# svenstaro/bvh

Measured on AMD Instinct MI355X. Metric: Mrays/s (build+traverse), higher is better.
Workload: dtype f32; 1 GPU; configs[1]: create_n_cubes(10000), 120000 triangles f32/3D, 1000000 create_ray rays per GPU; step = build_par+flatten+traverse; triangles=120000, rays_per_gpu=1000000, rays_total=1000000, scene_dist=single, flat_array=eager, parallelism=rays sharded x1

## Files before the change

### bvh_amd/csrc/build.hip

```cpp
#include "flatten_node.hpp"

namespace bvhgpu {

constexpr int MAXLV = 96;
constexpr int CTR_SMALL = 0;
constexpr int CTR_MID2 = 2;
constexpr int CTR_FLAGS = 4;
constexpr int CTR_TOPMASK = BUILD_CTR_TOPMASK;
constexpr uint32_t BUILD_FLAG_NONFINITE = 1u;
constexpr uint32_t BUILD_FLAG_PERSIST_GAVE_UP = BSTAT_UNFINISHED;
constexpr uint32_t BUILD_FLAG_EMPTY_SPLIT = 2u;
#ifndef BVH_MID_SMALL_MAXN
#define BVH_MID_SMALL_MAXN 768
#endif
#ifndef BVH_MID_SMALL_THREADS
#define BVH_MID_SMALL_THREADS 384
#endif
template <typename T> struct MidSmallScene {
    static constexpr int MAXN = BVH_MID_SMALL_MAXN;
    static constexpr int THREADS = BVH_MID_SMALL_THREADS;
    static constexpr int HANDOFF = SMALL_MAX;
};
#ifndef BVH_MID_LARGE_MAXN
#define BVH_MID_LARGE_MAXN 1536
#endif
#ifndef BVH_MID_LARGE_THREADS
#define BVH_MID_LARGE_THREADS 256
#endif
template <typename T> struct MidLargeScene {
    static constexpr int MAXN = sizeof(T) == 4 ? BVH_MID_LARGE_MAXN : BVH_MID_LARGE_MAXN * 2 / 3;
    static constexpr int THREADS = BVH_MID_LARGE_THREADS;
    static constexpr int HANDOFF = SMALL_MAX;
};
constexpr size_t MID_SCENE_SPLIT = 250000;
#ifndef BVH_STAT_REP
#define BVH_STAT_REP 8
#endif
constexpr int STAT_REP = BVH_STAT_REP;
constexpr int CTR_LEVEL0 = 16;
constexpr int CTR_XDIR = CTR_LEVEL0 + 2 * MAXLV;
static_assert((CTR_XDIR + 8 * 4) * 4 <= 1024, "the directory lives inside the counter page");
constexpr size_t ROOTKEY_OFF = 1024;
constexpr int PREP_MAX_WG = 1024;

__host__ __device__ inline int lvl_slot(int L) { return L < MAXLV - 2 ? L : (MAXLV - 2 + (L & 1)); }

template <typename T> struct ItemStats {
    typename Traits<T>::Key k[NUM_BUCKETS * STAT_KEYS];
    uint32_t cnt[NUM_BUCKETS];
    uint32_t _pad[2];
};

template <typename T> struct LevelArgs {
    Item<T>* item[2];
    uint4* tile_map[3];
    ItemStats<T>* stats[3];
    uint32_t* tile_cnt[3];
    uint8_t* bk[2];
    uint32_t slot_div, n_slots, n_tiles;
};

template <typename T> struct BuildArgs {
    LevelArgs<T> lv;
    uint32_t mid_max;
    const T* aabbs;
    const T* src;
    typename Traits<T>::Node* nodes;
    uint32_t* node_start;
    uint32_t* node_count;
    uint32_t* shape_node;
    uint16_t* node_slot;
    uint32_t* slot_entry;
    uint32_t n_slots;
    uint32_t* wslot_node;
    uint32_t* idx[2];
    uint8_t* bk;
    Item<T>* big[2];
    Item<T>* mid2;
    Item<T>* small;
    ItemStats<T>* stats[2];
    uint32_t* tile_item[2];
    uint32_t* tile_cnt;
    uint32_t* chunk_cnt[2];
    uint32_t n_chunks;
    FlattenArgs<T> fl;
    uint32_t fl_parts;
    uint32_t tile2;
    uint32_t* ctr;
    typename Traits<T>::Key* rootkeys;
    uint32_t prep_wgs;
    uint32_t n;
    unsigned long long* xbar;
};
constexpr int XBAR_WORDS = 8 * 32;

__device__ __forceinline__ bool key_is_min(int j) { return j < 3 || (j >= 6 && j < 9); }

template <typename T>
__device__ void push_item(const BuildArgs<T>& a, int next_level, uint32_t ni, uint32_t parent, uint32_t start,
                          uint32_t count, const T* A, const T* C, uint32_t heap, int lane);
template <typename T> __device__ void init_stats(ItemStats<T>* s, int lane);

template <typename T> __global__ __launch_bounds__(256) void k_prep(BuildArgs<T> a) {
    using Tr = Traits<T>;
    using Key = typename Tr::Key;
    __shared__ Key sk[STAT_KEYS];
    if (threadIdx.x < STAT_KEYS) sk[threadIdx.x] = key_is_min(threadIdx.x) ? Tr::KEY_POS_INF : Tr::KEY_NEG_INF;
    __syncthreads();
    T loc[STAT_KEYS];
#pragma unroll
    for (int j = 0; j < STAT_KEYS; j++) loc[j] = key_is_min(j) ? Tr::inf() : -Tr::inf();
    if (a.lv.tile_map[0]) {
        const uint32_t gt = blockIdx.x * blockDim.x + threadIdx.x, gs = gridDim.x * blockDim.x;
        for (uint32_t i = gt; i < 3u * a.lv.n_tiles; i += gs) a.lv.tile_map[i / a.lv.n_tiles][i % a.lv.n_tiles] = make_uint4(NONE, 0u, 0u, 0u);
        const uint32_t nc = a.lv.n_tiles * (uint32_t)NUM_BUCKETS;
        for (uint32_t i = gt; i < 3u * nc; i += gs) a.lv.tile_cnt[i / nc][i % nc] = 0u;
    }
    if (a.lv.tile_map[0] && blockIdx.x == 0 && threadIdx.x < WAVE)
        for (int r = 0; r < STAT_REP; r++) init_stats<T>(&a.lv.stats[0][r], (int)threadIdx.x);
    if (a.xbar && blockIdx.x == 0)
        for (uint32_t i = threadIdx.x; i < (uint32_t)XBAR_WORDS; i += blockDim.x) a.xbar[i] = 0ull;
    if (a.chunk_cnt[0] && blockIdx.x == 1 % gridDim.x)
        for (uint32_t i = threadIdx.x; i < 2u * a.n_chunks * 2u * (uint32_t)NUM_BUCKETS; i += blockDim.x) a.chunk_cnt[0][i] = 0u;
    if (blockIdx.x == 0) {
        for (uint32_t i = threadIdx.x; i < a.n_slots; i += blockDim.x) a.slot_entry[i] = NONE;
        for (uint32_t i = threadIdx.x; i < WIDE_SLOTS; i += blockDim.x) a.wslot_node[i] = NONE;
    }
    const bool copy = a.src != a.aabbs;
    T* own = const_cast<T*>(a.aabbs);
    bool bad = false;
    for (uint32_t i = blockIdx.x * blockDim.x + threadIdx.x; i < a.n; i += gridDim.x * blockDim.x) {
        a.idx[0][i] = i;
        const T* b = a.src + 6 * (size_t)i;
        T bx[6];
#pragma unroll
        for (int k = 0; k < 6; k++) bx[k] = b[k];
#pragma unroll
        for (int k = 0; k < 6; k++) bad = bad || !(fabs(bx[k]) < Tr::inf());
        if (copy) {
#pragma unroll
            for (int k = 0; k < 6; k++) own[6 * (size_t)i + k] = bx[k];
        }
#pragma unroll
        for (int k = 0; k < 3; k++) {
            const T c = center1(bx[k], bx[3 + k]);
            loc[k] = join_min(loc[k], bx[k]);
            loc[3 + k] = join_max(loc[3 + k], bx[3 + k]);
            loc[6 + k] = join_min(loc[6 + k], c);
            loc[9 + k] = join_max(loc[9 + k], c);
        }
    }
    {
        const int lane = lane_id();
#pragma unroll
        for (int d = 32; d > 0; d >>= 1) {
            T u[STAT_KEYS];
#pragma unroll
            for (int j = 0; j < STAT_KEYS; j++) u[j] = lane_fetch(loc[j], (lane ^ d) << 2);
#pragma unroll
            for (int j = 0; j < STAT_KEYS; j++) loc[j] = key_is_min(j) ? join_min(loc[j], u[j]) : join_max(loc[j], u[j]);
        }
        if (lane == 0) {
#pragma unroll
            for (int j = 0; j < STAT_KEYS; j++) {
                if (key_is_min(j)) atomicMin(&sk[j], Tr::key(loc[j]));
                else atomicMax(&sk[j], Tr::key(loc[j]));
            }
        }
    }
    if (a.n > 1 && __any(bad) && lane_id() == 0) atomicOr(&a.ctr[CTR_FLAGS], BUILD_FLAG_NONFINITE);
    __syncthreads();
    if (threadIdx.x < STAT_KEYS) a.rootkeys[(size_t)blockIdx.x * STAT_KEYS + threadIdx.x] = sk[threadIdx.x];
}

template <typename T> __global__ __launch_bounds__(256) void k_root(BuildArgs<T> a, uint32_t prep_wgs, int fused) {
    using Tr = Traits<T>;
    using Key = typename Tr::Key;
    __shared__ Key sk[STAT_KEYS];
    if (threadIdx.x < STAT_KEYS) sk[threadIdx.x] = key_is_min(threadIdx.x) ? Tr::KEY_POS_INF : Tr::KEY_NEG_INF;
    __syncthreads();
    for (uint32_t e = threadIdx.x; e < prep_wgs * (uint32_t)STAT_KEYS; e += blockDim.x) {
        const Key v = a.rootkeys[e];
        const int j = (int)(e % (uint32_t)STAT_KEYS);
        if (key_is_min(j)) atomicMin(&sk[j], v);
        else atomicMax(&sk[j], v);
    }
    __syncthreads();
    if (threadIdx.x < WAVE) {
        T A[6], C[6];
#pragma unroll
        for (int k = 0; k < 6; k++) { A[k] = Tr::unkey(sk[k]); C[k] = Tr::unkey(sk[6 + k]); }
        uint32_t flags = a.ctr[CTR_FLAGS];
        if (a.n > 1) {
            bool ovf = false;
#pragma unroll
            for (int k = 0; k < 3; k++) ovf = ovf || !(fabs(C[3 + k] - C[k]) < Tr::inf());
            if (ovf) { flags |= BUILD_FLAG_NONFINITE; if (threadIdx.x == 0) atomicOr(&a.ctr[CTR_FLAGS], BUILD_FLAG_NONFINITE); }
        }
        if (flags & BUILD_FLAG_NONFINITE) return;
        if (fused && a.n > a.mid_max) {
            const int lane = (int)threadIdx.x;
            Item<T>* it = &a.lv.item[0][0];
            if (lane == 0) {
                it->ni = 0; it->parent = 0; it->start = 0; it->count = a.n; it->tile_base = 0; it->parity = 0; it->heap = 1u; it->_r1 = 0;
                a.ctr[CTR_LEVEL0] = 1u;
            }
            if (lane < 6) { it->A[lane] = A[lane]; it->C[lane] = C[lane]; }
            const uint32_t ntile = (a.n + TILE - 1) / TILE;
            for (uint32_t j = lane; j < ntile; j += WAVE) a.lv.tile_map[0][j] = make_uint4(0u, 0u, a.n, 0u);
            for (int r = 0; r < STAT_REP; r++) init_stats<T>(&a.lv.stats[0][r], lane);
        } else {
            push_item<T>(a, 0, 0u, 0u, 0u, a.n, A, C, 1u, (int)threadIdx.x);
        }
    }
}

template <typename T> __device__ void init_stats(ItemStats<T>* s, int lane) {
    using Tr = Traits<T>;
    for (int j = lane; j < NUM_BUCKETS * STAT_KEYS; j += WAVE)
        s->k[j] = key_is_min(j % STAT_KEYS) ? Tr::KEY_POS_INF : Tr::KEY_NEG_INF;
    if (lane < NUM_BUCKETS) s->cnt[lane] = 0;
}

template <typename T>
__device__ void push_item(const BuildArgs<T>& a, int next_level, uint32_t ni, uint32_t parent, uint32_t start,
                          uint32_t count, const T* A, const T* C, uint32_t heap, int lane) {
    const int nslot = lvl_slot(next_level);
    const int npar = next_level & 1;
    uint32_t slot = 0, tb = 0;
    const bool is_small = count <= (uint32_t)SMALL_MAX;
    const bool is_mid2 = !is_small && count <= a.mid_max;
    const uint32_t ntile = (count + a.tile2 - 1) / a.tile2;
    if (lane == 0) {
        if (is_small) slot = atomicAdd(&a.ctr[CTR_SMALL], 1u);
        else if (is_mid2) slot = atomicAdd(&a.ctr[CTR_MID2], 1u);
        else {
            slot = atomicAdd(&a.ctr[CTR_LEVEL0 + 2 * nslot], 1u);
            tb = atomicAdd(&a.ctr[CTR_LEVEL0 + 2 * nslot + 1], ntile);
        }
    }
    slot = __shfl(slot, 0);
    tb = __shfl(tb, 0);
    Item<T>* it = is_small ? &a.small[slot] : (is_mid2 ? &a.mid2[slot] : &a.big[npar][slot]);
    if (lane == 0) {
        it->ni = ni; it->parent = parent; it->start = start; it->count = count;
        it->tile_base = tb; it->parity = (uint32_t)npar; it->heap = heap; it->_r1 = 0;
    }
    if (lane < 6) { it->A[lane] = A[lane]; it->C[lane] = C[lane]; }
    if (!is_small && !is_mid2) {
        for (uint32_t j = lane; j < ntile; j += WAVE) a.tile_item[npar][tb + j] = slot;
        for (int r = 0; r < STAT_REP; r++) init_stats<T>(&a.stats[npar][(size_t)slot * STAT_REP + r], lane);
    }
}

template <typename T>
__device__ void push_pair(const BuildArgs<T>& a, int next_level, uint32_t parent, uint32_t li, uint32_t lstart, uint32_t lcount,
                          const T* AL, const T* CL, uint32_t lheap, uint32_t ri, uint32_t rstart, uint32_t rcount,
                          const T* AR, const T* CR, uint32_t rheap, int lane) {
    const int nslot = lvl_slot(next_level);
    const int npar = next_level & 1;
    const uint32_t mycount = lane == 0 ? lcount : rcount;
    const int mykind = mycount <= (uint32_t)SMALL_MAX ? 0 : (mycount <= a.mid_max ? 1 : 3);
    const uint32_t myntile = (mycount + a.tile2 - 1) / a.tile2;
    uint32_t slot = 0, tb = 0;
    if (lane < 2) {
        if (mykind == 0) slot = atomicAdd(&a.ctr[CTR_SMALL], 1u);
        else if (mykind == 1) slot = atomicAdd(&a.ctr[CTR_MID2], 1u);
        else {
            const unsigned long long old = atomicAdd(reinterpret_cast<unsigned long long*>(&a.ctr[CTR_LEVEL0 + 2 * nslot]),
                                                     1ull | ((unsigned long long)myntile << 32));
            slot = (uint32_t)old; tb = (uint32_t)(old >> 32);
        }
    }
#pragma unroll
    for (int side = 0; side < 2; side++) {
        const uint32_t cslot = __shfl(slot, side), ctb = __shfl(tb, side);
        const int kind = __shfl(mykind, side);
        const uint32_t ccount = side ? rcount : lcount, ntile = (ccount + a.tile2 - 1) / a.tile2;
        Item<T>* it = kind == 0 ? &a.small[cslot] : (kind == 1 ? &a.mid2[cslot] : &a.big[npar][cslot]);
        if (lane == 0) {
            it->ni = side ? ri : li; it->parent = parent; it->start = side ? rstart : lstart; it->count = ccount;
            it->tile_base = ctb; it->parity = (uint32_t)npar; it->heap = side ? rheap : lheap; it->_r1 = 0;
        }
        if (lane < 6) { it->A[lane] = side ? AR[lane] : AL[lane]; it->C[lane] = side ? CR[lane] : CL[lane]; }
        if (kind == 3) {
            for (uint32_t j = lane; j < ntile; j += WAVE) a.tile_item[npar][ctb + j] = cslot;
            for (int r = 0; r < STAT_REP; r++) init_stats<T>(&a.stats[npar][(size_t)cslot * STAT_REP + r], lane);
        }
    }
}

template <typename T> __global__ __launch_bounds__(256) void k_init(BuildArgs<T> a) {
    for (int i = threadIdx.x; i < (int)(ROOTKEY_OFF / 4); i += 256) a.ctr[i] = 0;
}

template <typename T> __global__ __launch_bounds__(256) void k_publish_build(BuildArgs<T> a, uint32_t* __restrict__ host_page) {
    for (int i = threadIdx.x; i < (int)(ROOTKEY_OFF / 4); i += 256) { host_page[i] = a.ctr[i]; a.ctr[i] = 0; }
    __threadfence_system();
}

#ifndef BVH_CHUNK_TILES
#define BVH_CHUNK_TILES 256
#endif
constexpr int SCATTER_AHEAD = 4;
constexpr int CHUNK_TILES = BVH_CHUNK_TILES;
constexpr int BIN_REP = 16;
template <typename T> __global__ __launch_bounds__(256) void k_bin(BuildArgs<T> a, int level) {
    using Tr = Traits<T>;
    using Key = typename Tr::Key;
    const int slot = lvl_slot(level), par = level & 1;
    const uint32_t ntiles = a.ctr[CTR_LEVEL0 + 2 * slot + 1];
    __shared__ Key sk[BIN_REP][NUM_BUCKETS * STAT_KEYS];
    __shared__ uint32_t sc[BIN_REP][NUM_BUCKETS];
    const uint32_t* idx = a.idx[par];
    const int rep = threadIdx.x & (BIN_REP - 1);
    for (uint32_t t = blockIdx.x; t < ntiles; t += gridDim.x) {
        const uint32_t item_id = a.tile_item[par][t];
        const Item<T>* it = &a.big[par][item_id];
        const uint32_t start = it->start, count = it->count;
        const uint32_t p0 = start + (t - it->tile_base) * a.tile2;
        const uint32_t pend = min(start + count, p0 + a.tile2);
        T C[6];
#pragma unroll
        for (int k = 0; k < 6; k++) C[k] = it->C[k];
        const int ax = largest_axis(C);
        const T cmin = C[ax];
        const T ext = C[3 + ax] - C[ax];
        const bool degen = ext < Tr::eps();
        const uint32_t half = count / 2;
        for (int j = threadIdx.x; j < BIN_REP * NUM_BUCKETS * STAT_KEYS; j += 256)
            (&sk[0][0])[j] = key_is_min(j % STAT_KEYS) ? Tr::KEY_POS_INF : Tr::KEY_NEG_INF;
        if (threadIdx.x < BIN_REP * NUM_BUCKETS) (&sc[0][0])[threadIdx.x] = 0;
        __syncthreads();
        for (uint32_t p = p0 + threadIdx.x; p < pend; p += 256) {
            const uint32_t s = idx[p];
            const T* b = a.aabbs + 6 * (size_t)s;
            T bx[6];
#pragma unroll
            for (int k = 0; k < 6; k++) bx[k] = b[k];
            T c[3];
#pragma unroll
            for (int k = 0; k < 3; k++) c[k] = center1(bx[k], bx[3 + k]);
            int bkt;
            if (degen) bkt = (p - start) < half ? 0 : 1;
            else bkt = bucket_of(c[ax], cmin, ext);
            a.bk[p] = (uint8_t)bkt;
            Key* kk = &sk[rep][bkt * STAT_KEYS];
#pragma unroll
            for (int k = 0; k < 3; k++) {
                atomicMin(&kk[k], Tr::key(bx[k]));
                atomicMax(&kk[3 + k], Tr::key(bx[3 + k]));
                Key kc = Tr::key(c[k]);
                atomicMin(&kk[6 + k], kc);
                atomicMax(&kk[9 + k], kc);
            }
            atomicAdd(&sc[rep][bkt], 1u);
        }
        __syncthreads();
        ItemStats<T>* gs = &a.stats[par][(size_t)item_id * STAT_REP + ((t - it->tile_base) & (STAT_REP - 1))];
        if (threadIdx.x < NUM_BUCKETS) {
            uint32_t c = 0;
#pragma unroll
            for (int r = 0; r < BIN_REP; r++) c += sc[r][threadIdx.x];
            sc[0][threadIdx.x] = c;
            a.tile_cnt[t * NUM_BUCKETS + threadIdx.x] = c;
            if (c) atomicAdd(&gs->cnt[threadIdx.x], c);
            if (c && count > (uint32_t)CHUNK_TILES * a.tile2) {
                const uint32_t blk = t / (uint32_t)CHUNK_TILES;
                const uint32_t slot = it->tile_base > blk * (uint32_t)CHUNK_TILES ? 1u : 0u;
                atomicAdd(&a.chunk_cnt[par][(size_t)(blk * 2u + slot) * NUM_BUCKETS + threadIdx.x], c);
            }
        }
        __syncthreads();
        if (threadIdx.x < NUM_BUCKETS * STAT_KEYS) {
            const int j = threadIdx.x;
            if (sc[0][j / STAT_KEYS]) {
                Key v = sk[0][j];
                const bool mn = key_is_min(j % STAT_KEYS);
#pragma unroll
                for (int r = 1; r < BIN_REP; r++) { const Key u = sk[r][j]; v = mn ? (u < v ? u : v) : (u > v ? u : v); }
                if (mn) atomicMin(&gs->k[j], v);
                else atomicMax(&gs->k[j], v);
            }
        }
        __syncthreads();
    }
}

template <typename T> __device__ __forceinline__ void box_empty(T* b) {
    b[0] = b[1] = b[2] = Traits<T>::inf();
    b[3] = b[4] = b[5] = -Traits<T>::inf();
}
template <typename T> __device__ __forceinline__ void box_join(T* a, const T* b) {
#pragma unroll
    for (int k = 0; k < 3; k++) {
        a[k] = tmin(a[k], b[k]);
        a[3 + k] = tmax(a[3 + k], b[3 + k]);
    }
}

template <typename T, typename KeyPtr, typename CntPtr>
__device__ __forceinline__ uint32_t sah_select(KeyPtr keys, CntPtr cnts, const T* A, bool degen, uint32_t* cnt, T* AL,
                                               T* CL, T* AR, T* CR, bool& no_winner) {
    using Tr = Traits<T>;
    using Key = typename Tr::Key;
    Key pa[NUM_BUCKETS][6], sa[NUM_BUCKETS][6];
#pragma unroll
    for (int b = 0; b < NUM_BUCKETS; b++) {
        cnt[b] = cnts[b];
#pragma unroll
        for (int k = 0; k < 6; k++) { pa[b][k] = keys[b * STAT_KEYS + k]; sa[b][k] = pa[b][k]; }
    }
#pragma unroll
    for (int b = 1; b < NUM_BUCKETS; b++) {
#pragma unroll
        for (int k = 0; k < 3; k++) {
            pa[b][k] = pa[b][k] < pa[b - 1][k] ? pa[b][k] : pa[b - 1][k];
            pa[b][3 + k] = pa[b][3 + k] > pa[b - 1][3 + k] ? pa[b][3 + k] : pa[b - 1][3 + k];
        }
    }
#pragma unroll
    for (int b = NUM_BUCKETS - 2; b >= 0; b--) {
#pragma unroll
        for (int k = 0; k < 3; k++) {
            sa[b][k] = sa[b][k] < sa[b + 1][k] ? sa[b][k] : sa[b + 1][k];
            sa[b][3 + k] = sa[b][3 + k] > sa[b + 1][3 + k] ? sa[b][3 + k] : sa[b + 1][3 + k];
        }
    }
    T min_cost = Tr::inf();
    int best = -1;
    const T sa_parent = surface_area(A);
    uint32_t ln = 0, total = 0;
#pragma unroll
    for (int b = 0; b < NUM_BUCKETS; b++) total += cnt[b];
#pragma unroll
    for (int s = 0; s < NUM_BUCKETS - 1; s++) {
        ln += cnt[s];
        T la[6], ra[6];
#pragma unroll
        for (int k = 0; k < 6; k++) { la[k] = Tr::unkey(pa[s][k]); ra[k] = Tr::unkey(sa[s + 1][k]); }
        T cl = (T)ln * surface_area(la);
        T cr = (T)(total - ln) * surface_area(ra);
        T num = cl + cr;
        T cost = num / sa_parent;
        bool take = degen ? (s == 0) : (cost < min_cost);
        if (take) { min_cost = cost; best = s; }
    }
    no_winner = best < 0;
    if (best < 0) {
        box_empty(AL); box_empty(CL); box_empty(AR); box_empty(CR);
        return cnt[0];
    }
    Key cl_[6], cr_[6];
#pragma unroll
    for (int k = 0; k < 6; k++) {
        cl_[k] = key_is_min(k) ? Tr::KEY_POS_INF : Tr::KEY_NEG_INF;
        cr_[k] = cl_[k];
    }
    uint32_t nl = 0;
#pragma unroll
    for (int b = 0; b < NUM_BUCKETS; b++) {
        const bool left = b <= best;
        if (left) nl += cnt[b];
#pragma unroll
        for (int k = 0; k < 6; k++) {
            const Key v = keys[b * STAT_KEYS + 6 + k];
            const Key jl = key_is_min(k) ? (v < cl_[k] ? v : cl_[k]) : (v > cl_[k] ? v : cl_[k]);
            const Key jr = key_is_min(k) ? (v < cr_[k] ? v : cr_[k]) : (v > cr_[k] ? v : cr_[k]);
            cl_[k] = left ? jl : cl_[k];
            cr_[k] = left ? cr_[k] : jr;
        }
    }
#pragma unroll
    for (int k = 0; k < 6; k++) {
        Key l = pa[0][k], r = sa[1][k];
#pragma unroll
        for (int s = 1; s < NUM_BUCKETS - 1; s++) { if (best == s) { l = pa[s][k]; r = sa[s + 1][k]; } }
        AL[k] = Tr::unkey(l); AR[k] = Tr::unkey(r);
        CL[k] = Tr::unkey(cl_[k]); CR[k] = Tr::unkey(cr_[k]);
    }
    return nl;
}

template <typename T> __device__ void select_role(const BuildArgs<T>& a, int level, uint32_t block, uint32_t nblocks) {
    using Tr = Traits<T>;
    const int slot = lvl_slot(level), par = level & 1;
    const uint32_t nitems = a.ctr[CTR_LEVEL0 + 2 * slot];
    const int lane = lane_id();
    const uint32_t wave0 = (block * blockDim.x + threadIdx.x) >> 6;
    const uint32_t nwaves = (nblocks * blockDim.x) >> 6;
    for (uint32_t id = wave0; id < nitems; id += nwaves) {
        const Item<T>* it = &a.big[par][id];
        __shared__ ItemStats<T> s_merged[4];
        ItemStats<T>* st = &s_merged[threadIdx.x >> 6];
        {
            using Key = typename Tr::Key;
            const ItemStats<T>* rep = &a.stats[par][(size_t)id * STAT_REP];
            for (int j = lane; j < NUM_BUCKETS * STAT_KEYS; j += WAVE) {
                const bool mn = key_is_min(j % STAT_KEYS);
                Key v = rep[0].k[j];
#pragma unroll
                for (int r = 1; r < STAT_REP; r++) { const Key u = rep[r].k[j]; v = mn ? (u < v ? u : v) : (u > v ? u : v); }
                st->k[j] = v;
            }
            if (lane < NUM_BUCKETS) {
                uint32_t c = 0;
#pragma unroll
                for (int r = 0; r < STAT_REP; r++) c += rep[r].cnt[lane];
                st->cnt[lane] = c;
            }
        }
        const uint32_t ni = it->ni, parent = it->parent, start = it->start, count = it->count;
        T A[6], C[6];
#pragma unroll
        for (int k = 0; k < 6; k++) { A[k] = it->A[k]; C[k] = it->C[k]; }
        const int ax = largest_axis(C);
        const T ext = C[3 + ax] - C[ax];
        const bool degen = ext < Tr::eps();

        uint32_t cnt[NUM_BUCKETS];
        T AL[6], CL[6], AR[6], CR[6];
        bool no_winner;
        const uint32_t nl = sah_select<T>(st->k, st->cnt, A, degen, cnt, AL, CL, AR, CR, no_winner);
        if (no_winner && lane == 0) atomicOr(&a.ctr[CTR_FLAGS], BUILD_FLAG_EMPTY_SPLIT);
        const uint32_t li = ni + 1;
        const uint32_t ri = li + (2 * nl - 1);
        if (lane == 0) {
            typename Tr::Node* nd = &a.nodes[ni];
#pragma unroll
            for (int k = 0; k < 3; k++) {
                nd->l_min[k] = AL[k]; nd->l_max[k] = AL[3 + k];
                nd->r_min[k] = AR[k]; nd->r_max[k] = AR[3 + k];
            }
            nd->parent = parent; nd->l = li; nd->r = ri; nd->shape = NONE;
            a.node_start[ni] = start;
            a.node_count[ni] = count;
            a.node_slot[ni] = (uint16_t)it->heap;
            if (it->heap < 16u) atomicOr(&a.ctr[CTR_TOPMASK], 1u << it->heap);
        }
        push_pair<T>(a, level + 1, ni, li, start, nl, AL, CL, heap_child(it->heap, 0u), ri, start + nl, count - nl, AR, CR,
                     heap_child(it->heap, 1u), lane);

    }
}

template <typename T> __device__ void scatter_role(const BuildArgs<T>& a, int level, uint32_t block, uint32_t nblocks) {
    const int slot = lvl_slot(level), par = level & 1;
    const uint32_t ntiles = a.ctr[CTR_LEVEL0 + 2 * slot + 1];
    __shared__ uint32_t run[NUM_BUCKETS];
    __shared__ uint32_t wcnt[4][NUM_BUCKETS];
    __shared__ __attribute__((aligned(16))) uint32_t wcnt2[2][NUM_BUCKETS][4];
    const int lane = lane_id(), w = threadIdx.x >> 6;
    const unsigned long long lt = lanemask_lt();
    const uint32_t* src = a.idx[par];
    uint32_t* dst = a.idx[par ^ 1];
    for (uint32_t t = block; t < ntiles; t += nblocks) {
        const Item<T>* it = &a.big[par][a.tile_item[par][t]];
        const uint32_t start = it->start, count = it->count;
        const uint32_t p0 = start + (t - it->tile_base) * a.tile2;
        const uint32_t pend = min(start + count, p0 + a.tile2);
        {
            const uint32_t tl = t - it->tile_base, ntl = (count + a.tile2 - 1) / a.tile2;
            uint32_t before[NUM_BUCKETS], all[NUM_BUCKETS];
#pragma unroll
            for (int b = 0; b < NUM_BUCKETS; b++) { before[b] = 0; all[b] = 0; }
            const uint32_t* tc = a.tile_cnt + (size_t)it->tile_base * NUM_BUCKETS;
            if (count > (uint32_t)CHUNK_TILES * a.tile2) {
                const uint32_t T0 = it->tile_base, T1 = T0 + ntl;
                const uint32_t g0 = T0 / (uint32_t)CHUNK_TILES, g1 = (T1 - 1u) / (uint32_t)CHUNK_TILES, gt = t / (uint32_t)CHUNK_TILES;
                const uint32_t* cc = a.chunk_cnt[par];
                for (uint32_t g = g0 + threadIdx.x; g <= g1; g += 256) {
                    const uint32_t sl = T0 > g * (uint32_t)CHUNK_TILES ? 1u : 0u;
#pragma unroll
                    for (int b = 0; b < NUM_BUCKETS; b++) {
                        const uint32_t v = cc[(size_t)(g * 2u + sl) * NUM_BUCKETS + b];
                        all[b] += v;
                        before[b] += g < gt ? v : 0u;
                    }
                }
                const uint32_t j0 = max(gt * (uint32_t)CHUNK_TILES, T0);
                for (uint32_t j = j0 + threadIdx.x; j < t; j += 256) {
#pragma unroll
                    for (int b = 0; b < NUM_BUCKETS; b++) before[b] += a.tile_cnt[(size_t)j * NUM_BUCKETS + b];
                }
            } else {
                for (uint32_t j = threadIdx.x; j < ntl; j += 256) {
#pragma unroll
                    for (int b = 0; b < NUM_BUCKETS; b++) {
                        const uint32_t v = tc[(size_t)j * NUM_BUCKETS + b];
                        all[b] += v;
                        before[b] += j < tl ? v : 0u;
                    }
                }
            }
            uint32_t mine[NUM_BUCKETS];
            uint32_t acc = 0;
#pragma unroll
            for (int b = 0; b < NUM_BUCKETS; b++) { mine[b] = acc + before[b]; acc += all[b]; }
#pragma unroll
// ... 1230 lines not shown
        T salv[NUM_BUCKETS - 1], sarv[NUM_BUCKETS - 1];
        {
            int cum = 0;
#pragma unroll
            for (int s2 = 0; s2 < NUM_BUCKETS - 1; s2++) { cum += cnt[s2]; cumv[s2] = cum; }
        }
#pragma unroll
        for (int s2 = 0; s2 < NUM_BUCKETS - 1; s2++) {
            const int q2 = lo + cumv[s2];
            salv[s2] = lane_fetch(saP, (q2 - 1) << 2);
            sarv[s2] = lane_fetch(saS, q2 << 2);
        }
        int nl = cnt[0];
        bool taken = false;
        T min_cost = Tr::inf();
#pragma unroll
        for (int s2 = 0; s2 < NUM_BUCKETS - 1; s2++) {
            T cl = (T)cumv[s2] * salv[s2];
            T cr = (T)(segn - cumv[s2]) * sarv[s2];
            T num = cl + cr;
            T cost = num / saA;
            bool take = degen ? (s2 == 0) : (cost < min_cost);
            if (take) { min_cost = cost; nl = cumv[s2]; taken = true; }
        }
        const int q = lo + nl;
        const int ql4 = (q - 1) << 2, qr4 = q << 2;
        T AL[6], AR[6], Cn[6];
        const bool left = lane < q;
        {
#pragma unroll
            for (int k = 0; k < 6; k++) AL[k] = lane_fetch(P[k], ql4);
#pragma unroll
            for (int k = 0; k < 6; k++) AR[k] = lane_fetch(S[k], qr4);
            const int nlo = done ? lane : (left ? lo : q), nhi = done ? lane + 1 : (left ? q : hi);
            T Cq[6];
#pragma unroll
            for (int k = 0; k < 3; k++) { Cq[k] = c[k]; Cq[3 + k] = c[k]; }
            seg_prefix_scan<T, 6>(Cq, lane, nlo, span);
            const int last4 = (nhi - 1) << 2;
#pragma unroll
            for (int k = 0; k < 6; k++) Cn[k] = lane_fetch(Cq[k], last4);
        }
        if (!taken) { box_empty(AL); box_empty(AR); box_empty(Cn); }
        if (!done && !taken && lane == lo) atomicOr(&a.ctr[CTR_FLAGS], BUILD_FLAG_EMPTY_SPLIT);
        if constexpr (FLAT_INLINE) {
            wave_empty = wave_empty || __any(!done && !taken);
            const unsigned long long cm = __ballot(!done && lane == lo);
            if (!done && lane == lo) my_inner[ninner + (uint32_t)__popcll(cm & lt)] = ni;
            ninner += (uint32_t)__popcll(cm);
        }
        if (!done) {
            const uint32_t li = ni + 1;
            const uint32_t ri = li + (uint32_t)(2 * nl - 1);
            if (lane == lo) {
                typename Tr::Node* nd = &a.nodes[ni];
#pragma unroll
                for (int k = 0; k < 3; k++) {
                    nd->l_min[k] = AL[k]; nd->l_max[k] = AL[3 + k];
                    nd->r_min[k] = AR[k]; nd->r_max[k] = AR[3 + k];
                }
                nd->parent = parent; nd->l = li; nd->r = ri; nd->shape = NONE;
                a.node_start[ni] = istart + lo;
                a.node_count[ni] = segn;
                a.node_slot[ni] = (uint16_t)heap;
            }
            parent = ni;
            if (left) { hi = q; ni = li; saA = surface_area(AL); heap = heap_child(heap, 0u); }
            else { lo = q; ni = ri; saA = surface_area(AR); heap = heap_child(heap, 1u); }
#pragma unroll
            for (int k = 0; k < 6; k++) Cb[k] = Cn[k];
        }
    }
    if constexpr (FLAT_INLINE && sizeof(T) == 4) if (a.fl_parts != 0u) {
        __builtin_amdgcn_fence(__ATOMIC_SEQ_CST, "workgroup");
        const bool with_flat = (a.fl_parts & (uint32_t)FLATTEN_FLAT) != 0u;
        const bool fast = n >= 2 && !(with_flat && wave_empty);
        if (fast) {
            if (with_flat && lane < n) {
                const uint32_t nav = ni - 1u + (istart + (uint32_t)lane);
                typename Tr::Flat fe = {}, lf = {};
#pragma unroll
                for (int k = 0; k < 3; k++) { fe.min[k] = box[k]; fe.max[k] = box[3 + k]; lf.min[k] = Tr::inf(); lf.max[k] = -Tr::inf(); }
                fe.entry = nav + 1u; fe.exit = nav + 2u; fe.shape = NONE;
                lf.entry = NONE; lf.exit = nav + 2u; lf.shape = shape;
                a.fl.flat[nav] = fe;
                a.fl.flat[nav + 1u] = lf;
            }
        }
        const uint32_t nn_item = 2u * (uint32_t)n - 1u;
        const uint32_t todo = fast ? ninner : nn_item;
#pragma unroll 1
        for (uint32_t j = (uint32_t)lane; j < todo; j += WAVE) {
            const uint32_t i = fast ? my_inner[j] : ni0 + j;
            const typename Tr::Node ndf = a.fl.nodes[i];
            if (with_flat) flatten_node<T, FLATTEN_FLAT | FLATTEN_WIDE>(a.fl, i, ndf);
            else flatten_node<T, FLATTEN_WIDE>(a.fl, i, ndf);
        }
    }
#ifdef BVH_SMALL_PROFILE
    if (sp_on) g_small_prof[20 * wave + 18] = wall_clock64();
#endif
    }
}

template <typename T> struct LevelLayout {
    size_t n_slots, n_tiles, sz_tile_item, sz_tile_cnt, sz_stats, off_tile_item, off_tile_cnt, off_stats, bytes;
    LevelLayout(size_t n, size_t mid_max) {
        n_slots = n / (mid_max + 1) + 2;
        n_tiles = n / TILE + n_slots + 4;
        auto up = [](size_t x) { return (x + 255) & ~(size_t)255; };
        sz_tile_item = up(n_tiles * 16);
        sz_tile_cnt = up(n_tiles * NUM_BUCKETS * 4);
        sz_stats = up(n_slots * STAT_REP * sizeof(ItemStats<T>));
        off_tile_item = 0;
        off_tile_cnt = off_tile_item + 3 * sz_tile_item;
        off_stats = off_tile_cnt + 3 * sz_tile_cnt;
        bytes = off_stats + 3 * sz_stats;
    }
};

template <typename T> static bool level_fused(const bvhgpu_tree* t) {
    const int v = t->ctx->tune[BVHGPU_TUNE_BUILD_LEVEL_LAUNCHES];
    return v == 1 || (v != 2 && t->n <= MID_SCENE_SPLIT);
}
template <typename T> static uint32_t level_tile(const bvhgpu_tree* t) {
    if (level_fused<T>(t)) return (uint32_t)TILE;
    const int v = t->ctx->tune[BVHGPU_TUNE_BUILD_LEVEL_TILE];
    if (v > 0) return (uint32_t)std::min(std::max((v + 255) / 256 * 256, (int)TILE), 16384);
    return t->n >= 6000000 ? 4096u : t->n >= 2000000 ? 2048u : t->n >= 600000 ? 1024u : (uint32_t)TILE;
}

template <typename T> static BuildArgs<T> make_args(bvhgpu_tree* t, const T* src) {
    using Tr = Traits<T>;
    using Key = typename Tr::Key;
    BuildArgs<T> a;
    a.aabbs = t->aabbs.as<T>();
    a.src = src ? src : t->aabbs.as<T>();
    a.nodes = t->nodes.as<typename Tr::Node>();
    a.node_start = t->node_start.as<uint32_t>();
    a.node_count = t->node_count.as<uint32_t>();
    a.shape_node = t->shape_node.as<uint32_t>();
    a.node_slot = t->node_slot.as<uint16_t>();
    a.slot_entry = t->slot_entry.as<uint32_t>();
    a.n_slots = TopCfg<T>::SLOTS;
    a.wslot_node = t->wslot_node.as<uint32_t>();
    a.idx[0] = t->idx[0].as<uint32_t>(); a.idx[1] = t->idx[1].as<uint32_t>();
    a.bk = t->bk.as<uint8_t>();
    a.big[0] = t->big[0].as<Item<T>>(); a.big[1] = t->big[1].as<Item<T>>();
    a.mid2 = t->mid2.as<Item<T>>();
    a.small = t->small.as<Item<T>>();
    a.stats[0] = t->stats[0].as<ItemStats<T>>(); a.stats[1] = t->stats[1].as<ItemStats<T>>();
    a.tile_item[0] = t->tile_item[0].as<uint32_t>(); a.tile_item[1] = t->tile_item[1].as<uint32_t>();
    a.tile_cnt = t->tile_cnt.as<uint32_t>();
    a.tile2 = level_tile<T>(t);
    a.fl = FlattenArgs<T>{}; a.fl_parts = 0;
    a.n_chunks = (uint32_t)(t->chunk_cnt.cap / (2 * 2 * NUM_BUCKETS * 4));
    a.chunk_cnt[0] = t->chunk_cnt.as<uint32_t>();
    a.chunk_cnt[1] = a.chunk_cnt[0] ? a.chunk_cnt[0] + (size_t)a.n_chunks * 2 * NUM_BUCKETS : nullptr;
    a.ctr = t->ctr.as<uint32_t>();
    a.rootkeys = reinterpret_cast<Key*>(reinterpret_cast<char*>(t->ctr.p) + ROOTKEY_OFF);
    a.n = (uint32_t)t->n;
    a.xbar = t->xbar.as<unsigned long long>();
    a.prep_wgs = 0;
    const bool small_scene = t->n <= MID_SCENE_SPLIT;
    a.mid_max = (uint32_t)(small_scene ? MidSmallScene<T>::MAXN : MidLargeScene<T>::MAXN);
    const LevelLayout<T> ly(t->n, a.mid_max);
    a.lv.slot_div = a.mid_max + 1u; a.lv.n_slots = (uint32_t)ly.n_slots; a.lv.n_tiles = (uint32_t)ly.n_tiles;
    char* base = t->lvbuf.cap >= ly.bytes ? reinterpret_cast<char*>(t->lvbuf.p) : nullptr;
    for (int i = 0; i < 3; i++) {
        a.lv.tile_map[i] = base ? reinterpret_cast<uint4*>(base + ly.off_tile_item + i * ly.sz_tile_item) : nullptr;
        a.lv.tile_cnt[i] = base ? reinterpret_cast<uint32_t*>(base + ly.off_tile_cnt + i * ly.sz_tile_cnt) : nullptr;
        a.lv.stats[i] = base ? reinterpret_cast<ItemStats<T>*>(base + ly.off_stats + i * ly.sz_stats) : nullptr;
    }
    a.lv.item[0] = a.big[0]; a.lv.item[1] = a.big[1];
    a.lv.bk[0] = a.bk; a.lv.bk[1] = a.bk ? a.bk + t->n : nullptr;
    return a;
}

template <typename T> struct BuildGrid {
    size_t max_big, max_mid2, max_tiles;
    int tile_grid, sel_grid, mid2_grid, small_grid, level_grid;
    BuildGrid(const bvhgpu_tree* t, size_t mid_max) {
        const size_t n = t->n;
        max_big = n / (mid_max + 1) + 2;
        max_mid2 = n / (SMALL_MAX + 1) + 2;
        max_tiles = n / TILE + max_big + 2;
        tile_grid = (int)std::min<size_t>(n / level_tile<T>(t) + max_big + 2, 2048);
        sel_grid = (int)std::min<size_t>((max_big + 3) / 4, 1024);
        mid2_grid = (int)std::min<size_t>(max_mid2, (size_t)t->ctx->n_cu * 4);
        small_grid = (int)std::min<size_t>((n + 3) / 4, (size_t)t->ctx->n_cu * 8);
        level_grid = (int)std::min<size_t>(LevelLayout<T>(n, mid_max).n_tiles, 2048);
    }
};

template <typename T> static void run_level(bvhgpu_tree* t, const BuildArgs<T>& a, const BuildGrid<T>& g, int L) {
    hipStream_t st = t->ctx->stream;
    if (level_fused<T>(t)) {
        if (L == 0) hipLaunchKernelGGL((k_level<T, true>), dim3(g.level_grid), dim3(LEVEL_THREADS), 0, st, a, 0);
        hipLaunchKernelGGL((k_level<T, false>), dim3(g.level_grid), dim3(LEVEL_THREADS), 0, st, a, L + 1);
        return;
    }
    hipLaunchKernelGGL(k_bin<T>, dim3(g.tile_grid), dim3(256), 0, st, a, L);
    hipLaunchKernelGGL(k_split<T>, dim3(g.sel_grid + g.tile_grid), dim3(256), 0, st, a, L, (uint32_t)g.sel_grid);
}
template <typename T> static void run_lower_tiers(bvhgpu_tree* t, const BuildArgs<T>& a, const BuildGrid<T>& g, uint32_t mid2_done,
                                                  uint32_t small_done) {
    hipStream_t st = t->ctx->stream;
    if (t->n > (size_t)SMALL_MAX) {
        if (t->n <= MID_SCENE_SPLIT) hipLaunchKernelGGL((k_mid<T, MidSmallScene<T>>), dim3(g.mid2_grid), dim3(MidSmallScene<T>::THREADS), 0, st, a, mid2_done);
        else hipLaunchKernelGGL((k_mid<T, MidLargeScene<T>>), dim3(g.mid2_grid), dim3(MidLargeScene<T>::THREADS), 0, st, a, mid2_done);
    }
    if (a.fl_parts != 0u) hipLaunchKernelGGL((k_small<T, true>), dim3(g.small_grid), dim3(256), 0, st, a, small_done);
    else hipLaunchKernelGGL((k_small<T, false>), dim3(g.small_grid), dim3(256), 0, st, a, small_done);
}

template <typename T> void build_enqueue(bvhgpu_tree* t, const T* aabbs_dev, size_t n, bool flatten_after, bool redo) {
    using Tr = Traits<T>;
    using Key = typename Tr::Key;
    bvhgpu_ctx* ctx = t->ctx;
    hipStream_t st = ctx->stream;
    join_flat(t);
    t->built = false; t->flattened = false; t->lazy_flat = false; t->pending_build = false; t->exact_only = false; t->pending_recv = false;
    t->pend_persist = false;
    if (!redo) t->gen++;
    if (n != t->n) { t->has_tris = false; t->has_spheres = false; }
    t->n = n; t->n_nodes = n ? 2 * n - 1 : 0;
    t->n_flat = n >= 2 ? 3 * n - 2 : n;
    t->n_trav = n >= 2 ? 2 * n - 2 : n;
    t->levels = 0;
    if (n == 0) { t->built = true; t->flattened = flatten_after; return; }

    const size_t MID_MAX = n <= MID_SCENE_SPLIT ? (size_t)MidSmallScene<T>::MAXN : (size_t)MidLargeScene<T>::MAXN;
    const BuildGrid<T> g(t, MID_MAX);
    t->aabbs.reserve(n * 6 * sizeof(T));
    if (t->nodes.reserve(t->n_nodes * sizeof(typename Tr::Node))) BVH_HIP(hipMemsetAsync(t->nodes.p, 0, t->nodes.cap, st));
    if (t->node_start.reserve(t->n_nodes * 4)) BVH_HIP(hipMemsetAsync(t->node_start.p, 0, t->node_start.cap, st));
    if (t->node_count.reserve(t->n_nodes * 4)) BVH_HIP(hipMemsetAsync(t->node_count.p, 0, t->node_count.cap, st));
    t->shape_node.reserve(n * 4);
    if (t->node_slot.reserve(t->n_nodes * 2)) BVH_HIP(hipMemsetAsync(t->node_slot.p, 0xFF, t->node_slot.cap, st));
    t->slot_entry.reserve(TopCfg<T>::SLOTS * 4);
    t->wslot_node.reserve(WIDE_SLOTS * 4);
    t->idx[0].reserve(n * 4);
    t->idx[1].reserve(n * 4);
    t->bk.reserve(2 * n);
    if (level_fused<T>(t) && n > (size_t)MID_MAX) t->lvbuf.reserve(LevelLayout<T>(n, MID_MAX).bytes);
    const int persist_knob = ctx->tune[BVHGPU_TUNE_BUILD_LEVEL_PERSIST];
    if (t->persist_broken && persist_knob != 0 && !redo && t->persist_retry_in > 0 && --t->persist_retry_in == 0) t->persist_broken = false;
    const bool persist = persist_knob != 0 && !t->persist_broken && level_fused<T>(t) && n >= 32 * (MID_MAX + 1);
    if (persist) t->xbar.reserve(XBAR_WORDS * sizeof(unsigned long long));
    for (int i = 0; i < 2; i++) {
        t->big[i].reserve(g.max_big * sizeof(Item<T>));
        t->stats[i].reserve(g.max_big * STAT_REP * sizeof(ItemStats<T>));
        t->tile_item[i].reserve(g.max_tiles * 4);
    }
    t->mid2.reserve(g.max_mid2 * sizeof(Item<T>));
    t->small.reserve((n + 1) * sizeof(Item<T>));
    t->tile_cnt.reserve(g.max_tiles * NUM_BUCKETS * 4);
    if (!level_fused<T>(t)) t->chunk_cnt.reserve((g.max_tiles / CHUNK_TILES + 2) * 2 * 2 * NUM_BUCKETS * 4);
    if (t->ctr.reserve(ROOTKEY_OFF + (size_t)PREP_MAX_WG * STAT_KEYS * sizeof(Key))) t->ctr_ready = false;
    if (!t->pin) BVH_HIP(hipHostMalloc(&t->pin, ROOTKEY_OFF, hipHostMallocDefault));

    BuildArgs<T> a = make_args<T>(t, aabbs_dev);
    if (!t->ctr_ready) hipLaunchKernelGGL(k_init<T>, dim3(1), dim3(256), 0, st, a);
    t->ctr_ready = false;
#ifndef BVH_PREP_PER_WG
#define BVH_PREP_PER_WG 1024
#endif
    const int prep_grid = (int)std::min<size_t>((n + BVH_PREP_PER_WG - 1) / BVH_PREP_PER_WG, (size_t)PREP_MAX_WG);
    a.prep_wgs = (uint32_t)prep_grid;
    hipLaunchKernelGGL(k_prep<T>, dim3(prep_grid), dim3(256), 0, st, a);
    if (!(level_fused<T>(t) && n > (size_t)MID_MAX)) hipLaunchKernelGGL(k_root<T>, dim3(1), dim3(256), 0, st, a, (uint32_t)prep_grid, 0);

    int level = 0;
    if (n > (size_t)MID_MAX) {
        int fixed = 1;
        for (size_t m = n; m > (size_t)MID_MAX; m = (m + 1) / 2) fixed++;
        if (t->hint_levels > 0 && t->hint_n == n) fixed = t->hint_levels;
        if (fixed > MAXLV - 4) fixed = MAXLV - 4;
        if (persist) {
            for (; level < 3; level++) run_level<T>(t, a, g, level);
            const int nx = persist_knob >= 8 ? std::min(persist_knob, 64) : 32;
            hipLaunchKernelGGL((k_level<T, false, true>), dim3(8 * nx), dim3(LEVEL_THREADS), 0, st, a, 4);
            t->pend_persist = true;
            fixed = level;
        }
        for (; level < fixed; level++) {
            run_level<T>(t, a, g, level);
            if (level == 3 && ctx->tune[BVHGPU_TUNE_WIDE_EARLY_ITEMS] != 0 && !t->pend_persist) {
                if (!t->ev_top) BVH_HIP(hipEventCreateWithFlags(&t->ev_top, hipEventDisableTiming));
                BVH_HIP(hipEventRecord(t->ev_top, st));
                t->ev_top_gen = t->gen;
            }
        }
    }
    uint32_t inline_parts = 0;
    if (flatten_after && n >= 2 && sizeof(T) == 4 && ctx->tune[BVHGPU_TUNE_FLATTEN_INLINE] != 0) {
        const FlattenPlan p = flatten_plan<T>(t, ctx->tune[BVHGPU_TUNE_FLATTEN_LAZY] != 0);
        if (p.with_wide) {
            inline_parts = (uint32_t)(p.parts & (FLATTEN_FLAT | FLATTEN_WIDE));
            a.fl = flatten_args<T>(t, p.with_wide, p.with_guide); a.fl_parts = inline_parts;
        }
    }
    run_lower_tiers<T>(t, a, g, 0u, 0u);
    t->bstat.reserve(64);
    if (flatten_after && n >= 1)
        flatten_tree<T>(t, a.ctr, reinterpret_cast<uint32_t*>(t->pin), (uint32_t)(ROOTKEY_OFF / 4), t->bstat.as<uint32_t>(), (uint32_t)CTR_FLAGS,
                        (n > (size_t)MID_MAX && !t->pend_persist) ? (uint32_t)(CTR_LEVEL0 + 2 * lvl_slot(level)) : (uint32_t)CTR_FLAGS,
                        ctx->tune[BVHGPU_TUNE_FLATTEN_LAZY] != 0, inline_parts);
    else hipLaunchKernelGGL(k_publish_build<T>, dim3(1), dim3(256), 0, st, a, reinterpret_cast<uint32_t*>(t->pin));
    t->ctr_ready = true;
    t->pending_build = true; t->pend_level = level; t->pend_flatten = flatten_after;
}

template <typename T> void build_finalize(bvhgpu_tree* t) {
    if (!t->pending_build) return;
    t->pending_build = false;
    bvhgpu_ctx* ctx = t->ctx;
    hipStream_t st = ctx->stream;
    join_flat(t);
    BVH_HIP(hipStreamSynchronize(st));
    BVH_HIP(hipGetLastError());
    const size_t n = t->n;
    const size_t MID_MAX = n <= MID_SCENE_SPLIT ? (size_t)MidSmallScene<T>::MAXN : (size_t)MidLargeScene<T>::MAXN;
    uint32_t* pin = reinterpret_cast<uint32_t*>(t->pin);
    if (pin[CTR_FLAGS] & BUILD_FLAG_NONFINITE) {
        t->flattened = false;
        t->failed_gen = t->gen; t->failed_what = Fail::NonFinite;
        throw HipFail{hipErrorInvalidValue, nullptr, __LINE__, Fail::NonFinite};
    }
    if (t->pend_persist && (pin[CTR_FLAGS] & BUILD_FLAG_PERSIST_GAVE_UP)) {
        t->persist_broken = true;
        t->persist_retry_in = 64;
        const bool fl = t->pend_flatten;
        build_enqueue<T>(t, static_cast<const T*>(nullptr), n, fl, true);
        build_finalize<T>(t);
        t->redone_gen = t->gen;
        return;
    }
    int level = t->pend_persist ? MAXLV - 3 : t->pend_level;
    if (n > (size_t)MID_MAX && !t->pend_persist && pin[CTR_LEVEL0 + 2 * lvl_slot(level)] != 0) {
        const BuildGrid<T> g(t, MID_MAX);
        const BuildArgs<T> a = make_args<T>(t, nullptr);
        BVH_HIP(hipMemcpyAsync(a.ctr, t->pin, ROOTKEY_OFF, hipMemcpyHostToDevice, st));
        t->ctr_ready = false;
        uint32_t mid2_done = pin[CTR_MID2], small_done = pin[CTR_SMALL];
        while (true) {
            if (level + 1 >= MAXLV - 2)
                BVH_HIP(hipMemsetAsync(a.ctr + CTR_LEVEL0 + 2 * lvl_slot(level + 1), 0, 8, st));
            run_level<T>(t, a, g, level);
            level++;
            BVH_HIP(hipMemcpyAsync(t->pin, a.ctr, ROOTKEY_OFF, hipMemcpyDeviceToHost, st));
            BVH_HIP(hipStreamSynchronize(st));
            if (pin[CTR_LEVEL0 + 2 * lvl_slot(level)] == 0) break;
        }
        run_lower_tiers<T>(t, a, g, mid2_done, small_done);
        hipLaunchKernelGGL(k_publish_build<T>, dim3(1), dim3(256), 0, st, a, reinterpret_cast<uint32_t*>(t->pin));
        t->ctr_ready = true;
        if (t->pend_flatten) {
            BVH_HIP(hipMemsetAsync(t->wslot_node.p, 0xFF, WIDE_SLOTS * 4, st));
            BVH_HIP(hipMemsetAsync(t->slot_entry.p, 0xFF, TopCfg<T>::SLOTS * 4, st));
            flatten_tree<T>(t);
        }
        BVH_HIP(hipStreamSynchronize(st));
        BVH_HIP(hipGetLastError());
        t->redone_gen = t->gen;
    }
    int used = level;
    while (used > 0 && used - 1 < MAXLV - 2 && pin[CTR_LEVEL0 + 2 * (used - 1)] == 0) used--;
    t->levels = used;
    if (!t->pend_persist) { t->hint_levels = used > 0 ? used : 0; t->hint_n = n; }
    t->exact_only = (pin[CTR_FLAGS] & BUILD_FLAG_EMPTY_SPLIT) != 0;
    t->built = true;
}

template <typename T> void build_tree(bvhgpu_tree* t, const T* aabbs_dev, size_t n, bool flatten_after) {
    build_enqueue<T>(t, aabbs_dev, n, flatten_after, false);
    build_finalize<T>(t);
}

#ifdef BVH_PROFILE_MID
void debug_mid_prof(unsigned long long* out, bool reset) {
    (void)hipDeviceSynchronize();
    (void)hipMemcpyFromSymbol(out, HIP_SYMBOL(g_mid_prof), sizeof(unsigned long long) * 8);
    if (reset) { unsigned long long z[8] = {0}; (void)hipMemcpyToSymbol(HIP_SYMBOL(g_mid_prof), z, sizeof z); }
}
#endif

template void build_tree<float>(bvhgpu_tree*, const float*, size_t, bool);
template void build_tree<double>(bvhgpu_tree*, const double*, size_t, bool);
template void build_enqueue<float>(bvhgpu_tree*, const float*, size_t, bool, bool);
template void build_enqueue<double>(bvhgpu_tree*, const double*, size_t, bool, bool);
template void build_finalize<float>(bvhgpu_tree*);
template void build_finalize<double>(bvhgpu_tree*);

}
```

### bvh_amd/csrc/common.hpp

```cpp
#pragma once

#include <hip/hip_runtime.h>
#include <stdint.h>

#include <cfloat>
#include <cmath>

#include "../../include/bvh_mi355x.h"

namespace bvhgpu {

constexpr uint32_t NONE = BVHGPU_NONE;
constexpr int NUM_BUCKETS = 6;
constexpr int WAVE = 64;
constexpr int SMALL_MAX = 64;
#ifndef BVH_TILE
#define BVH_TILE 512
#endif
constexpr int TILE = BVH_TILE;
constexpr int STAT_KEYS = 12;

template <typename T> struct Traits;

template <> struct Traits<float> {
    using Key = uint32_t;
    using Node = bvhgpu_node_f32;
    using Flat = bvhgpu_flat_f32;
    using Ray = bvhgpu_ray_f32;
    static constexpr int dtype = BVHGPU_F32;
    __host__ __device__ static constexpr float eps() { return FLT_EPSILON; }
    __host__ __device__ static float inf() { return INFINITY; }
    __host__ __device__ static Key key(float f) {
        uint32_t b;
        __builtin_memcpy(&b, &f, 4);
        return (b & 0x80000000u) ? ~b : (b | 0x80000000u);
    }
    __host__ __device__ static float unkey(Key k) {
        uint32_t b = (k & 0x80000000u) ? (k & 0x7FFFFFFFu) : ~k;
        float f;
        __builtin_memcpy(&f, &b, 4);
        return f;
    }
    static constexpr Key KEY_POS_INF = 0xFF800000u;
    static constexpr Key KEY_NEG_INF = 0x007FFFFFu;
};

template <> struct Traits<double> {
    using Key = unsigned long long;
    using Node = bvhgpu_node_f64;
    using Flat = bvhgpu_flat_f64;
    using Ray = bvhgpu_ray_f64;
    static constexpr int dtype = BVHGPU_F64;
    __host__ __device__ static constexpr double eps() { return DBL_EPSILON; }
    __host__ __device__ static double inf() { return INFINITY; }
    __host__ __device__ static Key key(double f) {
        unsigned long long b;
        __builtin_memcpy(&b, &f, 8);
        return (b & 0x8000000000000000ull) ? ~b : (b | 0x8000000000000000ull);
    }
    __host__ __device__ static double unkey(Key k) {
        unsigned long long b = (k & 0x8000000000000000ull) ? (k & 0x7FFFFFFFFFFFFFFFull) : ~k;
        double f;
        __builtin_memcpy(&f, &b, 8);
        return f;
    }
    static constexpr Key KEY_POS_INF = 0xFFF0000000000000ull;
    static constexpr Key KEY_NEG_INF = 0x000FFFFFFFFFFFFFull;
};

template <typename T> struct TravNode;
template <> struct __attribute__((aligned(32))) TravNode<float> {
    float mn[3];
    uint32_t exit;
    float mx[3];
    uint32_t shape;
};
template <> struct __attribute__((aligned(64))) TravNode<double> {
    double mn[3];
    double mx[3];
    uint32_t exit;
    uint32_t shape;
    uint64_t _pad;
};
constexpr uint32_t TRAV_INNER = 0x80000000u;
constexpr uint32_t SLOT_NONE = 0xFFFFu;
__host__ __device__ inline bool trav_is_leaf(uint32_t w) { return (w & TRAV_INNER) == 0u; }
__host__ __device__ inline uint32_t heap_child(uint32_t h, uint32_t side) {
    const uint32_t c = 2u * h + side;
    return (h >= 0x8000u || c > SLOT_NONE) ? SLOT_NONE : c;
}
template <typename T> struct TopCfg;
#ifndef BVH_TOP_SLOTS_F32
#define BVH_TOP_SLOTS_F32 5056
#endif
template <> struct TopCfg<float> { static constexpr uint32_t SLOTS = BVH_TOP_SLOTS_F32; };
template <> struct TopCfg<double> { static constexpr uint32_t SLOTS = 2880; };
static_assert(sizeof(TravNode<float>) == 32, "trav f32");
static_assert(sizeof(TravNode<double>) == 64, "trav f64");

template <typename T> struct WideNode;
template <> struct __attribute__((aligned(128))) WideNode<float> {
    float mn[3][4], mx[3][4];
    uint32_t ref[4];
    uint32_t _pad[4];
};
template <> struct __attribute__((aligned(256))) WideNode<double> {
    double mn[3][4], mx[3][4];
    uint32_t ref[4];
    uint32_t _pad[12];
};
static_assert(sizeof(WideNode<float>) == 128, "wide f32");
static_assert(sizeof(WideNode<double>) == 256, "wide f64");
constexpr double GUIDE_GROW = 1.0 / 262144.0;
constexpr double GUIDE_ORIGIN_MAX = 3.0;
constexpr double GUIDE_SCENE_MIN = 0x1p-125;
constexpr double GUIDE_SCENE_MAX = 0x1p125;
constexpr double GUIDE_F32_MAX = 0x1.fffffep127;
constexpr double GUIDE_F32_MIN_NORMAL = 0x1p-126;
__host__ __device__ inline float f32_below(double x) {
    float f = (float)x;
    if ((double)f > x) {
        uint32_t b; __builtin_memcpy(&b, &f, 4);
        b = f > 0.0f ? b - 1u : (f < 0.0f ? b + 1u : 0x80000001u);
        __builtin_memcpy(&f, &b, 4);
    }
    return f;
}
__host__ __device__ inline float f32_above(double x) { return -f32_below(-x); }
constexpr uint32_t WIDE_INNER = 0x80000000u;
constexpr uint32_t WIDE_RESIDENT = 0x40000000u;
constexpr size_t WIDE_MAX_SHAPES = (size_t)1 << 28;
constexpr uint32_t WIDE_SLOTS = 1365;
__host__ __device__ inline uint32_t wide_level_base(int k) { return ((1u << (2 * k)) - 1u) / 3u; }

template <typename T> struct Item {
    uint32_t ni;
    uint32_t parent;
    uint32_t start;
    uint32_t count;
    uint32_t tile_base;
    uint32_t parity;
    uint32_t heap;
    uint32_t _r1;
    T A[6];
    T C[6];
};

template <typename T> __host__ __device__ inline T tmin(T a, T b) {
    return (a < b || (a == b && signbit(a))) ? a : b;
}
template <typename T> __host__ __device__ inline T tmax(T a, T b) {
    return (a > b || (a == b && !signbit(a))) ? a : b;
}
template <typename T> __host__ __device__ inline T center1(T mn, T mx) {
    T lo = mn * (T)0.5;
    T hi = mx * (T)0.5;
    return lo + hi;
}
template <typename T> __host__ __device__ inline T surface_area(const T* b) {
    T sx = b[3] - b[0], sy = b[4] - b[1], sz = b[5] - b[2];
    T xx = sx * sx, yy = sy * sy, zz = sz * sz;
    T d = xx + yy;
    d = d + zz;
    return (T)2 * d;
}
template <typename T> __host__ __device__ inline int largest_axis(const T* b) {
    T s0 = b[3] - b[0], s1 = b[4] - b[1], s2 = b[5] - b[2];
    int a = 0;
    T m = s0;
    if (s1 > m) { m = s1; a = 1; }
    if (s2 > m) { m = s2; a = 2; }
    return a;
}
template <typename T> __host__ __device__ inline int bucket_of(T c, T cmin, T ext) {
    const T K = (T)NUM_BUCKETS - (T)0.01;
    T rel = (c - cmin) / ext;
    T scaled = rel * K;
    return (int)scaled;
}

__device__ __forceinline__ float join_min(float a, float b) { float r; asm("v_min_f32 %0, %1, %2" : "=v"(r) : "v"(a), "v"(b)); return r; }
__device__ __forceinline__ float join_max(float a, float b) { float r; asm("v_max_f32 %0, %1, %2" : "=v"(r) : "v"(a), "v"(b)); return r; }
__device__ __forceinline__ double join_min(double a, double b) { double r; asm("v_min_f64 %0, %1, %2" : "=v"(r) : "v"(a), "v"(b)); return r; }
__device__ __forceinline__ double join_max(double a, double b) { double r; asm("v_max_f64 %0, %1, %2" : "=v"(r) : "v"(a), "v"(b)); return r; }

template <typename T>
__device__ __forceinline__ bool slab_hit(const T o[3], const T inv[3], const T mn[3], const T mx[3], T& tmin_out,
                                         T& tmax_out) {
    T l0 = (mn[0] - o[0]) * inv[0], h0 = (mx[0] - o[0]) * inv[0];
    T l1 = (mn[1] - o[1]) * inv[1], h1 = (mx[1] - o[1]) * inv[1];
    T l2 = (mn[2] - o[2]) * inv[2], h2 = (mx[2] - o[2]) * inv[2];
    bool nan = (l0 != l0) | (h0 != h0) | (l1 != l1) | (h1 != h1) | (l2 != l2) | (h2 != h2);
    T a0 = join_min(l0, h0), b0 = join_max(l0, h0);
    T a1 = join_min(l1, h1), b1 = join_max(l1, h1);
    T a2 = join_min(l2, h2), b2 = join_max(l2, h2);
    T tmn = join_max(join_max(a0, a1), a2);
    T tmx = join_min(join_min(b0, b1), b2);
    T z = tmn > (T)0 ? tmn : (T)0;
    tmin_out = z;
    tmax_out = tmx;
    return !nan && (tmx >= z);
}

template <typename T>
__device__ __forceinline__ bool slab_hit_finite(const T o[3], const T inv[3], const T mn[3], const T mx[3]) {
    T l0 = (mn[0] - o[0]) * inv[0], h0 = (mx[0] - o[0]) * inv[0];
    T l1 = (mn[1] - o[1]) * inv[1], h1 = (mx[1] - o[1]) * inv[1];
    T l2 = (mn[2] - o[2]) * inv[2], h2 = (mx[2] - o[2]) * inv[2];
    T tmn = fmax(fmax(fmin(l0, h0), fmin(l1, h1)), fmin(l2, h2));
    T tmx = fmin(fmin(fmax(l0, h0), fmax(l1, h1)), fmax(l2, h2));
    return tmx >= fmax(tmn, (T)0);
}
template <>
__device__ __forceinline__ bool slab_hit_finite<float>(const float o[3], const float inv[3], const float mn[3],
                                                       const float mx[3]) {
    float l0 = (mn[0] - o[0]) * inv[0], h0 = (mx[0] - o[0]) * inv[0];
    float l1 = (mn[1] - o[1]) * inv[1], h1 = (mx[1] - o[1]) * inv[1];
    float l2 = (mn[2] - o[2]) * inv[2], h2 = (mx[2] - o[2]) * inv[2];
    float a0, a1, a2, b0, b1, b2, tmn, tmx;
    asm("v_min_f32 %0, %1, %2" : "=v"(a0) : "v"(l0), "v"(h0));
    asm("v_max_f32 %0, %1, %2" : "=v"(b0) : "v"(l0), "v"(h0));
    asm("v_min_f32 %0, %1, %2" : "=v"(a1) : "v"(l1), "v"(h1));
    asm("v_max_f32 %0, %1, %2" : "=v"(b1) : "v"(l1), "v"(h1));
    asm("v_min_f32 %0, %1, %2" : "=v"(a2) : "v"(l2), "v"(h2));
    asm("v_max_f32 %0, %1, %2" : "=v"(b2) : "v"(l2), "v"(h2));
    asm("v_max3_f32 %0, %1, %2, %3" : "=v"(tmn) : "v"(a0), "v"(a1), "v"(a2));
    asm("v_min3_f32 %0, %1, %2, %3" : "=v"(tmx) : "v"(b0), "v"(b1), "v"(b2));
    return (tmx >= tmn) & (tmx >= 0.0f);
}
template <typename T>
__device__ __forceinline__ bool slab_hit_finite_len(const T o[3], const T inv[3], const T mn[3], const T mx[3], T& len) {
    T l0 = (mn[0] - o[0]) * inv[0], h0 = (mx[0] - o[0]) * inv[0];
    T l1 = (mn[1] - o[1]) * inv[1], h1 = (mx[1] - o[1]) * inv[1];
    T l2 = (mn[2] - o[2]) * inv[2], h2 = (mx[2] - o[2]) * inv[2];
    T tmn = fmax(fmax(fmin(l0, h0), fmin(l1, h1)), fmin(l2, h2));
    T tmx = fmin(fmin(fmax(l0, h0), fmax(l1, h1)), fmax(l2, h2));
    const T t0 = fmax(tmn, (T)0);
    len = tmx - t0;
    return tmx >= t0;
}
template <>
__device__ __forceinline__ bool slab_hit_finite_len<float>(const float o[3], const float inv[3], const float mn[3], const float mx[3],
                                                           float& len) {
    float l0 = (mn[0] - o[0]) * inv[0], h0 = (mx[0] - o[0]) * inv[0];
    float l1 = (mn[1] - o[1]) * inv[1], h1 = (mx[1] - o[1]) * inv[1];
    float l2 = (mn[2] - o[2]) * inv[2], h2 = (mx[2] - o[2]) * inv[2];
    float a0, a1, a2, b0, b1, b2, tmn, tmx, t0;
    asm("v_min_f32 %0, %1, %2" : "=v"(a0) : "v"(l0), "v"(h0));
    asm("v_max_f32 %0, %1, %2" : "=v"(b0) : "v"(l0), "v"(h0));
    asm("v_min_f32 %0, %1, %2" : "=v"(a1) : "v"(l1), "v"(h1));
    asm("v_max_f32 %0, %1, %2" : "=v"(b1) : "v"(l1), "v"(h1));
    asm("v_min_f32 %0, %1, %2" : "=v"(a2) : "v"(l2), "v"(h2));
    asm("v_max_f32 %0, %1, %2" : "=v"(b2) : "v"(l2), "v"(h2));
    asm("v_max3_f32 %0, %1, %2, %3" : "=v"(tmn) : "v"(a0), "v"(a1), "v"(a2));
    asm("v_min3_f32 %0, %1, %2, %3" : "=v"(tmx) : "v"(b0), "v"(b1), "v"(b2));
    asm("v_max_f32 %0, 0, %1" : "=v"(t0) : "v"(tmn));
    len = tmx - t0;
    return tmx >= t0;
}
template <typename T> __device__ __forceinline__ bool ray_is_finite(const T o[3], const T inv[3]) {
    bool f = true;
#pragma unroll
    for (int k = 0; k < 3; k++)
        f = f && (fabs(o[k]) < Traits<T>::inf()) && (fabs(inv[k]) < Traits<T>::inf()) && (inv[k] != (T)0);
    return f;
}

__device__ __forceinline__ float lane_fetch(float v, int addr4) {
    return __int_as_float(__builtin_amdgcn_ds_bpermute(addr4, __float_as_int(v)));
}
__device__ __forceinline__ double lane_fetch(double v, int addr4) {
    const long long b = __double_as_longlong(v);
    const int lo = __builtin_amdgcn_ds_bpermute(addr4, (int)(b & 0xFFFFFFFFll));
    const int hi = __builtin_amdgcn_ds_bpermute(addr4, (int)(b >> 32));
    return __longlong_as_double(((long long)hi << 32) | (unsigned int)lo);
}
template <int CTRL, int ROW_MASK = 0xF> __device__ __forceinline__ float dpp_fetch(float v) {
    const int b = __float_as_int(v);
    return __int_as_float(__builtin_amdgcn_update_dpp(b, b, CTRL, ROW_MASK, 0xF, false));
}
template <int CTRL, int ROW_MASK = 0xF> __device__ __forceinline__ double dpp_fetch(double v) {
    const long long b = __double_as_longlong(v);
    const int lo = (int)(b & 0xFFFFFFFFll), hi = (int)(b >> 32);
    const int l2 = __builtin_amdgcn_update_dpp(lo, lo, CTRL, ROW_MASK, 0xF, false);
    const int h2 = __builtin_amdgcn_update_dpp(hi, hi, CTRL, ROW_MASK, 0xF, false);
    return __longlong_as_double(((long long)h2 << 32) | (unsigned int)l2);
}
template <int CTRL, int ROW_MASK = 0xF> __device__ __forceinline__ float dpp_fetch_raw(float v) {
    return __int_as_float(__builtin_amdgcn_mov_dpp(__float_as_int(v), CTRL, ROW_MASK, 0xF, false));
}
template <int CTRL, int ROW_MASK = 0xF> __device__ __forceinline__ double dpp_fetch_raw(double v) {
    const long long b = __double_as_longlong(v);
    const int l2 = __builtin_amdgcn_mov_dpp((int)(b & 0xFFFFFFFFll), CTRL, ROW_MASK, 0xF, false);
    const int h2 = __builtin_amdgcn_mov_dpp((int)(b >> 32), CTRL, ROW_MASK, 0xF, false);
    return __longlong_as_double(((long long)h2 << 32) | (unsigned int)l2);
}
template <int LANE> __device__ __forceinline__ float lane_bcast(float v) { return __int_as_float(__builtin_amdgcn_readlane(__float_as_int(v), LANE)); }
template <int LANE> __device__ __forceinline__ double lane_bcast(double v) {
    const long long b = __double_as_longlong(v);
    const int lo = __builtin_amdgcn_readlane((int)(b & 0xFFFFFFFFll), LANE), hi = __builtin_amdgcn_readlane((int)(b >> 32), LANE);
    return __longlong_as_double(((long long)hi << 32) | (unsigned int)lo);
}
__device__ __forceinline__ int lane_id() { return (int)(threadIdx.x & 63); }
#ifndef BVH_LDS_BARRIER
#define BVH_LDS_BARRIER 1
#endif
__device__ __forceinline__ void lds_barrier() {
#if BVH_LDS_BARRIER
    asm volatile("s_waitcnt lgkmcnt(0)\n\ts_barrier" ::: "memory");
#else
    __syncthreads();
#endif
}
__device__ __forceinline__ unsigned long long lanemask_lt() {
    int l = lane_id();
    return l == 0 ? 0ull : (~0ull >> (64 - l));
}
__device__ __forceinline__ unsigned long long mask_range(int lo, int hi) {
    unsigned long long h = hi >= 64 ? ~0ull : ((1ull << hi) - 1ull);
    unsigned long long l = lo >= 64 ? ~0ull : ((1ull << lo) - 1ull);
    return h & ~l;
}

enum class Fail { None, NonFinite, Overflow, Rebroadcast, RecvRebroadcast, RecvInvalid, RecvGarbled, StaleTree, OrderedDepth };
struct HipFail { hipError_t err; const char* what; int line; Fail kind = Fail::None; };
#define BVH_HIP(x)                                                     \
    do {                                                               \
        hipError_t _e = (x);                                           \
        if (_e != hipSuccess) throw ::bvhgpu::HipFail{_e, #x, __LINE__}; \
    } while (0)

}
```

### bvh_amd/csrc/engine.hpp

```cpp
#pragma once

#include <string>
#include <vector>

#include "common.hpp"

namespace bvhgpu {

struct DevBuf {
    void* p = nullptr;
    size_t cap = 0;
    DevBuf() = default;
    DevBuf(const DevBuf&) = delete;
    DevBuf& operator=(const DevBuf&) = delete;
    ~DevBuf() { release(); }
    bool reserve(size_t bytes) {
        if (bytes <= cap) return false;
        if (p) (void)hipFree(p);
        p = nullptr;
        cap = 0;
        size_t want = bytes + bytes / 8 + 256;
        hipError_t e = hipMalloc(&p, want);
        if (e != hipSuccess) {
            p = nullptr;
            throw HipFail{e, "hipMalloc", __LINE__};
        }
        cap = want;
        return true;
    }
    void release() {
        if (p) (void)hipFree(p);
        p = nullptr;
        cap = 0;
    }
    template <typename U> U* as() const { return reinterpret_cast<U*>(p); }
};

constexpr unsigned TRAVERSE_ANY_HIT = 1u << 31;
constexpr unsigned TRAVERSE_BOX_HIT = 1u << 30;
constexpr unsigned TRAVERSE_SPHERE_HIT = 1u << 29;
constexpr unsigned TRAVERSE_ALLHITS = 1u << 28;

}

struct bvhgpu_comm;
struct bvhgpu_hits;
namespace bvhgpu {
struct HostBatch {
    static constexpr int MAX_CHUNKS = 16;
    bvhgpu_hits* hits[MAX_CHUNKS] = {};
    hipEvent_t ev_up[MAX_CHUNKS] = {}, ev_done[MAX_CHUNKS] = {};
    hipStream_t up = nullptr, up2 = nullptr, down = nullptr;
    hipEvent_t ev_main = nullptr, ev_aabbs = nullptr, ev_up2[MAX_CHUNKS] = {};
    DevBuf indices;
    static constexpr size_t IDX_STAGE_MAX = (size_t)1 << 26;
    size_t idx_stage = 0;
    uint64_t guess = 0;
    DevBuf od;
    DevBuf rays;
    DevBuf offsets;
    size_t n_rays = 0, r0[MAX_CHUNKS + 1] = {};
    int chunks = 0;
    uint64_t total = 0;
    bool fetched = false;
    bool zero_copy_in = false;
    uint32_t* offsets_host = nullptr;
    uint32_t* indices_host = nullptr;
    bool od6 = false;
    bool with_od = false;
    ~HostBatch() {
        for (auto& h : hits) if (h) { bvhgpu_hits_destroy(h); h = nullptr; }
        for (auto& e : ev_up) if (e) (void)hipEventDestroy(e);
        for (auto& e : ev_done) if (e) (void)hipEventDestroy(e);
        if (up) { (void)hipStreamSynchronize(up); (void)hipStreamDestroy(up); }
        if (up2) { (void)hipStreamSynchronize(up2); (void)hipStreamDestroy(up2); }
        for (auto& e : ev_up2) if (e) (void)hipEventDestroy(e);
        if (ev_main) (void)hipEventDestroy(ev_main);
        if (ev_aabbs) (void)hipEventDestroy(ev_aabbs);
        if (down) { (void)hipStreamSynchronize(down); (void)hipStreamDestroy(down); }
    }
};
}

#ifndef BVH_FLATTEN_INLINE_DEFAULT
#define BVH_FLATTEN_INLINE_DEFAULT 1
#endif
struct bvhgpu_ctx {
    int device = 0;
    hipStream_t stream = nullptr;
    bool own_stream = false;
    std::string err;
    int n_cu = 256;
    int tune[BVHGPU_TUNE_COUNT] = {3, -1, -1, 16384, 0, 0, 1, 0, 0, 0, 0, 0, -1, 1, 1, 1, 0, 0, 256, 2, 0, BVH_FLATTEN_INLINE_DEFAULT, -1};
    bool timing = false;
    hipEvent_t ev[8] = {};
    unsigned ev_set = 0;
    bvhgpu_timings last = {0, 0, 0, 0};
    bvhgpu::DevBuf upload;
    bvhgpu::DevBuf counters;
    void* pinned = nullptr;
    bvhgpu::HostBatch* host = nullptr;
    hipStream_t side = nullptr;
    ~bvhgpu_ctx() {
        delete host;
        for (auto& e : ev) if (e) (void)hipEventDestroy(e);
        if (pinned) (void)hipHostFree(pinned);
        if (side) { (void)hipStreamSynchronize(side); (void)hipStreamDestroy(side); }
        if (own_stream && stream) (void)hipStreamDestroy(stream);
    }
};

struct bvhgpu_tree {
    bvhgpu_ctx* ctx = nullptr;
    int dtype = BVHGPU_F32;
    size_t n = 0;
    size_t n_nodes = 0;
    size_t n_flat = 0;
    size_t n_trav = 0;
    bool built = false;
    bool flattened = false;
    bool lazy_flat = false;
    int lazy_parts = 0;
    bool flat_beside = false;
    hipEvent_t ev_flat0 = nullptr, ev_flat = nullptr;
    bool unfolded = false;
    bool ctr_ready = false;
    bool pending_build = false;
    bool pend_flatten = false;
    uint64_t gen = 0;
    uint64_t redone_gen = 0;
    uint64_t bcast_gen = 0;
    uint64_t failed_gen = 0;
    bvhgpu::Fail failed_what = bvhgpu::Fail::None;
    bool pending_recv = false;
    void* pin_recv = nullptr;
    bvhgpu_comm* recv_comm = nullptr;
    bvhgpu::DevBuf bstat;
    std::vector<bvhgpu_hits*> waiters;
    hipEvent_t ev_top = nullptr;
    uint64_t ev_top_gen = 0;
    bool exact_only = false;
    int pend_level = 0;
    bool pend_persist = false;
    bool persist_broken = false;
    int persist_retry_in = 0;
    int levels = 0;
    int hint_levels = 0;
    size_t hint_n = 0;
    void* pin = nullptr;
    bvhgpu::DevBuf aabbs;
    bvhgpu::DevBuf nodes;
    bvhgpu::DevBuf node_start;
    bvhgpu::DevBuf node_count;
    bvhgpu::DevBuf shape_node;
    bvhgpu::DevBuf flat;
    bvhgpu::DevBuf trav;
    bvhgpu::DevBuf wide;
    bvhgpu::DevBuf wslot_node;
    bool has_wide = false;
    bvhgpu::DevBuf wide_guide;
    bvhgpu::DevBuf guide_info;
    bool has_guide = false;
    bvhgpu::DevBuf tris;
    bool has_tris = false;
    bvhgpu::DevBuf spheres;
    bool has_spheres = false;
    bvhgpu::DevBuf slot_entry;
    bvhgpu::DevBuf node_slot;
    bvhgpu::DevBuf idx[2];
    bvhgpu::DevBuf bk;
    bvhgpu::DevBuf lvbuf;
    bvhgpu::DevBuf xbar;
    bvhgpu::DevBuf big[2];
    bvhgpu::DevBuf mid2;
    bvhgpu::DevBuf small;
    bvhgpu::DevBuf stats[2];
    bvhgpu::DevBuf tile_item[2];
    bvhgpu::DevBuf tile_cnt;
    bvhgpu::DevBuf chunk_cnt;
    bvhgpu::DevBuf ctr;
    bvhgpu::DevBuf refit_seg;
    ~bvhgpu_tree() {
        if (flat_beside && ctx && ctx->side) { (void)hipStreamSynchronize(ctx->side); flat_beside = false; }
        if (ev_flat0) (void)hipEventDestroy(ev_flat0);
        if (ev_flat) (void)hipEventDestroy(ev_flat);
        if (ev_top) (void)hipEventDestroy(ev_top);
        if (pin) (void)hipHostFree(pin);
        if (pin_recv) (void)hipHostFree(pin_recv);
    }
};

struct bvhgpu_hits {
    bvhgpu_ctx* ctx = nullptr;
    int dtype = BVHGPU_F32;
    size_t n_rays = 0;
    uint64_t total = 0;
    unsigned flags = 0;
    bvhgpu_traverse_stats stats = {0, 0, 0, 0, 0};
    bvhgpu::DevBuf counts;
    bvhgpu::DevBuf offsets;
    bvhgpu::DevBuf pool;
    bvhgpu::DevBuf pool_t;
    bvhgpu::DevBuf indices;
    bvhgpu::DevBuf tslice;
    bvhgpu::DevBuf isect;
    bvhgpu::DevBuf closest;
    bvhgpu::DevBuf closest_prim;
    bvhgpu::DevBuf closest_key;
    bool ckey_clean = false;
    bvhgpu::DevBuf blocksums;
    bvhgpu::DevBuf scan_sums;
    bvhgpu::DevBuf ctr;
    bvhgpu::DevBuf heap_dist, heap_node;
    uint32_t heap_cap = 48;
    size_t pool_cap = 0;
    size_t idx_cap = 0;
    bvhgpu::DevBuf raybuf;
    bool pend_staged = false;
    std::string walk_kernel;
    bool pend_rec8 = false;
    bool pend_guide = false, no_guide = false;
    uint32_t guide_backoff = 0, guide_skip = 0;
    bool ctr_clean = false;
    int ctr_set = 0;
    int bsum_set = 0;
    bvhgpu::DevBuf wcounts;
    bvhgpu::DevBuf ray_mask;
    bvhgpu::DevBuf ray_items;
    bvhgpu::DevBuf witems;
    bvhgpu::DevBuf item_cnt;
    bvhgpu::DevBuf wstack;
    bool wcounts_clean = false;
    bool bs_clean = false;
    bool force_binary = false;
    void* pin = nullptr;
    bvhgpu_tree* pend_tree = nullptr;
    const void* pend_rays = nullptr;
    bool pend_wide = false, pend_unfolded = false, pend_async = false;
    int pend_attempts = 0;
    bvhgpu_tree* wait_tree = nullptr;
    uint64_t pend_gen = 0;
    bool pend_on_pending = false;
    hipEvent_t ev_items = nullptr;
    bvhgpu::DevBuf wg_items;
    int pend_kind = 0;
    const void* pend_queries = nullptr;
    bool pend_qwide = false;
    bvhgpu::DevBuf qbuf;
    const void* pend_tmax = nullptr;
    bvhgpu::DevBuf tmaxbuf;
    bvhgpu::DevBuf any_key;
    bool akey_clean = false;
    bvhgpu::DevBuf any_part;
    int ah_leaf = 0;
    bvhgpu::DevBuf ah_vals;
    bvhgpu::DevBuf ah_counts, ah_sums;
    bvhgpu::DevBuf ah_work, ah_pos;
    uint32_t replays = 0;
    int deferred_rc = 0;
    std::string deferred_err;
    ~bvhgpu_hits() {
        if (ev_items) (void)hipEventDestroy(ev_items);
        if (pin) (void)hipHostFree(pin);
    }
};

namespace bvhgpu {

template <typename T> void build_tree(bvhgpu_tree* t, const T* aabbs_dev, size_t n, bool flatten_after);
template <typename T> void build_enqueue(bvhgpu_tree* t, const T* aabbs_dev, size_t n, bool flatten_after, bool redo = false);
template <typename T> void build_finalize(bvhgpu_tree* t);
template <typename T> void flatten_tree(bvhgpu_tree* t, uint32_t* pub_ctr = nullptr, uint32_t* pub_host = nullptr, uint32_t pub_words = 0,
                                        uint32_t* bstat = nullptr, uint32_t flags_idx = 0, uint32_t level_idx = 0, bool wide_only = false,
                                        uint32_t inline_parts = 0);
struct FlattenPlan { int parts = 0; bool with_wide = false, with_guide = false; };
template <typename T> FlattenPlan flatten_plan(bvhgpu_tree* t, bool wide_only);
void ensure_flat_arrays(bvhgpu_tree* t);
void join_flat(bvhgpu_tree* t);
constexpr uint32_t BSTAT_NONFINITE = 1u, BSTAT_EMPTY_SPLIT = 2u;
constexpr uint32_t BSTAT_UNFINISHED = 0x100u;
constexpr int BUILD_CTR_TOPMASK = 5;
template <typename T> void wide_from_trav(bvhgpu_tree* t);
void recv_finalize(bvhgpu_tree* t);
void settle_waiters(bvhgpu_tree* t);
template <typename T> void query_batch(bvhgpu_tree* t, int kind, const T* queries_dev, size_t n, bvhgpu_hits* h);
template <typename T> struct WalkOut;
template <typename T> void launch_query(bvhgpu_tree* t, size_t n, const WalkOut<T>& w, bvhgpu_hits* h, uint32_t* ovf_flag);
template <typename T> void refit_tree(bvhgpu_tree* t, const T* aabbs_dev);
template <typename T> bool refit_input_ok(bvhgpu_tree* t, const T* aabbs_dev);
template <typename T>
void traverse_batch(bvhgpu_tree* t, const typename Traits<T>::Ray* rays_dev, size_t n_rays, unsigned flags,
                    bvhgpu_hits* h);
template <typename T>
void traverse_enqueue(bvhgpu_tree* t, const typename Traits<T>::Ray* rays_dev, size_t n_rays, unsigned flags,
                      bvhgpu_hits* h);
bool traverse_check(bvhgpu_hits* h);
template <typename T>
void nearest_batch(bvhgpu_tree* t, const T* points_dev, size_t n, int kind, uint32_t* out_shape_dev, T* out_dist_dev);
template <typename T>
void knearest_batch(bvhgpu_tree* t, const T* points_dev, size_t n, int kind, uint32_t k, uint32_t* out_shape_dev, T* out_dist_dev);
template <typename T>
void knearest_tree_batch(bvhgpu_tree* t, const T* points_dev, size_t n, int kind, uint32_t k, const T* max_dist_dev, uint32_t* out_shape_dev,
                         T* out_dist_dev);
template <typename T>
void khits_batch(bvhgpu_tree* t, const typename Traits<T>::Ray* rays_dev, const T* tmax_dev, size_t n, int leaf, uint32_t k,
                 uint32_t* out_shape_dev, T* out_vals_dev);
template <typename T>
void allhits_batch(bvhgpu_tree* t, const typename Traits<T>::Ray* rays_dev, const T* tmax_dev, size_t n, int leaf, unsigned flags, bvhgpu_hits* h);
template <typename T>
void ray_triangle_pairs(bvhgpu_ctx* ctx, const typename Traits<T>::Ray* rays_dev, const T* tris_dev, size_t n, T* out_dev);
template <typename T>
void rays_new(bvhgpu_ctx* ctx, const T* origins_dev, const T* dirs_dev, size_t n, typename Traits<T>::Ray* out_dev, hipStream_t st = nullptr,
              unsigned max_blocks = 0, unsigned stride = 3);
void offsets_rebase(hipStream_t st, const uint32_t* offs_dev, size_t n_rays, uint32_t* out_dev, uint32_t* out_host = nullptr,
                    const uint32_t* idx_dev = nullptr, uint32_t* idx_all = nullptr, size_t idx_cap = 0, bool first = false);
void copy16(hipStream_t st, const void* src, void* dst, size_t bytes);
template <typename T>
void gen_primary(bvhgpu_ctx* ctx, const float cam[14], uint32_t width, uint32_t height, uint64_t first, size_t n,
                 typename Traits<T>::Ray* out_dev);
void gen_rays_f32(bvhgpu_ctx* ctx, uint64_t first, size_t n, const float bounds[6], bvhgpu_ray_f32* out_dev);
void gen_rays_f64(bvhgpu_ctx* ctx, uint64_t first, size_t n, const float bounds[6], bvhgpu_ray_f64* out_dev);

}
```

### bvh_amd/csrc/flatten.hip

```cpp
#include <algorithm>

#include "flatten_node.hpp"

namespace bvhgpu {

template <typename T, int PARTS>
__global__ __launch_bounds__(256) void k_flatten(const typename Traits<T>::Node* __restrict__ nodes,
                                                 const uint32_t* __restrict__ node_start,
                                                 const uint32_t* __restrict__ node_count, const T* __restrict__ aabbs,
                                                 const uint16_t* __restrict__ node_slot, uint32_t* __restrict__ slot_entry,
                                                 typename Traits<T>::Flat* __restrict__ flat, TravNode<T>* __restrict__ trav,
                                                 WideNode<T>* __restrict__ wide, uint32_t* __restrict__ wslot_node,
                                                 uint32_t n_nodes, uint32_t n_shapes, uint32_t* __restrict__ pub_ctr,
                                                 uint32_t* __restrict__ pub_host, uint32_t pub_words, uint32_t* __restrict__ bstat,
                                                 uint32_t flags_idx, uint32_t level_idx, WideNode<float>* __restrict__ guide,
                                                 float* __restrict__ guide_info, uint32_t inline_parts) {
    if (pub_ctr && blockIdx.x == 0) {
        if (bstat) {
            if (threadIdx.x == 0) bstat[0] = pub_ctr[flags_idx] | ((level_idx != flags_idx && pub_ctr[level_idx] != 0u) ? BSTAT_UNFINISHED : 0u);
            __syncthreads();
        }
        for (uint32_t k = threadIdx.x; k < pub_words; k += blockDim.x) { pub_host[k] = pub_ctr[k]; pub_ctr[k] = 0; }
        __threadfence_system();
    }
    const uint32_t i = blockIdx.x * blockDim.x + threadIdx.x;
    if (i >= n_nodes) return;
    if (inline_parts != 0u && node_count[i] <= (uint32_t)SMALL_MAX) {
        if ((PARTS & FLATTEN_WIDE) && wide) {
            const uint32_t h = node_slot[i];
            if (h >= 1u && h < 2048u && ((31 - __clz((int)h)) & 1) == 0) {
                const typename Traits<T>::Node nd = nodes[i];
                if (nd.shape == NONE && nd.l < n_nodes && nd.r < n_nodes) {
                    const int level = 31 - __clz((int)h);
                    wslot_node[wide_level_base(level >> 1) + (h - (1u << level))] = i;
                }
            }
        }
        constexpr int REST = PARTS & FLATTEN_TRAV;
        if (REST != 0 && (PARTS & ~(int)inline_parts) == REST) {
            flatten_node_impl<T, REST>(nodes, node_start, node_count, aabbs, node_slot, slot_entry, flat, trav, wide, wslot_node, guide, guide_info, n_nodes,
                                       n_shapes, i, nodes[i]);
            return;
        }
        if ((PARTS & ~(int)inline_parts) == 0) return;
    }
    flatten_node_impl<T, PARTS>(nodes, node_start, node_count, aabbs, node_slot, slot_entry, flat, trav, wide, wslot_node, guide, guide_info, n_nodes, n_shapes,
                                i, nodes[i]);
}

template <typename T> struct WideSlot { T mn[3], mx[3]; uint32_t ref; };

template <typename T> __device__ __forceinline__ void wide_slot_from_entry(const TravNode<T>* __restrict__ trav, uint32_t e,
                                                                           WideSlot<T>& s) {
    const TravNode<T> g = trav[e];
#pragma unroll
    for (int k = 0; k < 3; k++) { s.mn[k] = g.mn[k]; s.mx[k] = g.mx[k]; }
    s.ref = trav_is_leaf(g.shape) ? g.shape : (WIDE_INNER | (e + 1u));
}
template <typename T> __device__ __forceinline__ void wide_slot_absent(WideSlot<T>& s) {
    const T nan = __builtin_nan("");
#pragma unroll
    for (int k = 0; k < 3; k++) { s.mn[k] = nan; s.mx[k] = nan; }
    s.ref = NONE;
}

template <typename T>
__global__ __launch_bounds__(256) void k_wide(const TravNode<T>* __restrict__ trav, uint32_t n_nodes, uint32_t n_trav,
                                              const uint32_t* __restrict__ slot_entry, uint32_t n_bin_slots,
                                              WideNode<T>* __restrict__ wide, uint32_t* __restrict__ wslot_node,
                                              WideNode<float>* __restrict__ guide, float* __restrict__ guide_info) {
    const uint32_t b = blockIdx.x * blockDim.x + threadIdx.x;
    if (b < WIDE_SLOTS) {
        int k = 0;
        while (k < 5 && wide_level_base(k + 1) <= b) k++;
        const uint32_t h = (1u << (2 * k)) + (b - wide_level_base(k));
        uint32_t node = NONE;
        if (h == 1u) node = 0u;
        else if (h < n_bin_slots) {
            const uint32_t e = slot_entry[h];
            if (e != NONE && e < n_trav && !trav_is_leaf(trav[e].shape)) node = e + 1u;
        }
        wslot_node[b] = node;
    }
    if (b >= n_nodes) return;
    if (b > 0 && trav_is_leaf(trav[b - 1].shape)) return;
    WideSlot<T> s[4];
    uint32_t child = b < n_trav ? b : n_trav - 1u;
#pragma unroll
    for (int side = 0; side < 2; side++) {
        const TravNode<T> c = trav[child];
        if (trav_is_leaf(c.shape) || child + 1u >= n_trav) {
#pragma unroll
            for (int k = 0; k < 3; k++) { s[2 * side].mn[k] = c.mn[k]; s[2 * side].mx[k] = c.mx[k]; }
            s[2 * side].ref = trav_is_leaf(c.shape) ? c.shape : NONE;
            wide_slot_absent<T>(s[2 * side + 1]);
        } else {
            wide_slot_from_entry<T>(trav, child + 1u, s[2 * side]);
            const uint32_t g1 = trav[child + 1u].exit;
            if (g1 < n_trav) wide_slot_from_entry<T>(trav, g1, s[2 * side + 1]); else wide_slot_absent<T>(s[2 * side + 1]);
        }
        child = c.exit < n_trav ? c.exit : n_trav - 1u;
    }
    WideNode<T> w;
#pragma unroll
    for (int c = 0; c < 4; c++) {
#pragma unroll
        for (int k = 0; k < 3; k++) { w.mn[k][c] = s[c].mn[k]; w.mx[k][c] = s[c].mx[k]; }
        w.ref[c] = s[c].ref;
    }
    for (int k = 0; k < (int)(sizeof(w._pad) / 4); k++) w._pad[k] = 0;
    wide[b] = w;
    if (sizeof(T) == 8 && guide && n_trav >= 2u) {
        const TravNode<T> c0 = trav[0];
        const TravNode<T> c1 = trav[c0.exit < n_trav ? c0.exit : n_trav - 1u];
        const double S = guide_scene_extent<T>(c0.mn, c0.mx, c1.mn, c1.mx);
        guide[b] = guide_node(w, GUIDE_GROW * S);
        if (b == 0 && guide_info) guide_info[0] = (float)S;
    }
}

template <typename T> void wide_from_trav(bvhgpu_tree* t) {
    t->has_wide = false; t->has_guide = false;
    if (t->n < 2 || t->n >= WIDE_MAX_SHAPES || t->unfolded || !t->slot_entry.p) return;
    const uint32_t nn = (uint32_t)(t->n_trav + 1);
    t->wide.reserve((size_t)nn * sizeof(WideNode<T>));
    t->wslot_node.reserve(WIDE_SLOTS * 4);
    const bool with_guide = sizeof(T) == 8;
    if (with_guide) { t->wide_guide.reserve((size_t)nn * sizeof(WideNode<float>)); t->guide_info.reserve(16); }
    hipLaunchKernelGGL(k_wide<T>, dim3((std::max(nn, WIDE_SLOTS) + 255) / 256), dim3(256), 0, t->ctx->stream, t->trav.as<TravNode<T>>(),
                       nn, (uint32_t)t->n_trav, t->slot_entry.as<uint32_t>(), (uint32_t)TopCfg<T>::SLOTS, t->wide.as<WideNode<T>>(),
                       t->wslot_node.as<uint32_t>(), with_guide ? t->wide_guide.as<WideNode<float>>() : nullptr,
                       with_guide ? t->guide_info.as<float>() : nullptr);
    BVH_HIP(hipGetLastError());
    t->has_wide = true;
    t->has_guide = with_guide;
}
template void wide_from_trav<float>(bvhgpu_tree*);
template void wide_from_trav<double>(bvhgpu_tree*);

template <typename T> FlattenArgs<T> flatten_args(bvhgpu_tree* t, bool with_wide, bool with_guide) {
    using Tr = Traits<T>;
    FlattenArgs<T> f;
    f.nodes = t->nodes.as<typename Tr::Node>(); f.node_start = t->node_start.as<uint32_t>(); f.node_count = t->node_count.as<uint32_t>();
    f.aabbs = t->aabbs.as<T>(); f.node_slot = t->node_slot.as<uint16_t>(); f.slot_entry = t->slot_entry.as<uint32_t>();
    f.flat = t->flat.as<typename Tr::Flat>(); f.trav = t->trav.as<TravNode<T>>();
    f.wide = with_wide ? t->wide.as<WideNode<T>>() : nullptr; f.wslot_node = t->wslot_node.as<uint32_t>();
    f.guide = with_guide ? t->wide_guide.as<WideNode<float>>() : nullptr; f.guide_info = with_guide ? t->guide_info.as<float>() : nullptr;
    f.n_nodes = (uint32_t)t->n_nodes; f.n_shapes = (uint32_t)t->n;
    return f;
}
template FlattenArgs<float> flatten_args<float>(bvhgpu_tree*, bool, bool);
template FlattenArgs<double> flatten_args<double>(bvhgpu_tree*, bool, bool);

template <typename T> FlattenPlan flatten_plan(bvhgpu_tree* t, bool wide_only) {
    using Tr = Traits<T>;
    FlattenPlan p;
    p.with_wide = t->n >= 2 && t->n < WIDE_MAX_SHAPES && t->wslot_node.p != nullptr;
    p.with_guide = p.with_wide && sizeof(T) == 8;
    const uint32_t nn = (uint32_t)t->n_nodes;
    if (p.with_wide && t->wide.reserve((size_t)nn * sizeof(WideNode<T>))) BVH_HIP(hipMemsetAsync(t->wide.p, 0xFF, t->wide.cap, t->ctx->stream));
    if (p.with_guide) { t->wide_guide.reserve((size_t)nn * sizeof(WideNode<float>)); t->guide_info.reserve(16); }
    if (wide_only && p.with_wide && t->ctx->tune[BVHGPU_TUNE_FLATTEN_LAZY] == 3) p.parts = FLATTEN_FLAT | FLATTEN_WIDE;
    else if (wide_only && p.with_wide) p.parts = FLATTEN_WIDE;
    else p.parts = FLATTEN_FLAT | FLATTEN_TRAV | FLATTEN_WIDE;
    if (p.parts & FLATTEN_FLAT) t->flat.reserve(t->n_flat * sizeof(typename Tr::Flat));
    if (p.parts & FLATTEN_TRAV) t->trav.reserve(t->n_trav * sizeof(TravNode<T>));
    return p;
}
template FlattenPlan flatten_plan<float>(bvhgpu_tree*, bool);
template FlattenPlan flatten_plan<double>(bvhgpu_tree*, bool);

template <typename T, int PARTS> static void launch_flatten(bvhgpu_tree* t, bool with_wide, bool with_guide, uint32_t* pub_ctr, uint32_t* pub_host,
                                                             uint32_t pub_words, uint32_t* bstat, uint32_t flags_idx, uint32_t level_idx,
                                                             hipStream_t st = nullptr, uint32_t inline_parts = 0) {
    const uint32_t nn = (uint32_t)t->n_nodes;
    const FlattenArgs<T> f = flatten_args<T>(t, with_wide, with_guide);
    hipLaunchKernelGGL((k_flatten<T, PARTS>), dim3((nn + 255) / 256), dim3(256), 0, st ? st : t->ctx->stream, f.nodes, f.node_start, f.node_count, f.aabbs,
                       f.node_slot, f.slot_entry, f.flat, f.trav, f.wide, f.wslot_node, nn, (uint32_t)t->n, pub_ctr, pub_host, pub_words, bstat, flags_idx,
                       level_idx, f.guide, f.guide_info, inline_parts);
    BVH_HIP(hipGetLastError());
}

void join_flat(bvhgpu_tree* t) {
    if (!t->flat_beside) return;
    t->flat_beside = false;
    BVH_HIP(hipStreamWaitEvent(t->ctx->stream, t->ev_flat, 0));
}

template <typename T> static void flat_beside(bvhgpu_tree* t) {
    bvhgpu_ctx* ctx = t->ctx;
    if (!ctx->side) BVH_HIP(hipStreamCreateWithFlags(&ctx->side, hipStreamNonBlocking));
    if (!t->ev_flat0) BVH_HIP(hipEventCreateWithFlags(&t->ev_flat0, hipEventDisableTiming));
    if (!t->ev_flat) BVH_HIP(hipEventCreateWithFlags(&t->ev_flat, hipEventDisableTiming));
    t->flat.reserve(t->n_flat * sizeof(typename Traits<T>::Flat));
    t->trav.reserve(t->n_trav * sizeof(TravNode<T>));
    BVH_HIP(hipEventRecord(t->ev_flat0, ctx->stream));
    BVH_HIP(hipStreamWaitEvent(ctx->side, t->ev_flat0, 0));
    launch_flatten<T, FLATTEN_FLAT | FLATTEN_TRAV>(t, false, false, nullptr, nullptr, 0, nullptr, 0, 0, ctx->side);
    BVH_HIP(hipEventRecord(t->ev_flat, ctx->side));
    t->lazy_flat = false;
    t->flat_beside = true;
}

template <typename T> void flatten_tree(bvhgpu_tree* t, uint32_t* pub_ctr, uint32_t* pub_host, uint32_t pub_words, uint32_t* bstat,
                                        uint32_t flags_idx, uint32_t level_idx, bool wide_only, uint32_t inline_parts) {
    join_flat(t);
    t->lazy_flat = false;
    if (t->n == 0) { t->flattened = true; return; }
    const FlattenPlan p = flatten_plan<T>(t, wide_only);
    const bool with_wide = p.with_wide, with_guide = p.with_guide;
    if (p.parts == (FLATTEN_FLAT | FLATTEN_WIDE)) {
        launch_flatten<T, FLATTEN_FLAT | FLATTEN_WIDE>(t, true, with_guide, pub_ctr, pub_host, pub_words, bstat, flags_idx, level_idx, nullptr, inline_parts);
        t->lazy_flat = true; t->lazy_parts = FLATTEN_TRAV;
    } else if (p.parts == FLATTEN_WIDE) {
        launch_flatten<T, FLATTEN_WIDE>(t, true, with_guide, pub_ctr, pub_host, pub_words, bstat, flags_idx, level_idx, nullptr, inline_parts);
        t->lazy_flat = true; t->lazy_parts = FLATTEN_FLAT | FLATTEN_TRAV;
        if (t->ctx->tune[BVHGPU_TUNE_FLATTEN_LAZY] == 2) flat_beside<T>(t);
    } else {
        launch_flatten<T, FLATTEN_FLAT | FLATTEN_TRAV | FLATTEN_WIDE>(t, with_wide, with_guide, pub_ctr, pub_host, pub_words, bstat, flags_idx, level_idx, nullptr, inline_parts);
    }
    t->has_wide = with_wide;
    t->has_guide = with_guide;
    t->flattened = true;
}

void ensure_flat_arrays(bvhgpu_tree* t) {
    join_flat(t);
    if (!t->lazy_flat) return;
    t->lazy_flat = false;
    const bool trav_only = t->lazy_parts == FLATTEN_TRAV;
    if (t->dtype == BVHGPU_F32) {
        t->flat.reserve(t->n_flat * sizeof(Traits<float>::Flat));
        t->trav.reserve(t->n_trav * sizeof(TravNode<float>));
        if (trav_only) launch_flatten<float, FLATTEN_TRAV>(t, false, false, nullptr, nullptr, 0, nullptr, 0, 0);
        else launch_flatten<float, FLATTEN_FLAT | FLATTEN_TRAV>(t, false, false, nullptr, nullptr, 0, nullptr, 0, 0);
    } else {
        t->flat.reserve(t->n_flat * sizeof(Traits<double>::Flat));
        t->trav.reserve(t->n_trav * sizeof(TravNode<double>));
        if (trav_only) launch_flatten<double, FLATTEN_TRAV>(t, false, false, nullptr, nullptr, 0, nullptr, 0, 0);
        else launch_flatten<double, FLATTEN_FLAT | FLATTEN_TRAV>(t, false, false, nullptr, nullptr, 0, nullptr, 0, 0);
    }
}

template void flatten_tree<float>(bvhgpu_tree*, uint32_t*, uint32_t*, uint32_t, uint32_t*, uint32_t, uint32_t, bool, uint32_t);
template void flatten_tree<double>(bvhgpu_tree*, uint32_t*, uint32_t*, uint32_t, uint32_t*, uint32_t, uint32_t, bool, uint32_t);

}
```

### bvh_amd/csrc/refit.hip

```cpp
#include "engine.hpp"

namespace bvhgpu {

constexpr uint32_t SEG_GROUP = 1024;

template <typename T>
__global__ __launch_bounds__(256) void k_refit_leaves(const T* __restrict__ new_aabbs, const uint32_t* __restrict__ shape_node,
                                                      const uint32_t* __restrict__ node_start, T* __restrict__ tree_aabbs,
                                                      T* __restrict__ seg, uint32_t n, uint32_t n_pad) {
    const uint32_t s = blockIdx.x * blockDim.x + threadIdx.x;
    if (s >= n_pad) return;
    if (s < n) {
        const uint32_t pos = node_start[shape_node[s]];
        T b[6];
#pragma unroll
        for (int k = 0; k < 6; k++) b[k] = new_aabbs[6 * (size_t)s + k];
#pragma unroll
        for (int k = 0; k < 6; k++) seg[6 * ((size_t)n_pad + pos) + k] = b[k];
        if (tree_aabbs) {
#pragma unroll
            for (int k = 0; k < 6; k++) tree_aabbs[6 * (size_t)s + k] = b[k];
        }
    } else {
#pragma unroll
        for (int k = 0; k < 6; k++) seg[6 * ((size_t)n_pad + s) + k] = k < 3 ? Traits<T>::inf() : -Traits<T>::inf();
    }
}

template <typename T>
__global__ __launch_bounds__(256) void k_refit_segs(T* __restrict__ seg, uint32_t lv, uint32_t group, int levels) {
    __shared__ T s_box[SEG_GROUP * 6];
    const uint32_t b = blockIdx.x, tid = threadIdx.x;
    const T* src = seg + 6 * ((size_t)lv + (size_t)b * group);
    for (uint32_t e = tid; e < group * 6; e += 256) s_box[e] = src[e];
    __syncthreads();
    for (int d = 1; d <= levels; d++) {
        const uint32_t cnt = group >> d;
        T out[(SEG_GROUP / 2 / 256) > 0 ? (SEG_GROUP / 2 / 256) : 1][6];
        int m = 0;
        for (uint32_t j = tid; j < cnt; j += 256, m++) {
#pragma unroll
            for (int k = 0; k < 3; k++) {
                out[m][k] = join_min(s_box[6 * (2 * j) + k], s_box[6 * (2 * j + 1) + k]);
                out[m][3 + k] = join_max(s_box[6 * (2 * j) + 3 + k], s_box[6 * (2 * j + 1) + 3 + k]);
            }
        }
        __syncthreads();
        T* dst = seg + 6 * ((size_t)(lv >> d) + (size_t)b * cnt);
        m = 0;
        for (uint32_t j = tid; j < cnt; j += 256, m++) {
#pragma unroll
            for (int k = 0; k < 6; k++) { s_box[6 * j + k] = out[m][k]; dst[6 * (size_t)j + k] = out[m][k]; }
        }
        __syncthreads();
    }
}

template <typename T>
__device__ __forceinline__ void seg_query(const T* __restrict__ seg, uint32_t n_pad, uint32_t l, uint32_t r, T out[6]) {
#pragma unroll
    for (int k = 0; k < 6; k++) out[k] = k < 3 ? Traits<T>::inf() : -Traits<T>::inf();
    l += n_pad; r += n_pad;
    while (l < r) {
        if (l & 1u) {
            const T* p = seg + 6 * (size_t)l;
#pragma unroll
            for (int k = 0; k < 3; k++) { out[k] = join_min(out[k], p[k]); out[3 + k] = join_max(out[3 + k], p[3 + k]); }
            l++;
        }
        if (r & 1u) {
            r--;
            const T* p = seg + 6 * (size_t)r;
#pragma unroll
            for (int k = 0; k < 3; k++) { out[k] = join_min(out[k], p[k]); out[3 + k] = join_max(out[3 + k], p[3 + k]); }
        }
        l >>= 1; r >>= 1;
    }
}

template <typename T>
__global__ __launch_bounds__(256) void k_refit_nodes(typename Traits<T>::Node* __restrict__ nodes,
                                                     const uint32_t* __restrict__ node_start,
                                                     const uint32_t* __restrict__ node_count, const T* __restrict__ seg,
                                                     uint32_t n_pad, uint32_t n_nodes) {
    const uint32_t i = blockIdx.x * blockDim.x + threadIdx.x;
    if (i >= n_nodes) return;
    typename Traits<T>::Node* nd = nodes + i;
    if (nd->shape != NONE) return;
    const uint32_t s = node_start[i], c = node_count[i];
    const uint32_t nl = node_count[nd->l];
    T lb[6], rb[6];
    seg_query<T>(seg, n_pad, s, s + nl, lb);
    seg_query<T>(seg, n_pad, s + nl, s + c, rb);
#pragma unroll
    for (int k = 0; k < 3; k++) {
        nd->l_min[k] = lb[k]; nd->l_max[k] = lb[3 + k];
        nd->r_min[k] = rb[k]; nd->r_max[k] = rb[3 + k];
    }
}

template <typename T>
__global__ __launch_bounds__(256) void k_refit_check(const T* __restrict__ aabbs, size_t count, uint32_t* __restrict__ flag) {
    bool bad = false;
    for (size_t i = (size_t)blockIdx.x * blockDim.x + threadIdx.x; i < count; i += (size_t)gridDim.x * blockDim.x)
        bad = bad || !(fabs(aabbs[i]) < Traits<T>::inf());
    if (__any(bad) && lane_id() == 0) atomicOr(flag, 1u);
}

template <typename T> bool refit_input_ok(bvhgpu_tree* t, const T* aabbs_dev) {
    if (t->n < 2) return true;
    bvhgpu_ctx* ctx = t->ctx;
    hipStream_t st = ctx->stream;
    ctx->counters.reserve(64);
    uint32_t* flag = ctx->counters.as<uint32_t>();
    BVH_HIP(hipMemsetAsync(flag, 0, sizeof(uint32_t), st));
    const size_t count = 6 * t->n;
    const uint32_t grid = (uint32_t)std::min<size_t>((count + 255) / 256, 2048);
    hipLaunchKernelGGL(k_refit_check<T>, dim3(grid), dim3(256), 0, st, aabbs_dev, count, flag);
    BVH_HIP(hipGetLastError());
    uint32_t* host = static_cast<uint32_t*>(ctx->pinned);
    BVH_HIP(hipMemcpyAsync(host, flag, sizeof(uint32_t), hipMemcpyDeviceToHost, st));
    BVH_HIP(hipStreamSynchronize(st));
    return *host == 0u;
}

template bool refit_input_ok<float>(bvhgpu_tree*, const float*);
template bool refit_input_ok<double>(bvhgpu_tree*, const double*);

template <typename T> void refit_tree(bvhgpu_tree* t, const T* aabbs_dev) {
    using Tr = Traits<T>;
    const size_t n = t->n;
    if (n == 0) return;
    hipStream_t st = t->ctx->stream;
    if (t->ctx->timing) { BVH_HIP(hipEventRecord(t->ctx->ev[0], st)); }
    if (n == 1) {
        if (aabbs_dev != t->aabbs.as<T>()) BVH_HIP(hipMemcpyAsync(t->aabbs.p, aabbs_dev, 6 * sizeof(T), hipMemcpyDeviceToDevice, st));
        if (t->ctx->timing) { BVH_HIP(hipEventRecord(t->ctx->ev[1], st)); t->ctx->ev_set |= 1u; }
        if (t->flattened) flatten_tree<T>(t, nullptr, nullptr, 0, nullptr, 0, 0, t->ctx->tune[BVHGPU_TUNE_FLATTEN_LAZY] != 0);
        return;
    }
    uint32_t n_pad = 1;
    while (n_pad < n) n_pad <<= 1;
    t->refit_seg.reserve((size_t)2 * n_pad * 6 * sizeof(T));
    T* seg = t->refit_seg.as<T>();
    hipLaunchKernelGGL(k_refit_leaves<T>, dim3((n_pad + 255) / 256), dim3(256), 0, st, aabbs_dev, t->shape_node.as<uint32_t>(),
                       t->node_start.as<uint32_t>(), aabbs_dev == t->aabbs.as<T>() ? nullptr : t->aabbs.as<T>(), seg, (uint32_t)n, n_pad);
    for (uint32_t lv = n_pad; lv > 1;) {
        const uint32_t group = std::min<uint32_t>(SEG_GROUP, lv);
        int levels = 0;
        while ((1u << levels) < group) levels++;
        hipLaunchKernelGGL(k_refit_segs<T>, dim3(lv / group), dim3(256), 0, st, seg, lv, group, levels);
        lv /= group;
    }
    const uint32_t nn = (uint32_t)t->n_nodes;
    hipLaunchKernelGGL(k_refit_nodes<T>, dim3((nn + 255) / 256), dim3(256), 0, st, t->nodes.as<typename Tr::Node>(),
                       t->node_start.as<uint32_t>(), t->node_count.as<uint32_t>(), seg, n_pad, nn);
    BVH_HIP(hipGetLastError());
    if (t->ctx->timing) { BVH_HIP(hipEventRecord(t->ctx->ev[1], st)); t->ctx->ev_set |= 1u; }
    t->exact_only = false;
    if (t->flattened) flatten_tree<T>(t, nullptr, nullptr, 0, nullptr, 0, 0, t->ctx->tune[BVHGPU_TUNE_FLATTEN_LAZY] != 0);
}

template void refit_tree<float>(bvhgpu_tree*, const float*);
template void refit_tree<double>(bvhgpu_tree*, const double*);

}
```

### bvh_amd/csrc/walk.hpp

```cpp
#pragma once

#include "engine.hpp"

namespace bvhgpu {

constexpr int SCAN_ITEMS = 4;
constexpr int SCAN_BLOCK = 256 * SCAN_ITEMS;
constexpr uint32_t SCAN_FUSED_MAX_BLOCKS = 2048;
constexpr int COUNT_PLAIN = 0, COUNT_PAIR = 1, COUNT_MASKED = 2;
constexpr uint32_t WIDE_ITEM_BITS = 5;
constexpr uint32_t WIDE_BSUM_MAX = 128;
constexpr size_t WIDE_ITEM_MAX_RAYS = (size_t)1 << 27;
constexpr unsigned long long WALK_FLAG_GUIDE_RANGE = 16ull;
constexpr uint32_t HEAP_OVERFLOW_BIT = 2u;

enum : int {
    MODE_INDICES = 0,
    MODE_T_SLICE = 1,
    MODE_TRIANGLES = 2,
    MODE_CLOSEST = 3,
    MODE_ANY = 4,
    MODE_BOX_CLOSEST = 5,
    MODE_BOX_FIRST = 6,
    MODE_SPHERE_CLOSEST = 7,
    MODE_SPHERE_FIRST = 8
};
constexpr bool mode_tris(int m) { return m >= MODE_TRIANGLES && m <= MODE_ANY; }
constexpr bool mode_box(int m) { return m == MODE_BOX_CLOSEST || m == MODE_BOX_FIRST; }
constexpr bool mode_sphere(int m) { return m == MODE_SPHERE_CLOSEST || m == MODE_SPHERE_FIRST; }
constexpr bool mode_first(int m) { return m == MODE_ANY || m == MODE_BOX_FIRST || m == MODE_SPHERE_FIRST; }
constexpr bool mode_tmax(int m) { return m == MODE_ANY || mode_box(m) || mode_sphere(m); }
constexpr bool mode_pair(int m) { return mode_box(m) || mode_sphere(m); }
template <int MODE> struct ModeVals { static constexpr int N = MODE == MODE_T_SLICE ? 2 : (MODE == MODE_TRIANGLES ? 3 : 0); };

template <typename T> struct NodeRegs { T mn[3], mx[3]; uint32_t exit, shape; };

__device__ __forceinline__ NodeRegs<float> load_node(const TravNode<float>* p) {
    const float4* q = reinterpret_cast<const float4*>(p);
    float4 a = q[0], b = q[1];
    NodeRegs<float> r;
    r.mn[0] = a.x; r.mn[1] = a.y; r.mn[2] = a.z; r.exit = __float_as_uint(a.w);
    r.mx[0] = b.x; r.mx[1] = b.y; r.mx[2] = b.z; r.shape = __float_as_uint(b.w);
    return r;
}
__device__ __forceinline__ NodeRegs<double> load_node(const TravNode<double>* p) {
    const double2* q = reinterpret_cast<const double2*>(p);
    double2 a = q[0], b = q[1], c = q[2], d = q[3];
    NodeRegs<double> r;
    r.mn[0] = a.x; r.mn[1] = a.y; r.mn[2] = b.x;
    r.mx[0] = b.y; r.mx[1] = c.x; r.mx[2] = c.y;
    unsigned long long es = (unsigned long long)__double_as_longlong(d.x);
    r.exit = (uint32_t)(es & 0xFFFFFFFFull);
    r.shape = (uint32_t)(es >> 32);
    return r;
}

struct HitRec { uint32_t ray, k, shape; };

template <typename T> struct WalkOut {
    uint32_t* counts;
    HitRec* pool;
    T* pool_v;
    unsigned long long pool_cap;
    unsigned long long* ctr;
    const T* tris;
    T* closest;
    uint32_t* closest_prim;
    unsigned long long* closest_key;
    uint32_t* item_cnt;
    uint32_t* ray_items;
    uint32_t* scan_sums;
    uint4* pool_pair;
    uint32_t* raybuf;
    uint32_t stage_shift;
    const T* tmax;
    uint32_t* any_key;
    __host__ __device__ __forceinline__ const T* box(uint32_t s) const { return tris + 6 * (size_t)s; }
    __host__ __device__ __forceinline__ void set_boxes(const T* aabbs) { tris = aabbs; }
    __host__ __device__ __forceinline__ const T* sphere(uint32_t s) const { return tris + 4 * (size_t)s; }
    __host__ __device__ __forceinline__ void set_spheres(const T* spheres) { tris = spheres; }
};

template <typename T> __device__ __forceinline__ void cross3(const T a[3], const T b[3], T out[3]) {
    T p0 = a[1] * b[2], q0 = a[2] * b[1];
    T p1 = a[2] * b[0], q1 = a[0] * b[2];
    T p2 = a[0] * b[1], q2 = a[1] * b[0];
    out[0] = p0 - q0; out[1] = p1 - q1; out[2] = p2 - q2;
}
template <typename T> __device__ __forceinline__ T dot3(const T a[3], const T b[3]) {
    T x = a[0] * b[0], y = a[1] * b[1], z = a[2] * b[2];
    T s = x + y;
    return s + z;
}
template <typename T>
__device__ __forceinline__ void ray_triangle(const T o[3], const T d[3], const T* __restrict__ tri, T out[3]) {
    const T a[3] = {tri[0], tri[1], tri[2]};
    T ab[3], ac[3], uvec[3], ao[3], vvec[3];
#pragma unroll
    for (int k = 0; k < 3; k++) { ab[k] = tri[3 + k] - a[k]; ac[k] = tri[6 + k] - a[k]; }
    cross3<T>(d, ac, uvec);
    const T det = dot3<T>(ab, uvec);
    out[0] = Traits<T>::inf(); out[1] = 0; out[2] = 0;
    if (det < Traits<T>::eps()) return;
    const T inv_det = (T)1 / det;
#pragma unroll
    for (int k = 0; k < 3; k++) ao[k] = o[k] - a[k];
    const T u = dot3<T>(ao, uvec) * inv_det;
    out[1] = u;
    if (!(u >= (T)0 && u <= (T)1)) return;
    cross3<T>(ao, ab, vvec);
    const T v = dot3<T>(d, vvec) * inv_det;
    out[2] = v;
    if (v < (T)0 || u + v > (T)1) return;
    const T dist = dot3<T>(ac, vvec) * inv_det;
    if (dist > Traits<T>::eps()) out[0] = dist;
}

__device__ __forceinline__ void load_sphere(const float* __restrict__ p, float s[4]) {
    const float4 v = *reinterpret_cast<const float4*>(p);
    s[0] = v.x; s[1] = v.y; s[2] = v.z; s[3] = v.w;
}
__device__ __forceinline__ void load_sphere(const double* __restrict__ p, double s[4]) {
    const double2 a = reinterpret_cast<const double2*>(p)[0], b = reinterpret_cast<const double2*>(p)[1];
    s[0] = a.x; s[1] = a.y; s[2] = b.x; s[3] = b.y;
}
template <typename T>
__device__ __forceinline__ void ray_sphere(const T o[3], const T d[3], const T* __restrict__ sphere, T out[2]) {
    T s[4], f[3], l[3];
    load_sphere(sphere, s);
#pragma unroll
    for (int k = 0; k < 3; k++) f[k] = o[k] - s[k];
    const T a = dot3<T>(d, d);
    const T tc = (-dot3<T>(f, d)) / a;
#pragma unroll
    for (int k = 0; k < 3; k++) { const T td = tc * d[k]; l[k] = f[k] + td; }
    const T rr = s[3] * s[3];
    const T disc = rr - dot3<T>(l, l);
    out[0] = Traits<T>::inf(); out[1] = 0;
    if (!(disc >= (T)0)) return;
    const T h = sqrt(disc / a);
    const T t0 = tc - h, t1 = tc + h;
    const T t = t0 > Traits<T>::eps() ? t0 : t1;
    if (t > Traits<T>::eps()) { out[0] = t; out[1] = t1; }
}

template <typename T, int MODE> struct LaneRay {
    T o[3], inv[3];
    T d[mode_tris(MODE) || mode_sphere(MODE) ? 3 : 1];
    T best[MODE >= MODE_CLOSEST ? 3 : 1];
    T tmax;
    uint32_t best_prim;
    uint32_t r, cnt;
    bool fin;
    __device__ __forceinline__ void clear() {
#pragma unroll
        for (int k = 0; k < 3; k++) { o[k] = 0; inv[k] = 0; }
        d[0] = 0; best[0] = 0; tmax = 0; best_prim = NONE; r = NONE; cnt = 0; fin = true;
    }
    __device__ __forceinline__ void load(const typename Traits<T>::Ray* __restrict__ rays, uint32_t ray, const T* __restrict__ tmaxs = nullptr) {
        const typename Traits<T>::Ray* rp = rays + ray;
#pragma unroll
        for (int k = 0; k < 3; k++) { o[k] = rp->o[k]; inv[k] = rp->inv[k]; }
        if (mode_tris(MODE) || mode_sphere(MODE)) {
#pragma unroll
            for (int k = 0; k < 3; k++) d[k] = rp->d[k];
        }
        if (MODE >= MODE_CLOSEST) { best[0] = Traits<T>::inf(); best[1] = 0; best[2] = 0; }
        if (mode_tmax(MODE)) tmax = tmaxs ? tmaxs[ray] : Traits<T>::inf();
        best_prim = NONE; r = ray; cnt = 0;
        fin = ray_is_finite<T>(o, inv);
    }
    __device__ __forceinline__ void loaded(uint32_t ray) {
        best_prim = NONE; r = ray; cnt = 0;
        fin = ray_is_finite<T>(o, inv);
    }
    __device__ __forceinline__ void retire(const WalkOut<T>& w) {
        if (mode_pair(MODE)) {
            w.closest[2 * (size_t)r] = best[0]; w.closest[2 * (size_t)r + 1] = best[1];
            w.closest_prim[r] = best_prim;
        } else if (MODE >= MODE_CLOSEST) {
            w.closest[3 * (size_t)r] = best[0]; w.closest[3 * (size_t)r + 1] = best[1]; w.closest[3 * (size_t)r + 2] = best[2];
            w.closest_prim[r] = best_prim;
        } else {
            w.counts[r] = cnt;
        }
        r = NONE;
    }
};

constexpr uint32_t POOL_CHUNK_MIN = 64;
constexpr uint32_t POOL_CHUNK_MAX = 8192;
struct PoolCursor { unsigned long long pos = 0; uint32_t left = 0; uint32_t next = POOL_CHUNK_MIN; };

__device__ __forceinline__ void pool_invalidate_tail(HitRec* pool, unsigned long long pool_cap, const PoolCursor& pc, int lane) {
    for (uint32_t j = (uint32_t)lane; j < pc.left; j += WAVE)
        if (pc.pos + j < pool_cap) pool[pc.pos + j].ray = NONE;
}

template <typename T, int MODE>
__device__ __forceinline__ void report(bool rec, uint32_t shape, T t0, T t1, LaneRay<T, MODE>& ray, const WalkOut<T>& w,
                                       PoolCursor& pc, int lane, unsigned long long lt) {
    const unsigned long long m = __ballot(rec);
    if (!m) return;
    T vals[3] = {t0, t1, 0};
    if (mode_tris(MODE) && rec) ray_triangle<T>(ray.o, ray.d, w.tris + 9 * (size_t)shape, vals);
    if (MODE == MODE_CLOSEST) {
        if (rec) {
            if (vals[0] < ray.best[0]) { ray.best[0] = vals[0]; ray.best[1] = vals[1]; ray.best[2] = vals[2]; ray.best_prim = shape; }
            ray.cnt++;
        }
        return;
    }
    if (MODE == MODE_ANY) {
        if (rec && vals[0] < ray.tmax) { ray.best[0] = vals[0]; ray.best[1] = vals[1]; ray.best[2] = vals[2]; ray.best_prim = shape; }
        return;
    }
    if (mode_box(MODE)) {
        if (rec && t0 < ray.tmax && (MODE == MODE_BOX_FIRST || t0 < ray.best[0])) { ray.best[0] = t0; ray.best[1] = t1; ray.best_prim = shape; }
        return;
    }
    if (mode_sphere(MODE)) {
        if (rec) {
            T hit[2];
            ray_sphere<T>(ray.o, ray.d, w.sphere(shape), hit);
            if (hit[0] < ray.tmax && (MODE == MODE_SPHERE_FIRST || hit[0] < ray.best[0])) { ray.best[0] = hit[0]; ray.best[1] = hit[1]; ray.best_prim = shape; }
        }
        return;
    }
    constexpr int NV = ModeVals<MODE>::N;
    const uint32_t h = (uint32_t)__popcll(m);
    if (h > pc.left) {
        pool_invalidate_tail(w.pool, w.pool_cap, pc, lane);
        unsigned int blo = 0, bhi = 0;
        if (lane == 0) {
            unsigned long long b = atomicAdd(&w.ctr[0], (unsigned long long)pc.next);
            blo = (unsigned int)b; bhi = (unsigned int)(b >> 32);
        }
        blo = __builtin_amdgcn_readfirstlane(blo); bhi = __builtin_amdgcn_readfirstlane(bhi);
        pc.pos = ((unsigned long long)bhi << 32) | blo;
        pc.left = pc.next;
        pc.next = pc.next < POOL_CHUNK_MAX ? pc.next * 2 : POOL_CHUNK_MAX;
    }
    if (rec) {
        const unsigned long long slot = pc.pos + __popcll(m & lt);
        if (slot < w.pool_cap) {
            HitRec hr; hr.ray = ray.r; hr.k = ray.cnt; hr.shape = shape;
            w.pool[slot] = hr;
#pragma unroll
            for (int k = 0; k < NV; k++) w.pool_v[NV * slot + k] = vals[k];
        }
        ray.cnt++;
    }
    pc.pos += h; pc.left -= h;
}

struct __attribute__((packed, aligned(4))) DwordPair { uint32_t a, b; };
#ifndef SCATTER8_UNROLL
#define SCATTER8_UNROLL 16
#endif
__device__ __forceinline__ void pool_invalidate_tail16(uint4* pool, unsigned long long pool_cap, const PoolCursor& pc, int lane) {
    for (uint32_t j = (uint32_t)lane; j < pc.left; j += WAVE)
        if (pc.pos + j < pool_cap) pool[pc.pos + j].x = NONE;
}
template <typename RAY>
__device__ __forceinline__ void report_pair(bool rec, bool flush, uint32_t shape, RAY& ray, uint32_t& pend, uint4* pool, unsigned long long pool_cap,
                                            unsigned long long* ctr, PoolCursor& pc, int lane, unsigned long long lt) {
    const bool emit = (rec || flush) && pend != NONE;
    const unsigned long long m = __ballot(emit);
    if (m) {
        const uint32_t h = (uint32_t)__popcll(m);
        if (h > pc.left) {
            pool_invalidate_tail16(pool, pool_cap, pc, lane);
            unsigned int blo = 0, bhi = 0;
            if (lane == 0) {
                unsigned long long b = atomicAdd(&ctr[0], (unsigned long long)pc.next);
                blo = (unsigned int)b; bhi = (unsigned int)(b >> 32);
            }
            blo = __builtin_amdgcn_readfirstlane(blo); bhi = __builtin_amdgcn_readfirstlane(bhi);
            pc.pos = ((unsigned long long)bhi << 32) | blo;
            pc.left = pc.next;
            pc.next = pc.next < POOL_CHUNK_MAX ? pc.next * 2 : POOL_CHUNK_MAX;
        }
        if (emit) {
            const unsigned long long slot = pc.pos + __popcll(m & lt);
            if (slot < pool_cap) pool[slot] = make_uint4(ray.r, ray.cnt - 1u, pend, rec ? shape : NONE);
        }
        pc.pos += h; pc.left -= h;
    }
    if (rec) { pend = emit ? NONE : shape; ray.cnt++; }
    else if (emit) pend = NONE;
}

template <typename T, int MODE>
__device__ __forceinline__ void walk_epilogue(const WalkOut<T>& w, PoolCursor& pc, int lane, bool stats,
                                              unsigned long long steps, unsigned long long leaf_steps,
                                              unsigned long long wsteps, unsigned long long cands) {
    if (MODE < MODE_CLOSEST) pool_invalidate_tail(w.pool, w.pool_cap, pc, lane);
    if (stats) {
#pragma unroll
        for (int d = 32; d > 0; d >>= 1) {
            steps += __shfl_down(steps, d);
            leaf_steps += __shfl_down(leaf_steps, d);
            cands += __shfl_down(cands, d);
        }
        if (lane == 0) {
            atomicAdd(&w.ctr[1], steps); atomicAdd(&w.ctr[2], leaf_steps); atomicAdd(&w.ctr[4], wsteps);
            if (MODE == MODE_CLOSEST) atomicAdd(&w.ctr[5], cands);
        }
    }
}

template <typename T> struct WideRegs { T mn[3][4], mx[3][4]; uint32_t ref[4]; };
template <typename T> struct WideIo {
    static constexpr int CHUNKS = (int)(sizeof(WideRegs<T>) / 16);
    static_assert(sizeof(WideRegs<T>) % 16 == 0, "wide regs");
    static __device__ __forceinline__ WideRegs<T> from_global(const WideNode<T>* __restrict__ p) {
        const uint4* q = reinterpret_cast<const uint4*>(p);
        uint4 c[CHUNKS];
#pragma unroll
        for (int j = 0; j < CHUNKS; j++) c[j] = q[j];
        WideRegs<T> r;
        __builtin_memcpy(&r, c, sizeof r);
        return r;
    }
    static __device__ __forceinline__ WideRegs<T> from_lds(const uint4* nodes, uint32_t slot) {
        const uint4* q = nodes + __umul24(slot, (uint32_t)CHUNKS);
        uint4 c[CHUNKS];
#pragma unroll
        for (int j = 0; j < CHUNKS; j++) c[j] = q[j];
        WideRegs<T> r;
        __builtin_memcpy(&r, c, sizeof r);
        return r;
    }
};

template <typename T> inline const char* walk_type_name() { return sizeof(T) == 4 ? "float" : "double"; }
template <typename T>
void launch_binary(bvhgpu_tree* t, const typename Traits<T>::Ray* rays_dev, size_t n_rays, const WalkOut<T>& w, bvhgpu_hits* h, int mode, bool stats,
                   bool use_lds, uint32_t split_at);
template <typename T>
void launch_ordered(bvhgpu_tree* t, const typename Traits<T>::Ray* rays_dev, size_t n_rays, const WalkOut<T>& w, bvhgpu_hits* h, int mode, bool ascending,
                    bool best_first, uint32_t* ovf_flag);
template <typename T>
void launch_wide_walk(bvhgpu_tree* t, const typename Traits<T>::Ray* rays_dev, size_t n_rays, const WalkOut<T>& w, bvhgpu_hits* h, int mode, int items_log4,
                      bool use_guide, bool early_items, uint32_t* ovf_flag);
template <typename T> size_t wide_walk_grid(const bvhgpu_ctx* ctx, size_t n_rays, int items_log4, bool coherent, bool use_guide);
struct CsrArgs {
    int count_kind;
    int nv;
    int items_log4;
    int stage_shift;
    bool rec8;
    uint32_t nb;
    unsigned long long cap;
    unsigned long long *ctr_other, *pin;
    uint32_t* bsum_other;
};
template <typename T> void csr_enqueue(bvhgpu_hits* h, size_t n_rays, const WalkOut<T>& w, const CsrArgs& a);
void publish_counters(hipStream_t st, unsigned long long* ctr, unsigned long long* host_page);

}
```

### bvh_amd/csrc/walk_wide.hip

```cpp
#include <cstdio>

#include "walk.hpp"

namespace bvhgpu {

constexpr uint32_t CUR_NONE = 0x7FFFFFFFu;
#ifndef BVH_WIDE_INNER_STEPS
#define BVH_WIDE_INNER_STEPS 4
#endif
#ifndef BVH_WIDE_INNER_STEPS_WHOLE
#define BVH_WIDE_INNER_STEPS_WHOLE 8
#endif
#ifndef BVH_WIDE_INNER_STEPS_COHERENT
#define BVH_WIDE_INNER_STEPS_COHERENT 12
#endif
#ifndef BVH_WIDE_MIN_WAVES_F32
#define BVH_WIDE_MIN_WAVES_F32 8
#endif
#ifndef BVH_WIDE_MIN_WAVES_F64
#define BVH_WIDE_MIN_WAVES_F64 4
#endif
constexpr uint32_t WIDE_ITEM_WHOLE = 16;


__device__ __forceinline__ uint32_t wide_resident_ref(uint32_t ref, uint32_t q, uint32_t c, uint32_t K) {
    const uint32_t cs = 4u * q + 1u + c;
    return (ref != NONE && (ref & WIDE_INNER) && cs < K) ? (WIDE_INNER | WIDE_RESIDENT | cs) : ref;
}

template <typename T, bool EXACT>
__device__ __forceinline__ uint32_t wide_hits(const T o[3], const T inv[3], const WideRegs<T>& nd) {
    uint32_t m = 0;
    if (!EXACT) {
#pragma unroll
        for (int c = 0; c < 4; c++) {
            const T mn[3] = {nd.mn[0][c], nd.mn[1][c], nd.mn[2][c]}, mx[3] = {nd.mx[0][c], nd.mx[1][c], nd.mx[2][c]};
            m |= slab_hit_finite<T>(o, inv, mn, mx) ? (1u << c) : 0u;
        }
        return m;
    }
#pragma unroll
    for (int p = 0; p < 2; p++) {
        const int c0 = 2 * p, c1 = 2 * p + 1;
        const T mn0[3] = {nd.mn[0][c0], nd.mn[1][c0], nd.mn[2][c0]}, mx0[3] = {nd.mx[0][c0], nd.mx[1][c0], nd.mx[2][c0]};
        T t0, t1;
        if (nd.ref[c1] == NONE) {
            if (nd.ref[c0] != NONE && slab_hit<T>(o, inv, mn0, mx0, t0, t1)) m |= 1u << c0;
        } else {
            const T mn1[3] = {nd.mn[0][c1], nd.mn[1][c1], nd.mn[2][c1]}, mx1[3] = {nd.mx[0][c1], nd.mx[1][c1], nd.mx[2][c1]};
            T jmn[3], jmx[3];
#pragma unroll
            for (int k = 0; k < 3; k++) { jmn[k] = tmin(mn0[k], mn1[k]); jmx[k] = tmax(mx0[k], mx1[k]); }
            if (slab_hit<T>(o, inv, jmn, jmx, t0, t1)) {
                if (slab_hit<T>(o, inv, mn0, mx0, t0, t1)) m |= 1u << c0;
                if (slab_hit<T>(o, inv, mn1, mx1, t0, t1)) m |= 1u << c1;
            }
        }
    }
    return m;
}

#ifndef BVH_WIDE_LONG_FRAC
#define BVH_WIDE_LONG_FRAC 0.2
#endif
template <typename T> struct ItemTable {
    T box[16][6];
    uint32_t ref[16];
    T half_diag[16];
};
template <typename T, int ITEMS_LOG4>
__device__ __forceinline__ void item_table_build(const WideNode<T>* __restrict__ wide, ItemTable<T>* tb, uint32_t tid) {
    constexpr uint32_t ITEMS = 1u << (2 * ITEMS_LOG4);
    if (tid < ITEMS) {
        const uint32_t c = ITEMS_LOG4 == 2 ? tid >> 2 : tid, k = tid & 3u;
        const WideNode<T>* root = wide;
        uint32_t ref = root->ref[c];
        T b[6];
#pragma unroll
        for (int a = 0; a < 3; a++) { b[a] = root->mn[a][c]; b[3 + a] = root->mx[a][c]; }
        if (ITEMS_LOG4 == 2) {
            if (ref != NONE && (ref & WIDE_INNER)) {
                const WideNode<T>* g = wide + (ref & (WIDE_RESIDENT - 1u));
                ref = g->ref[k];
#pragma unroll
                for (int a = 0; a < 3; a++) { b[a] = g->mn[a][k]; b[3 + a] = g->mx[a][k]; }
            } else if (k != 0) {
                ref = NONE;
            }
        }
        if (ref == NONE) {
            const T nan = __builtin_nan("");
#pragma unroll
            for (int a = 0; a < 6; a++) b[a] = nan;
        }
#pragma unroll
        for (int a = 0; a < 6; a++) tb->box[tid][a] = b[a];
        tb->ref[tid] = ref;
        const T dx = b[3] - b[0], dy = b[4] - b[1], dz = b[5] - b[2];
        tb->half_diag[tid] = (T)BVH_WIDE_LONG_FRAC * sqrt(dx * dx + dy * dy + dz * dz);
    }
}
template <int ITEMS_LOG4> __device__ __forceinline__ uint32_t item_slot(uint32_t j) {
    return ITEMS_LOG4 == 2 ? 5u + j : 1u + j;
}

struct GuideArgs;
__device__ __forceinline__ void guide_ray_load(const bvhgpu_ray_f64* __restrict__ rays64, uint32_t r, double S, float o[3], float inv[3], bool& bad);
template <typename T, int L4, bool GUIDE = false>
__device__ __forceinline__ void filter_rays_into_list(const ItemTable<T>* tb, const typename Traits<T>::Ray* __restrict__ rays, uint32_t n_rays,
                                                      uint32_t* __restrict__ list, uint32_t per_wg, uint32_t my_rays, uint32_t G, uint32_t b,
                                                      uint32_t tid, uint32_t bd, int lane, uint32_t* s_nlist, uint32_t* s_nback,
                                                      const bvhgpu_ray_f64* __restrict__ rays64 = nullptr, double guide_S = 0.0, bool* any_bad = nullptr) {
    constexpr uint32_t ITEMS = 1u << (2 * L4);
    for (uint32_t l0 = 0; l0 < my_rays; l0 += bd) {
        const uint32_t local = l0 + tid;
        const uint32_t r = local < my_rays ? ((((local >> 6) * G + b) << 6) | (local & 63u)) : n_rays;
        uint32_t mask = 0, longm = 0;
        if (r < n_rays) {
            T o[3], inv[3];
            if constexpr (GUIDE) {
                bool bad;
                guide_ray_load(rays64, r, guide_S, o, inv, bad);
                *any_bad = *any_bad || bad;
            } else {
                const typename Traits<T>::Ray* rp = rays + r;
#pragma unroll
                for (int k = 0; k < 3; k++) { o[k] = rp->o[k]; inv[k] = rp->inv[k]; }
            }
            if (!ray_is_finite<T>(o, inv)) {
                mask = 1u << WIDE_ITEM_WHOLE; longm = mask;
            } else {
#pragma unroll 4
                for (uint32_t j = 0; j < ITEMS; j++) {
                    const T mn[3] = {tb->box[j][0], tb->box[j][1], tb->box[j][2]}, mx[3] = {tb->box[j][3], tb->box[j][4], tb->box[j][5]};
                    T len;
                    const bool hit = slab_hit_finite_len<T>(o, inv, mn, mx, len);
                    mask |= hit ? (1u << j) : 0u;
                    longm |= (hit && len > tb->half_diag[j]) ? (1u << j) : 0u;
                }
            }
        }
        const uint32_t cap = per_wg * ITEMS;
#pragma unroll
        for (int side = 0; side < 2; side++) {
            const uint32_t mm0 = side ? (mask & ~longm) : (mask & longm);
            const uint32_t mine = (uint32_t)__popc(mm0);
            uint32_t incl = mine;
#pragma unroll
            for (int d = 1; d < WAVE; d <<= 1) {
                const uint32_t u = __shfl_up(incl, d);
                if (lane >= d) incl += u;
            }
            const uint32_t total = __shfl(incl, WAVE - 1);
            uint32_t base = 0;
            if (lane == 0 && total) base = atomicAdd(side ? s_nback : s_nlist, total);
            base = __shfl(base, 0) + incl - mine;
            uint32_t mm = mm0;
            while (mm) {
                const uint32_t bit = (uint32_t)__ffs(mm) - 1u;
                mm &= mm - 1u;
                list[side ? cap - 1u - base : base] = (r << WIDE_ITEM_BITS) | bit;
                base++;
            }
        }
    }
}

template <typename T>
__global__ __launch_bounds__(256) void k_wide_items(const typename Traits<T>::Node* __restrict__ nodes, uint32_t n_nodes,
                                                    const uint32_t* __restrict__ node_count, const uint32_t* __restrict__ build_ctr,
                                                    const typename Traits<T>::Ray* __restrict__ rays, uint32_t n_rays,
                                                    uint32_t* __restrict__ list_all, uint32_t* __restrict__ wg_items) {
    constexpr int L4 = 2;
    constexpr uint32_t ITEMS = 16;
    __shared__ ItemTable<T> tb;
    __shared__ uint32_t s_nlist, s_nback, s_bad;
    const uint32_t tid = threadIdx.x, bd = blockDim.x;
    const int lane = lane_id();
    if (tid == 0) { s_nlist = 0u; s_nback = 0u; s_bad = (build_ctr[BUILD_CTR_TOPMASK] & 0xFFFEu) == 0xFFFEu ? 0u : 1u; }
    __syncthreads();
    if (s_bad) { if (tid == 0) wg_items[2u * blockIdx.x] = NONE; return; }
    if (tid < ITEMS) {
        uint32_t node = 0;
        T bx[6];
        bool ok = n_nodes > 1u;
        uint32_t cnt = ok ? node_count[0] : 0u;
#pragma unroll
        for (int lv = 3; lv >= 0 && ok; lv--) {
            const typename Traits<T>::Node nd = nodes[node];
            const uint32_t right = ((16u + tid) >> lv) & 1u;
            ok = nd.shape == NONE && nd.l < n_nodes && nd.r < n_nodes && nd.r > nd.l;
            if (!ok) break;
            const uint32_t nl = (nd.r - nd.l + 1u) >> 1;
            cnt = right ? cnt - nl : nl;
            node = right ? nd.r : nd.l;
#pragma unroll
            for (int k = 0; k < 3; k++) { bx[k] = right ? nd.r_min[k] : nd.l_min[k]; bx[3 + k] = right ? nd.r_max[k] : nd.l_max[k]; }
        }
        ok = ok && cnt > 1u;
        if (!ok) atomicOr(&s_bad, 1u);
#pragma unroll
        for (int k = 0; k < 6; k++) tb.box[tid][k] = bx[k];
        const T dx = bx[3] - bx[0], dy = bx[4] - bx[1], dz = bx[5] - bx[2];
        tb.half_diag[tid] = (T)BVH_WIDE_LONG_FRAC * sqrt(dx * dx + dy * dy + dz * dz);
    }
    __syncthreads();
    if (s_bad) { if (tid == 0) wg_items[2u * blockIdx.x] = NONE; return; }
    const uint32_t n_blocks = (n_rays + 63u) >> 6;
    const uint32_t my_blocks = n_blocks > blockIdx.x ? (n_blocks - blockIdx.x + gridDim.x - 1u) / gridDim.x : 0u;
    const uint32_t per_wg = ((n_blocks + gridDim.x - 1u) / gridDim.x) << 6;
    uint32_t* list = list_all + (size_t)blockIdx.x * per_wg * ITEMS;
    filter_rays_into_list<T, L4>(&tb, rays, n_rays, list, per_wg, my_blocks << 6, gridDim.x, blockIdx.x, tid, bd, lane, &s_nlist, &s_nback);
    __syncthreads();
    if (tid == 0) { wg_items[2u * blockIdx.x] = s_nlist; wg_items[2u * blockIdx.x + 1u] = s_nback; }
}

struct GuideArgs { const bvhgpu_ray_f64* rays64; const double* aabbs64; const float* info; const double* tris64; };
__device__ __forceinline__ void guide_ray_load(const bvhgpu_ray_f64* __restrict__ rays64, uint32_t r, double S, float o[3], float inv[3], bool& bad) {
    const bvhgpu_ray_f64* q = rays64 + r;
    bad = !(S >= GUIDE_SCENE_MIN) || !(S <= GUIDE_SCENE_MAX);
#pragma unroll
    for (int k = 0; k < 3; k++) {
        const double ok = q->o[k], ik = q->inv[k];
        const double ao = fabs(ok), ainv = fabs(ik), ai = ainv * (4.0 * S);
        bad = bad || !(ao <= GUIDE_ORIGIN_MAX * S) || !(ao <= GUIDE_F32_MAX) || !(ai <= 0x1p100) || !(ai >= 0x1p-100) ||
              !(ainv <= GUIDE_F32_MAX) || !(ainv >= GUIDE_F32_MIN_NORMAL);
        o[k] = (float)ok; inv[k] = (float)ik;
    }
}
__device__ __forceinline__ bool guide_leaf_hit(const GuideArgs& ga, uint32_t ray, uint32_t shape) {
    const bvhgpu_ray_f64* rp = ga.rays64 + ray;
    const double* b = ga.aabbs64 + 6 * (size_t)shape;
    const double o[3] = {rp->o[0], rp->o[1], rp->o[2]}, inv[3] = {rp->inv[0], rp->inv[1], rp->inv[2]};
    const double mn[3] = {b[0], b[1], b[2]}, mx[3] = {b[3], b[4], b[5]};
    return slab_hit_finite<double>(o, inv, mn, mx);
}

#ifndef BVH_GUIDE_CANDIDATE_ATTR
#define BVH_GUIDE_CANDIDATE_ATTR __forceinline__
#endif
__device__ BVH_GUIDE_CANDIDATE_ATTR double guide_candidate_distance(const bvhgpu_ray_f64* __restrict__ rays64, const double* __restrict__ tris64, uint32_t ray, uint32_t shape) {
    const bvhgpu_ray_f64* rp = rays64 + ray;
    const double o[3] = {rp->o[0], rp->o[1], rp->o[2]}, d[3] = {rp->d[0], rp->d[1], rp->d[2]};
    double out[3];
    ray_triangle<double>(o, d, tris64 + 9 * (size_t)shape, out);
    return out[0];
}

#ifdef BVH_WIDE_PROFILE
__device__ unsigned long long g_wide_prof[4 * 16384];
__device__ unsigned long long g_wide_util[16 * 16384];
#endif
template <typename T, int MODE, int ITEMS_LOG4, int MAX_THREADS, int MIN_WAVES, int GUIDE = 0>
__global__ __launch_bounds__(MAX_THREADS, MIN_WAVES) void k_traverse_wide(
    const WideNode<T>* __restrict__ wide, const uint32_t* __restrict__ wslot_node, uint32_t K, uint32_t stack_lds,
    const typename Traits<T>::Ray* __restrict__ rays, uint32_t n_rays, uint32_t* __restrict__ list_all, const uint32_t* __restrict__ wg_items,
    WalkOut<T> w, uint32_t* __restrict__ gstack, uint32_t gstack_cap, uint32_t* __restrict__ overflow, GuideArgs ga, uint32_t whole_steps) {
    static_assert(GUIDE == 0 || ((MODE == MODE_INDICES || MODE == MODE_CLOSEST) && sizeof(T) == 4), "the guide walk is the f32 walk of an f64 index / closest-hit batch");
    constexpr bool GUIDE_CLOSEST = GUIDE != 0 && MODE == MODE_CLOSEST;
    double gbest = 0.0;
    static_assert(ITEMS_LOG4 >= 0 && ITEMS_LOG4 <= 2, "1, 4 or 16 items per ray");
    static_assert(MODE != MODE_T_SLICE, "the t-slice output walks the binary array");
    constexpr int CH = WideIo<T>::CHUNKS;
    constexpr int L4 = ITEMS_LOG4 > 0 ? ITEMS_LOG4 : 1;
    constexpr uint32_t ITEMS = 1u << (2 * L4);
    extern __shared__ __attribute__((aligned(16))) uint4 wsmem[];
    uint32_t& s_next = *reinterpret_cast<uint32_t*>(wsmem);
    uint32_t& s_nlist = *(reinterpret_cast<uint32_t*>(wsmem) + 1);
    uint32_t& s_nback = *(reinterpret_cast<uint32_t*>(wsmem) + 2);
    uint32_t* s_item_ref = reinterpret_cast<uint32_t*>(wsmem + 1);
    uint4* nodes = wsmem + 5;
    uint32_t* s_stack = reinterpret_cast<uint32_t*>(nodes + (size_t)CH * K);
    const uint32_t bd = blockDim.x, tid = threadIdx.x;
    const int WIDE_INNER_STEPS = ITEMS_LOG4 == 0 ? (int)whole_steps : BVH_WIDE_INNER_STEPS;
    constexpr uint32_t SB = MAX_THREADS;
    const size_t G = (size_t)gridDim.x * bd, gid = (size_t)blockIdx.x * bd + tid;
    const int lane = lane_id();
    const unsigned long long lt = lanemask_lt();
    double guide_S = 0.0;
    bool guide_bad = false;
    if constexpr (GUIDE != 0) guide_S = (double)ga.info[0];
#ifdef BVH_WIDE_PROFILE
    const unsigned long long prof_t0 = wall_clock64();
    unsigned long long prof_steps = 0;
    unsigned long long pu[16];
    for (int i = 0; i < 16; i++) pu[i] = 0;
    uint32_t pl_boxes = 0, pl_nohit = 0;
#endif
    const uint32_t n_blocks = (n_rays + 63u) >> 6;
    const uint32_t my_blocks = n_blocks > blockIdx.x ? (n_blocks - blockIdx.x + gridDim.x - 1u) / gridDim.x : 0u;
    const uint32_t per_wg = ((n_blocks + gridDim.x - 1u) / gridDim.x) << 6;
    const uint32_t my_rays = my_blocks << 6;
    auto ray_of = [&](uint32_t local) -> uint32_t { return (((local >> 6) * gridDim.x + blockIdx.x) << 6) | (local & 63u); };
    __shared__ uint32_t s_bsum[WIDE_BSUM_MAX];
    if (w.scan_sums) for (uint32_t b = tid; b < WIDE_BSUM_MAX; b += bd) s_bsum[b] = 0u;
    if (tid == 0) { s_next = 0u; s_nlist = 0u; s_nback = 0u; }
    for (uint32_t q = tid; q < K; q += bd) {
        const uint32_t node = wslot_node[q];
        if (node != NONE) {
            const uint4* src = reinterpret_cast<const uint4*>(wide + node);
            uint4* dst = nodes + (size_t)q * CH;
#pragma unroll
            for (int c = 0; c < CH - 1; c++) dst[c] = src[c];
            uint4 rf = src[CH - 1];
            rf.x = wide_resident_ref(rf.x, q, 0u, K); rf.y = wide_resident_ref(rf.y, q, 1u, K);
            rf.z = wide_resident_ref(rf.z, q, 2u, K); rf.w = wide_resident_ref(rf.w, q, 3u, K);
            dst[CH - 1] = rf;
        }
    }
    uint32_t* list = nullptr;
    if (ITEMS_LOG4 > 0) {
        __shared__ ItemTable<T> tb;
        item_table_build<T, L4>(wide, &tb, tid);
        __syncthreads();
        if (tid < ITEMS) {
            const uint32_t ref = tb.ref[tid], slot = item_slot<L4>(tid);
            s_item_ref[tid] = (ref != NONE && (ref & WIDE_INNER) && slot < K) ? (WIDE_INNER | WIDE_RESIDENT | slot) : ref;
        }
        list = list_all + (size_t)blockIdx.x * per_wg * ITEMS;
        const uint32_t pre_front = wg_items ? wg_items[2u * blockIdx.x] : NONE;
        if (pre_front != NONE) {
            if (tid == 0) { s_nlist = pre_front; s_nback = wg_items[2u * blockIdx.x + 1u]; }
        } else {
            if constexpr (GUIDE != 0) filter_rays_into_list<T, L4, true>(&tb, rays, n_rays, list, per_wg, my_rays, gridDim.x, blockIdx.x, tid, bd, lane, &s_nlist, &s_nback,
                                                                            ga.rays64, guide_S, &guide_bad);
            else filter_rays_into_list<T, L4>(&tb, rays, n_rays, list, per_wg, my_rays, gridDim.x, blockIdx.x, tid, bd, lane, &s_nlist, &s_nback);
        }
        __threadfence_block();
    }
    __syncthreads();
    const uint32_t wg_begin = 0u;
    const uint32_t n_front = s_nlist;
    const uint32_t wg_end = ITEMS_LOG4 == 0 ? my_rays : n_front + s_nback;
#ifdef BVH_WIDE_PROFILE
    const unsigned long long prof_t1 = wall_clock64();
#endif

    LaneRay<T, MODE> ray;
    ray.clear();
    uint32_t cur = CUR_NONE, sp = 0, item = NONE;
    bool exhausted = wg_begin >= wg_end;
    bool ovf = false;
    uint32_t pair_pend = NONE;
    PoolCursor pc;
    auto push_slow = [&](uint32_t v) {
        if (sp < stack_lds) s_stack[sp * SB + tid] = v;
        else if (sp - stack_lds < gstack_cap) gstack[(size_t)(sp - stack_lds) * G + gid] = v;
        else ovf = true;
        sp++;
    };
    auto pop_or_none = [&]() -> uint32_t {
        if (sp == 0) return CUR_NONE;
        sp--;
        if (sp < stack_lds) return s_stack[sp * SB + tid];
        return sp - stack_lds < gstack_cap ? gstack[(size_t)(sp - stack_lds) * G + gid] : CUR_NONE;
    };
    while (true) {
        bool run = cur != CUR_NONE;
        const unsigned long long idle = __ballot(!run);
        if (idle) {
            if (MODE == MODE_INDICES && ITEMS_LOG4 == 0 && w.pool_pair)
                report_pair(false, !run && item != NONE, 0u, ray, pair_pend, w.pool_pair, w.pool_cap, w.ctr, pc, lane, lt);
            if (!run && item != NONE) {
                if (mode_first(MODE)) {
                    if constexpr (ITEMS_LOG4 == 0) {
                        const size_t r = item;
                        if constexpr (mode_pair(MODE)) { w.closest[2 * r] = ray.best[0]; w.closest[2 * r + 1] = ray.best[1]; }
                        else { w.closest[3 * r] = ray.best[0]; w.closest[3 * r + 1] = ray.best[1]; w.closest[3 * r + 2] = ray.best[2]; }
                        w.closest_prim[r] = ray.best_prim;
                    } else if (ray.best_prim != NONE) {
                        const uint32_t j = item & ((1u << WIDE_ITEM_BITS) - 1u);
                        const uint32_t jj = j == WIDE_ITEM_WHOLE ? 0u : j;
                        atomicMin(&w.any_key[item >> WIDE_ITEM_BITS], (jj << 28) | ray.best_prim);
                    }
                } else if (MODE == MODE_CLOSEST || MODE == MODE_BOX_CLOSEST || MODE == MODE_SPHERE_CLOSEST) {
                    if constexpr (ITEMS_LOG4 == 0) {
                        const size_t r = item;
                        if constexpr (mode_pair(MODE)) { w.closest[2 * r] = ray.best[0]; w.closest[2 * r + 1] = ray.best[1]; }
                        else if constexpr (!GUIDE_CLOSEST) { w.closest[3 * r] = ray.best[0]; w.closest[3 * r + 1] = ray.best[1]; w.closest[3 * r + 2] = ray.best[2]; }
                        w.closest_prim[r] = ray.best_prim;
                    } else if (ray.best_prim != NONE) {
                        const uint32_t j = item & ((1u << WIDE_ITEM_BITS) - 1u);
                        const uint32_t jj = j == WIDE_ITEM_WHOLE ? 0u : j;
                        if constexpr (sizeof(T) == 4 && !GUIDE_CLOSEST) {
                            const unsigned long long key = ((unsigned long long)Traits<T>::key(ray.best[0]) << 32) | ((unsigned long long)jj << 28) | (unsigned long long)ray.best_prim;
                            atomicMin(&w.closest_key[item >> WIDE_ITEM_BITS], key);
                        } else {
                            const size_t r = item >> WIDE_ITEM_BITS;
                            w.item_cnt[(r << (2 * ITEMS_LOG4)) + jj] = ray.best_prim;
                            atomicOr(&w.ray_items[r], 1u << jj);
                        }
                    }
                } else if (ray.cnt) {
                    uint32_t r = item;
                    if (ITEMS_LOG4 == 0) {
                        w.counts[item] = ray.cnt;
                    } else {
                        const uint32_t j = item & ((1u << WIDE_ITEM_BITS) - 1u);
                        const uint32_t jj = j == WIDE_ITEM_WHOLE ? 0u : j;
                        r = item >> WIDE_ITEM_BITS;
                        atomicAdd(&w.counts[r], ray.cnt);
                        atomicOr(&w.ray_items[r], 1u << jj);
                        w.item_cnt[((size_t)r << (2 * ITEMS_LOG4)) + jj] = ray.cnt;
                    }
                    if (w.scan_sums) atomicAdd(&s_bsum[((r >> 6) - blockIdx.x) / gridDim.x], ray.cnt);
                }
                item = NONE;
            }
            if (!exhausted) {
                const uint32_t nidle = (uint32_t)__popcll(idle);
                uint32_t base = 0;
                if (lane == 0) base = atomicAdd(&s_next, nidle);
                base = __builtin_amdgcn_readfirstlane(base);
                const uint32_t mine = base + (uint32_t)__popcll(idle & lt);
                if (!run && base < wg_end && mine < wg_end) {
                    if (ITEMS_LOG4 == 0) {
                        item = ray_of(mine);
                        if (item < n_rays) {
                            if constexpr (GUIDE != 0) { bool bad; guide_ray_load(ga.rays64, item, guide_S, ray.o, ray.inv, bad); guide_bad = guide_bad || bad; ray.loaded(item); gbest = __builtin_inf(); }
                            else ray.load(rays, item, w.tmax);
                            cur = WIDE_INNER | WIDE_RESIDENT | 0u;
                        } else {
                            item = NONE;
                        }
                    } else {
                        item = list[mine < n_front ? mine : per_wg * ITEMS - 1u - (mine - n_front)];
                        const uint32_t j = item & ((1u << WIDE_ITEM_BITS) - 1u);
                        if constexpr (GUIDE != 0) { bool bad; guide_ray_load(ga.rays64, item >> WIDE_ITEM_BITS, guide_S, ray.o, ray.inv, bad); ray.loaded(item >> WIDE_ITEM_BITS); gbest = __builtin_inf(); }
                        else ray.load(rays, item >> WIDE_ITEM_BITS, w.tmax);
                        cur = j == WIDE_ITEM_WHOLE ? (WIDE_INNER | WIDE_RESIDENT | 0u) : s_item_ref[j];
                        if (j == WIDE_ITEM_WHOLE) item = item & ~((1u << WIDE_ITEM_BITS) - 1u);
                    }
                    ray.r = item;
                    sp = 0;
                    run = cur != CUR_NONE;
                }
                exhausted = base >= wg_end || (wg_end - base) <= nidle;
            }
            if (!__any(run)) break;
        }
        const bool fast = !__any(run && !ray.fin);
#ifdef BVH_WIDE_PROFILE
        prof_steps += WIDE_INNER_STEPS;
        pu[9]++; pu[10] += fast ? 0 : 1;
        pu[8] += WIDE_INNER_STEPS * (unsigned long long)__popcll(__ballot(run));
#endif
        for (int s = 0; s < WIDE_INNER_STEPS; s++) {
#ifdef BVH_WIDE_PROFILE
            {
                const bool in = (cur & WIDE_INNER) != 0u;
                pu[0]++; pu[1] += __popcll(__ballot(in));
                pu[2] += __any(in && (cur & WIDE_RESIDENT)) ? 1 : 0;
                pu[3] += __any(in && !(cur & WIDE_RESIDENT)) ? 1 : 0;
                const bool slow = in && sp + 3u > stack_lds;
                pu[4] += __any(slow) ? 1 : 0; pu[5] += __popcll(__ballot(slow));
                const bool lf = !in && cur < CUR_NONE;
                pu[6] += __popcll(__ballot(lf)); pu[7] += __any(lf) ? 1 : 0;
                pu[11] += __any((in || lf) && sp > stack_lds) ? 1 : 0;
            }
#endif
            if (cur & WIDE_INNER) {
                const uint32_t id = cur & (WIDE_RESIDENT - 1u);
                WideRegs<T> nd;
                if (cur & WIDE_RESIDENT) nd = WideIo<T>::from_lds(nodes, id);
                else nd = WideIo<T>::from_global(wide + id);
                const uint32_t m = fast ? wide_hits<T, false>(ray.o, ray.inv, nd) : wide_hits<T, true>(ray.o, ray.inv, nd);
                const uint32_t first = m & (0u - m);
                const uint32_t rest = m ^ first;
#ifdef BVH_WIDE_PROFILE
                pl_boxes += (uint32_t)__popc(m); pl_nohit += m == 0u ? 1u : 0u;
#endif
                const uint32_t s0 = (rest & 8u) ? nd.ref[3] : ((rest & 4u) ? nd.ref[2] : nd.ref[1]);
                const uint32_t s1 = ((rest & 12u) == 12u) ? nd.ref[2] : nd.ref[1];
                if (sp + 3u <= stack_lds) {
                    uint32_t* at = s_stack + sp * SB + tid;
                    at[0] = s0; at[SB] = s1; at[2 * SB] = nd.ref[1];
                    sp += (uint32_t)__popc(rest);
                } else {
                    if (rest & 8u) push_slow(nd.ref[3]);
                    if (rest & 4u) push_slow(nd.ref[2]);
                    if (rest & 2u) push_slow(nd.ref[1]);
                }
                cur = first == 0u ? pop_or_none() : (first == 1u ? nd.ref[0] : (first == 2u ? nd.ref[1] : (first == 4u ? nd.ref[2] : nd.ref[3])));
            }
            bool rec = cur < CUR_NONE;
            const uint32_t shape = cur;
            if (rec) cur = pop_or_none();
            if (GUIDE) {
                if (__any(rec)) {
                    if (rec) rec = guide_leaf_hit(ga, ITEMS_LOG4 == 0 ? ray.r : (ray.r >> WIDE_ITEM_BITS), shape);
                }
            }
            if (MODE == MODE_INDICES && ITEMS_LOG4 == 0 && w.raybuf) {
                if (rec && (ray.cnt >> w.stage_shift) == 0u) {
                    w.raybuf[((size_t)ray.r << w.stage_shift) | ray.cnt] = shape;
                    ray.cnt++;
                    rec = false;
                }
            }
            T t0 = 0, t1 = 0;
            if constexpr (mode_box(MODE)) {
                if (rec) {
                    const T* b = w.box(shape);
                    const T mn[3] = {b[0], b[1], b[2]}, mx[3] = {b[3], b[4], b[5]};
                    slab_hit<T>(ray.o, ray.inv, mn, mx, t0, t1);
                }
            }
            if constexpr (GUIDE_CLOSEST) {
                if (__any(rec)) {
                    if (rec) {
                        const double dist = guide_candidate_distance(ga.rays64, ga.tris64, ITEMS_LOG4 == 0 ? ray.r : (ray.r >> WIDE_ITEM_BITS), shape);
                        if (dist < gbest) { gbest = dist; ray.best_prim = shape; }
                        ray.cnt++;
                    }
                }
            } else if (MODE == MODE_INDICES && ITEMS_LOG4 == 0 && w.pool_pair) report_pair(rec, false, shape, ray, pair_pend, w.pool_pair, w.pool_cap, w.ctr, pc, lane, lt);
            else report<T, MODE>(rec, shape, t0, t1, ray, w, pc, lane, lt);
            if (mode_first(MODE) && ray.best_prim != NONE) { cur = CUR_NONE; sp = 0; }
        }
        if (ovf) { cur = CUR_NONE; sp = 0; }
    }
    if (__any(ovf) && lane == 0) atomicOr(overflow, 4u);
    if constexpr (GUIDE != 0) { if (__any(guide_bad) && lane == 0) atomicOr(overflow, (uint32_t)WALK_FLAG_GUIDE_RANGE); }
    if (MODE == MODE_INDICES && ITEMS_LOG4 == 0 && w.pool_pair) {
        pool_invalidate_tail16(w.pool_pair, w.pool_cap, pc, lane);
        pc.left = 0;
    }
    walk_epilogue<T, MODE>(w, pc, lane, false, 0, 0, 0, 0);
    if (MODE < MODE_CLOSEST && w.scan_sums) {
        __syncthreads();
        for (uint32_t b = tid; b < my_blocks; b += bd)
            if (s_bsum[b]) atomicAdd(&w.scan_sums[(b * gridDim.x + blockIdx.x) / (uint32_t)(SCAN_BLOCK / 64)], s_bsum[b]);
    }
#ifdef BVH_WIDE_PROFILE
    if (lane == 0) {
        const size_t wv = gid >> 6;
        if (wv < 16384) {
            g_wide_prof[4 * wv] = prof_t0; g_wide_prof[4 * wv + 1] = prof_t1; g_wide_prof[4 * wv + 2] = wall_clock64(); g_wide_prof[4 * wv + 3] = prof_steps;
            for (int i = 0; i < 12; i++) g_wide_util[16 * wv + i] = pu[i];
            g_wide_util[16 * wv + 12] = 0; g_wide_util[16 * wv + 13] = 0;
        }
    }
    __syncthreads();
    if ((gid >> 6) < 16384) { atomicAdd(&g_wide_util[16 * (gid >> 6) + 12], (unsigned long long)pl_boxes); atomicAdd(&g_wide_util[16 * (gid >> 6) + 13], (unsigned long long)pl_nohit); }
#endif
}

template <typename T> struct WideGeom {
    uint32_t threads, wg_per_cu, stack_lds, K;
    size_t lds_bytes;
    WideGeom(const bvhgpu_ctx* ctx, bool whole_rays, bool coherent = false) {
        const bool f64 = sizeof(T) == 8;
        const int want_threads = ctx->tune[BVHGPU_TUNE_WIDE_THREADS] > 0 ? ctx->tune[BVHGPU_TUNE_WIDE_THREADS] : (f64 ? 512 : 1024);
        threads = (uint32_t)std::min(f64 ? 512 : 1024, std::max(64, want_threads & ~63));
        wg_per_cu = (uint32_t)std::max(1, std::min(ctx->tune[BVHGPU_TUNE_WIDE_WG_PER_CU] > 0 ? ctx->tune[BVHGPU_TUNE_WIDE_WG_PER_CU] : 2,
                                                   (int)(2048 / threads)));
        stack_lds = (uint32_t)std::max(0, std::min(ctx->tune[BVHGPU_TUNE_WIDE_STACK_LDS] >= 0 ? ctx->tune[BVHGPU_TUNE_WIDE_STACK_LDS] : (whole_rays ? (coherent ? 10 : 8) : 6), 32));
        const size_t budget = (size_t)(160 * 1024) / wg_per_cu - (f64 ? 1536 : 1024);
        const size_t stack_stride = f64 ? 512 : 1024;
        const size_t fixed = 80 + (size_t)stack_lds * stack_stride * 4;
        const size_t per_slot = (size_t)WideIo<T>::CHUNKS * 16;
        size_t k = budget > fixed + per_slot ? (budget - fixed) / per_slot : 1;
        if (ctx->tune[BVHGPU_TUNE_WIDE_SLOTS] > 0) k = std::min<size_t>(k, (size_t)ctx->tune[BVHGPU_TUNE_WIDE_SLOTS]);
        K = (uint32_t)std::max<size_t>(1, std::min<size_t>(k, WIDE_SLOTS));
        lds_bytes = 80 + (size_t)K * per_slot + (size_t)stack_lds * stack_stride * 4;
    }
};
inline size_t wide_grid(const bvhgpu_ctx* ctx, uint32_t threads, uint32_t wg_per_cu, size_t n_rays, int items_log4) {
    const size_t slots = (size_t)ctx->n_cu * wg_per_cu;
    size_t per_wg = threads;
    const int min_rays = ctx->tune[BVHGPU_TUNE_WIDE_MIN_RAYS_PER_WG];
    if (items_log4 == 2 && min_rays > 0 && n_rays * 4 <= slots * threads) {
        const size_t spread = ((n_rays + slots - 1) / slots + 63) & ~(size_t)63;
        per_wg = std::min<size_t>(threads, std::max<size_t>(spread, (size_t)std::max(64, min_rays & ~63)));
    }
    const size_t full = (n_rays + per_wg - 1) / per_wg;
    return std::min<size_t>(std::max<size_t>(full, 1), slots);
}
constexpr uint32_t WIDE_GSTACK = 24;

template <typename T, int MODE, int ITEMS_LOG4, int GUIDE = 0>
static void launch_wide(bvhgpu_tree* t, const typename Traits<T>::Ray* rays_dev, size_t n_rays, const WalkOut<T>& w, bvhgpu_hits* h,
                        uint32_t* ovf_flag, bool early_items, GuideArgs ga = GuideArgs{nullptr, nullptr, nullptr, nullptr}) {
    bvhgpu_ctx* ctx = t->ctx;
    hipStream_t st = ctx->stream;
    const WideGeom<T> g(ctx, ITEMS_LOG4 == 0, (h->flags & BVHGPU_TRAVERSE_COHERENT) != 0);
    const dim3 grid((unsigned)wide_grid(ctx, g.threads, g.wg_per_cu, n_rays, ITEMS_LOG4));
    uint32_t* list = nullptr;
    if (ITEMS_LOG4 > 0) {
        const size_t n_blocks = (n_rays + 63) / 64;
        const size_t per_wg = ((n_blocks + grid.x - 1) / grid.x) * 64;
        h->witems.reserve(((size_t)grid.x * per_wg << (2 * ITEMS_LOG4)) * 4 + 16);
        list = h->witems.as<uint32_t>();
    }
    const uint32_t* wg_items = nullptr;
    if (ITEMS_LOG4 == 2 && early_items) {
        if (!ctx->side) BVH_HIP(hipStreamCreateWithFlags(&ctx->side, hipStreamNonBlocking));
        if (!h->ev_items) BVH_HIP(hipEventCreateWithFlags(&h->ev_items, hipEventDisableTiming));
        h->wg_items.reserve((size_t)grid.x * 2 * 4 + 16);
        BVH_HIP(hipStreamWaitEvent(ctx->side, t->ev_top, 0));
        hipLaunchKernelGGL(k_wide_items<T>, grid, dim3(256), 0, ctx->side, t->nodes.as<typename Traits<T>::Node>(), (uint32_t)t->n_nodes,
                           t->node_count.as<uint32_t>(), t->ctr.as<uint32_t>(), rays_dev, (uint32_t)n_rays, list, h->wg_items.as<uint32_t>());
        BVH_HIP(hipEventRecord(h->ev_items, ctx->side));
        BVH_HIP(hipStreamWaitEvent(st, h->ev_items, 0));
        wg_items = h->wg_items.as<uint32_t>();
    }
    const size_t lanes = (size_t)grid.x * g.threads;
    h->wstack.reserve(lanes * WIDE_GSTACK * 4);
    constexpr int MAXT = sizeof(T) == 8 ? 512 : 1024;
    constexpr int MINW = sizeof(T) == 8 ? BVH_WIDE_MIN_WAVES_F64 : BVH_WIDE_MIN_WAVES_F32;
    auto kern = &k_traverse_wide<T, MODE, ITEMS_LOG4, MAXT, MINW, GUIDE>;
    char name[128];
    std::snprintf(name, sizeof name, "bvhgpu::k_traverse_wide<%s, %d, %d, %d, %d, %d>", walk_type_name<T>(), MODE, ITEMS_LOG4, MAXT, MINW, GUIDE);
    static thread_local size_t lds_attr[16] = {};
    size_t& have = lds_attr[ctx->device & 15];
    if (have < g.lds_bytes) {
        BVH_HIP(hipFuncSetAttribute(reinterpret_cast<const void*>(kern), hipFuncAttributeMaxDynamicSharedMemorySize, (int)g.lds_bytes));
        have = g.lds_bytes;
    }
    hipLaunchKernelGGL(kern, grid, dim3(g.threads), g.lds_bytes, st, GUIDE ? t->wide_guide.as<WideNode<T>>() : t->wide.as<WideNode<T>>(),
                       t->wslot_node.as<uint32_t>(), g.K, g.stack_lds, rays_dev, (uint32_t)n_rays, list, wg_items, w, h->wstack.as<uint32_t>(),
                       WIDE_GSTACK, ovf_flag, ga,
                       (uint32_t)((h->flags & BVHGPU_TRAVERSE_COHERENT) ? BVH_WIDE_INNER_STEPS_COHERENT : BVH_WIDE_INNER_STEPS_WHOLE));
    h->walk_kernel = name;
}

template <typename T, int MODE, int GUIDE = 0>
static void launch_wide_items(bvhgpu_tree* t, const typename Traits<T>::Ray* rays_dev, size_t n_rays, const WalkOut<T>& w, bvhgpu_hits* h, int items_log4,
                              uint32_t* ovf_flag, bool early_items, GuideArgs ga = GuideArgs{nullptr, nullptr, nullptr, nullptr}) {
    if (items_log4 == 2) { launch_wide<T, MODE, 2, GUIDE>(t, rays_dev, n_rays, w, h, ovf_flag, early_items, ga); return; }
    if constexpr (MODE < MODE_CLOSEST) {
        if (items_log4 == 1) { launch_wide<T, MODE, 1, GUIDE>(t, rays_dev, n_rays, w, h, ovf_flag, false, ga); return; }
    }
    launch_wide<T, MODE, 0, GUIDE>(t, rays_dev, n_rays, w, h, ovf_flag, false, ga);
}

template <typename T>
void launch_wide_walk(bvhgpu_tree* t, const typename Traits<T>::Ray* rays_dev, size_t n_rays, const WalkOut<T>& w, bvhgpu_hits* h, int mode, int items_log4,
                      bool use_guide, bool early_items, uint32_t* ovf_flag) {
    if constexpr (sizeof(T) == 8) {
        if (use_guide) {
            WalkOut<float> wg{};
            wg.counts = w.counts; wg.pool = w.pool; wg.pool_cap = w.pool_cap; wg.ctr = w.ctr; wg.closest_prim = w.closest_prim;
            wg.item_cnt = w.item_cnt; wg.ray_items = w.ray_items; wg.scan_sums = w.scan_sums;
            wg.pool_pair = w.pool_pair; wg.raybuf = w.raybuf; wg.stage_shift = w.stage_shift;
            const GuideArgs ga{reinterpret_cast<const bvhgpu_ray_f64*>(rays_dev), t->aabbs.as<double>(), t->guide_info.as<float>(),
                               mode == MODE_CLOSEST ? t->tris.as<double>() : nullptr};
            if (mode == MODE_CLOSEST) launch_wide_items<float, MODE_CLOSEST, 1>(t, nullptr, n_rays, wg, h, items_log4, ovf_flag, false, ga);
            else launch_wide_items<float, MODE_INDICES, 1>(t, nullptr, n_rays, wg, h, items_log4, ovf_flag, false, ga);
            return;
        }
    }
    switch (mode) {
        case MODE_INDICES: launch_wide_items<T, MODE_INDICES>(t, rays_dev, n_rays, w, h, items_log4, ovf_flag, early_items); break;
        case MODE_TRIANGLES: launch_wide_items<T, MODE_TRIANGLES>(t, rays_dev, n_rays, w, h, items_log4, ovf_flag, early_items); break;
        case MODE_ANY: launch_wide_items<T, MODE_ANY>(t, rays_dev, n_rays, w, h, items_log4, ovf_flag, false); break;
        case MODE_BOX_CLOSEST: launch_wide_items<T, MODE_BOX_CLOSEST>(t, rays_dev, n_rays, w, h, items_log4, ovf_flag, false); break;
        case MODE_BOX_FIRST: launch_wide_items<T, MODE_BOX_FIRST>(t, rays_dev, n_rays, w, h, items_log4, ovf_flag, false); break;
        case MODE_SPHERE_CLOSEST: launch_wide_items<T, MODE_SPHERE_CLOSEST>(t, rays_dev, n_rays, w, h, items_log4, ovf_flag, false); break;
        case MODE_SPHERE_FIRST: launch_wide_items<T, MODE_SPHERE_FIRST>(t, rays_dev, n_rays, w, h, items_log4, ovf_flag, false); break;
        default: launch_wide_items<T, MODE_CLOSEST>(t, rays_dev, n_rays, w, h, items_log4, ovf_flag, false); break;
    }
}
template void launch_wide_walk<float>(bvhgpu_tree*, const bvhgpu_ray_f32*, size_t, const WalkOut<float>&, bvhgpu_hits*, int, int, bool, bool, uint32_t*);
template void launch_wide_walk<double>(bvhgpu_tree*, const bvhgpu_ray_f64*, size_t, const WalkOut<double>&, bvhgpu_hits*, int, int, bool, bool, uint32_t*);

template <typename T>
size_t wide_walk_grid(const bvhgpu_ctx* ctx, size_t n_rays, int items_log4, bool coherent, bool use_guide) {
    if (sizeof(T) == 8 && use_guide) return wide_walk_grid<float>(ctx, n_rays, items_log4, coherent, false);
    const WideGeom<T> g(ctx, items_log4 == 0, coherent);
    return wide_grid(ctx, g.threads, g.wg_per_cu, n_rays, items_log4);
}
template size_t wide_walk_grid<float>(const bvhgpu_ctx*, size_t, int, bool, bool);
template size_t wide_walk_grid<double>(const bvhgpu_ctx*, size_t, int, bool, bool);

#ifdef BVH_WIDE_PROFILE
void debug_wide_prof(unsigned long long* out, size_t n) {
    (void)hipDeviceSynchronize();
    (void)hipMemcpyFromSymbol(out, HIP_SYMBOL(g_wide_prof), sizeof(unsigned long long) * n);
}
void debug_wide_util(unsigned long long* out, size_t n) {
    (void)hipDeviceSynchronize();
    (void)hipMemcpyFromSymbol(out, HIP_SYMBOL(g_wide_util), sizeof(unsigned long long) * n);
}
#endif

}
```

Measured before the change: 2980 Mrays/s.

## Fetch wide-node planes in ray-sign order to drop per-axis min/max in slab test

Precomputes, per ray, a byte offset per axis from the sign of its inverse direction. Wide-node child boxes are then loaded from LDS or global memory with near and far planes already swapped, so the slab test needs no per-axis min/max, only max3/min3. The reordering is only valid when every box has min <= max, so build, flatten and refit now detect inverted boxes and record a per-tree flag that the traversal kernel reads to pick between the ordered path and the old one. The change also narrows the global-stack indexing to 32-bit and adds extra atomics and memsets around build and flatten.

```diff
diff --git a/bvh_amd/csrc/build.hip b/bvh_amd/csrc/build.hip
--- a/bvh_amd/csrc/build.hip
+++ b/bvh_amd/csrc/build.hip
@@ -9,6 +9,7 @@
 constexpr int CTR_TOPMASK = BUILD_CTR_TOPMASK;
 constexpr uint32_t BUILD_FLAG_NONFINITE = 1u;
 constexpr uint32_t BUILD_FLAG_PERSIST_GAVE_UP = BSTAT_UNFINISHED;
+constexpr uint32_t BUILD_FLAG_INVERTED = BSTAT_INVERTED;
 constexpr uint32_t BUILD_FLAG_EMPTY_SPLIT = 2u;
 #ifndef BVH_MID_SMALL_MAXN
 #define BVH_MID_SMALL_MAXN 768
@@ -129,6 +130,7 @@
     const bool copy = a.src != a.aabbs;
     T* own = const_cast<T*>(a.aabbs);
     bool bad = false;
+    bool inverted = false;
     for (uint32_t i = blockIdx.x * blockDim.x + threadIdx.x; i < a.n; i += gridDim.x * blockDim.x) {
         a.idx[0][i] = i;
         const T* b = a.src + 6 * (size_t)i;
@@ -137,6 +139,8 @@
         for (int k = 0; k < 6; k++) bx[k] = b[k];
 #pragma unroll
         for (int k = 0; k < 6; k++) bad = bad || !(fabs(bx[k]) < Tr::inf());
+#pragma unroll
+        for (int k = 0; k < 3; k++) inverted = inverted || bx[k] > bx[3 + k];
         if (copy) {
 #pragma unroll
             for (int k = 0; k < 6; k++) own[6 * (size_t)i + k] = bx[k];
@@ -169,6 +173,7 @@
         }
     }
     if (a.n > 1 && __any(bad) && lane_id() == 0) atomicOr(&a.ctr[CTR_FLAGS], BUILD_FLAG_NONFINITE);
+    if (__any(inverted) && lane_id() == 0) atomicOr(&a.ctr[CTR_FLAGS], BUILD_FLAG_INVERTED);
     __syncthreads();
     if (threadIdx.x < STAT_KEYS) a.rootkeys[(size_t)blockIdx.x * STAT_KEYS + threadIdx.x] = sk[threadIdx.x];
 }
@@ -294,7 +299,9 @@
     for (int i = threadIdx.x; i < (int)(ROOTKEY_OFF / 4); i += 256) a.ctr[i] = 0;
 }
 
-template <typename T> __global__ __launch_bounds__(256) void k_publish_build(BuildArgs<T> a, uint32_t* __restrict__ host_page) {
+template <typename T> __global__ __launch_bounds__(256) void k_publish_build(BuildArgs<T> a, uint32_t* __restrict__ host_page, uint32_t* __restrict__ fact) {
+    if (threadIdx.x == 0) fact[0] = a.ctr[CTR_FLAGS];
+    __syncthreads();
     for (int i = threadIdx.x; i < (int)(ROOTKEY_OFF / 4); i += 256) { host_page[i] = a.ctr[i]; a.ctr[i] = 0; }
     __threadfence_system();
 }
@@ -2131,12 +2138,12 @@
         }
     }
     run_lower_tiers<T>(t, a, g, 0u, 0u);
-    t->bstat.reserve(64);
+    uint32_t* const fact = tree_fact(t);
     if (flatten_after && n >= 1)
         flatten_tree<T>(t, a.ctr, reinterpret_cast<uint32_t*>(t->pin), (uint32_t)(ROOTKEY_OFF / 4), t->bstat.as<uint32_t>(), (uint32_t)CTR_FLAGS,
                         (n > (size_t)MID_MAX && !t->pend_persist) ? (uint32_t)(CTR_LEVEL0 + 2 * lvl_slot(level)) : (uint32_t)CTR_FLAGS,
                         ctx->tune[BVHGPU_TUNE_FLATTEN_LAZY] != 0, inline_parts);
-    else hipLaunchKernelGGL(k_publish_build<T>, dim3(1), dim3(256), 0, st, a, reinterpret_cast<uint32_t*>(t->pin));
+    else hipLaunchKernelGGL(k_publish_build<T>, dim3(1), dim3(256), 0, st, a, reinterpret_cast<uint32_t*>(t->pin), fact);
     t->ctr_ready = true;
     t->pending_build = true; t->pend_level = level; t->pend_flatten = flatten_after;
 }
@@ -2183,7 +2190,7 @@
             if (pin[CTR_LEVEL0 + 2 * lvl_slot(level)] == 0) break;
         }
         run_lower_tiers<T>(t, a, g, mid2_done, small_done);
-        hipLaunchKernelGGL(k_publish_build<T>, dim3(1), dim3(256), 0, st, a, reinterpret_cast<uint32_t*>(t->pin));
+        hipLaunchKernelGGL(k_publish_build<T>, dim3(1), dim3(256), 0, st, a, reinterpret_cast<uint32_t*>(t->pin), tree_fact(t));
         t->ctr_ready = true;
         if (t->pend_flatten) {
             BVH_HIP(hipMemsetAsync(t->wslot_node.p, 0xFF, WIDE_SLOTS * 4, st));
diff --git a/bvh_amd/csrc/common.hpp b/bvh_amd/csrc/common.hpp
--- a/bvh_amd/csrc/common.hpp
+++ b/bvh_amd/csrc/common.hpp
@@ -227,6 +227,48 @@
     asm("v_max3_f32 %0, %1, %2, %3" : "=v"(tmn) : "v"(a0), "v"(a1), "v"(a2));
     asm("v_min3_f32 %0, %1, %2, %3" : "=v"(tmx) : "v"(b0), "v"(b1), "v"(b2));
     return (tmx >= tmn) & (tmx >= 0.0f);
+}
+template <typename T>
+__device__ __forceinline__ bool slab_hit_ordered(const T o[3], const T inv[3], const T nr[3], const T fr[3]) {
+    T l0 = (nr[0] - o[0]) * inv[0], h0 = (fr[0] - o[0]) * inv[0];
+    T l1 = (nr[1] - o[1]) * inv[1], h1 = (fr[1] - o[1]) * inv[1];
+    T l2 = (nr[2] - o[2]) * inv[2], h2 = (fr[2] - o[2]) * inv[2];
+    T tmn = fmax(fmax(l0, l1), l2);
+    T tmx = fmin(fmin(h0, h1), h2);
+    return (tmx >= tmn) & (tmx >= (T)0);
+}
+template <>
+__device__ __forceinline__ bool slab_hit_ordered<float>(const float o[3], const float inv[3], const float nr[3], const float fr[3]) {
+    float l0 = (nr[0] - o[0]) * inv[0], h0 = (fr[0] - o[0]) * inv[0];
+    float l1 = (nr[1] - o[1]) * inv[1], h1 = (fr[1] - o[1]) * inv[1];
+    float l2 = (nr[2] - o[2]) * inv[2], h2 = (fr[2] - o[2]) * inv[2];
+    float tmn, tmx;
+    asm("v_max3_f32 %0, %1, %2, %3" : "=v"(tmn) : "v"(l0), "v"(l1), "v"(l2));
+    asm("v_min3_f32 %0, %1, %2, %3" : "=v"(tmx) : "v"(h0), "v"(h1), "v"(h2));
+    return (tmx >= tmn) & (tmx >= 0.0f);
+}
+template <typename T>
+__device__ __forceinline__ bool slab_hit_ordered_len(const T o[3], const T inv[3], const T nr[3], const T fr[3], T& len) {
+    T l0 = (nr[0] - o[0]) * inv[0], h0 = (fr[0] - o[0]) * inv[0];
+    T l1 = (nr[1] - o[1]) * inv[1], h1 = (fr[1] - o[1]) * inv[1];
+    T l2 = (nr[2] - o[2]) * inv[2], h2 = (fr[2] - o[2]) * inv[2];
+    T tmn = fmax(fmax(l0, l1), l2);
+    T tmx = fmin(fmin(h0, h1), h2);
+    const T t0 = fmax(tmn, (T)0);
+    len = tmx - t0;
+    return tmx >= t0;
+}
+template <>
+__device__ __forceinline__ bool slab_hit_ordered_len<float>(const float o[3], const float inv[3], const float nr[3], const float fr[3], float& len) {
+    float l0 = (nr[0] - o[0]) * inv[0], h0 = (fr[0] - o[0]) * inv[0];
+    float l1 = (nr[1] - o[1]) * inv[1], h1 = (fr[1] - o[1]) * inv[1];
+    float l2 = (nr[2] - o[2]) * inv[2], h2 = (fr[2] - o[2]) * inv[2];
+    float tmn, tmx, t0;
+    asm("v_max3_f32 %0, %1, %2, %3" : "=v"(tmn) : "v"(l0), "v"(l1), "v"(l2));
+    asm("v_min3_f32 %0, %1, %2, %3" : "=v"(tmx) : "v"(h0), "v"(h1), "v"(h2));
+    asm("v_max_f32 %0, 0, %1" : "=v"(t0) : "v"(tmn));
+    len = tmx - t0;
+    return tmx >= t0;
 }
 template <typename T>
 __device__ __forceinline__ bool slab_hit_finite_len(const T o[3], const T inv[3], const T mn[3], const T mx[3], T& len) {
diff --git a/bvh_amd/csrc/engine.hpp b/bvh_amd/csrc/engine.hpp
--- a/bvh_amd/csrc/engine.hpp
+++ b/bvh_amd/csrc/engine.hpp
@@ -139,6 +139,7 @@
     std::vector<bvhgpu_hits*> waiters;
     hipEvent_t ev_top = nullptr;
     uint64_t ev_top_gen = 0;
+    bool refit_inverted = false;
     bool exact_only = false;
     int pend_level = 0;
     bool pend_persist = false;
@@ -279,6 +280,12 @@
 void join_flat(bvhgpu_tree* t);
 constexpr uint32_t BSTAT_NONFINITE = 1u, BSTAT_EMPTY_SPLIT = 2u;
 constexpr uint32_t BSTAT_UNFINISHED = 0x100u;
+constexpr uint32_t BSTAT_INVERTED = 4u;
+inline uint32_t* tree_fact(bvhgpu_tree* t) {
+    if (t->bstat.reserve(64)) BVH_HIP(hipMemsetAsync(t->bstat.p, 0xFF, 64, t->ctx->stream));
+    return t->bstat.as<uint32_t>() + 1;
+}
+inline void tree_fact_set(bvhgpu_tree* t, bool regular) { BVH_HIP(hipMemsetAsync(tree_fact(t), regular ? 0 : 0xFF, sizeof(uint32_t), t->ctx->stream)); }
 constexpr int BUILD_CTR_TOPMASK = 5;
 template <typename T> void wide_from_trav(bvhgpu_tree* t);
 void recv_finalize(bvhgpu_tree* t);
diff --git a/bvh_amd/csrc/flatten.hip b/bvh_amd/csrc/flatten.hip
--- a/bvh_amd/csrc/flatten.hip
+++ b/bvh_amd/csrc/flatten.hip
@@ -17,7 +17,11 @@
                                                  float* __restrict__ guide_info, uint32_t inline_parts) {
     if (pub_ctr && blockIdx.x == 0) {
         if (bstat) {
-            if (threadIdx.x == 0) bstat[0] = pub_ctr[flags_idx] | ((level_idx != flags_idx && pub_ctr[level_idx] != 0u) ? BSTAT_UNFINISHED : 0u);
+            if (threadIdx.x == 0) {
+                const uint32_t s = pub_ctr[flags_idx] | ((level_idx != flags_idx && pub_ctr[level_idx] != 0u) ? BSTAT_UNFINISHED : 0u);
+                bstat[0] = s;
+                bstat[1] = s;
+            }
             __syncthreads();
         }
         for (uint32_t k = threadIdx.x; k < pub_words; k += blockDim.x) { pub_host[k] = pub_ctr[k]; pub_ctr[k] = 0; }
@@ -68,7 +72,7 @@
 __global__ __launch_bounds__(256) void k_wide(const TravNode<T>* __restrict__ trav, uint32_t n_nodes, uint32_t n_trav,
                                               const uint32_t* __restrict__ slot_entry, uint32_t n_bin_slots,
                                               WideNode<T>* __restrict__ wide, uint32_t* __restrict__ wslot_node,
-                                              WideNode<float>* __restrict__ guide, float* __restrict__ guide_info) {
+                                              WideNode<float>* __restrict__ guide, float* __restrict__ guide_info, uint32_t* __restrict__ fact) {
     const uint32_t b = blockIdx.x * blockDim.x + threadIdx.x;
     if (b < WIDE_SLOTS) {
         int k = 0;
@@ -102,12 +106,14 @@
         child = c.exit < n_trav ? c.exit : n_trav - 1u;
     }
     WideNode<T> w;
+    bool inverted = false;
 #pragma unroll
     for (int c = 0; c < 4; c++) {
 #pragma unroll
-        for (int k = 0; k < 3; k++) { w.mn[k][c] = s[c].mn[k]; w.mx[k][c] = s[c].mx[k]; }
+        for (int k = 0; k < 3; k++) { w.mn[k][c] = s[c].mn[k]; w.mx[k][c] = s[c].mx[k]; inverted = inverted || s[c].mn[k] > s[c].mx[k]; }
         w.ref[c] = s[c].ref;
     }
+    if (inverted) atomicOr(fact, BSTAT_INVERTED);
     for (int k = 0; k < (int)(sizeof(w._pad) / 4); k++) w._pad[k] = 0;
     wide[b] = w;
     if (sizeof(T) == 8 && guide && n_trav >= 2u) {
@@ -127,10 +133,11 @@
     t->wslot_node.reserve(WIDE_SLOTS * 4);
     const bool with_guide = sizeof(T) == 8;
     if (with_guide) { t->wide_guide.reserve((size_t)nn * sizeof(WideNode<float>)); t->guide_info.reserve(16); }
+    tree_fact_set(t, true);
     hipLaunchKernelGGL(k_wide<T>, dim3((std::max(nn, WIDE_SLOTS) + 255) / 256), dim3(256), 0, t->ctx->stream, t->trav.as<TravNode<T>>(),
                        nn, (uint32_t)t->n_trav, t->slot_entry.as<uint32_t>(), (uint32_t)TopCfg<T>::SLOTS, t->wide.as<WideNode<T>>(),
                        t->wslot_node.as<uint32_t>(), with_guide ? t->wide_guide.as<WideNode<float>>() : nullptr,
-                       with_guide ? t->guide_info.as<float>() : nullptr);
+                       with_guide ? t->guide_info.as<float>() : nullptr, tree_fact(t));
     BVH_HIP(hipGetLastError());
     t->has_wide = true;
     t->has_guide = with_guide;
diff --git a/bvh_amd/csrc/refit.hip b/bvh_amd/csrc/refit.hip
--- a/bvh_amd/csrc/refit.hip
+++ b/bvh_amd/csrc/refit.hip
@@ -101,10 +101,14 @@
 
 template <typename T>
 __global__ __launch_bounds__(256) void k_refit_check(const T* __restrict__ aabbs, size_t count, uint32_t* __restrict__ flag) {
-    bool bad = false;
-    for (size_t i = (size_t)blockIdx.x * blockDim.x + threadIdx.x; i < count; i += (size_t)gridDim.x * blockDim.x)
-        bad = bad || !(fabs(aabbs[i]) < Traits<T>::inf());
-    if (__any(bad) && lane_id() == 0) atomicOr(flag, 1u);
+    bool bad = false, inverted = false;
+    for (size_t i = (size_t)blockIdx.x * blockDim.x + threadIdx.x; i < count; i += (size_t)gridDim.x * blockDim.x) {
+        const T v = aabbs[i];
+        bad = bad || !(fabs(v) < Traits<T>::inf());
+        if (i % 6 < 3) inverted = inverted || v > aabbs[i + 3];
+    }
+    if (__any(bad) && lane_id() == 0) atomicOr(flag, BSTAT_NONFINITE);
+    if (__any(inverted) && lane_id() == 0) atomicOr(flag, BSTAT_INVERTED);
 }
 
 template <typename T> bool refit_input_ok(bvhgpu_tree* t, const T* aabbs_dev) {
@@ -121,7 +125,8 @@
     uint32_t* host = static_cast<uint32_t*>(ctx->pinned);
     BVH_HIP(hipMemcpyAsync(host, flag, sizeof(uint32_t), hipMemcpyDeviceToHost, st));
     BVH_HIP(hipStreamSynchronize(st));
-    return *host == 0u;
+    t->refit_inverted = (*host & BSTAT_INVERTED) != 0u;
+    return (*host & BSTAT_NONFINITE) == 0u;
 }
 
 template bool refit_input_ok<float>(bvhgpu_tree*, const float*);
@@ -158,6 +163,7 @@
     BVH_HIP(hipGetLastError());
     if (t->ctx->timing) { BVH_HIP(hipEventRecord(t->ctx->ev[1], st)); t->ctx->ev_set |= 1u; }
     t->exact_only = false;
+    tree_fact_set(t, !t->refit_inverted);
     if (t->flattened) flatten_tree<T>(t, nullptr, nullptr, 0, nullptr, 0, 0, t->ctx->tune[BVHGPU_TUNE_FLATTEN_LAZY] != 0);
 }
 
diff --git a/bvh_amd/csrc/walk.hpp b/bvh_amd/csrc/walk.hpp
--- a/bvh_amd/csrc/walk.hpp
+++ b/bvh_amd/csrc/walk.hpp
@@ -144,6 +144,20 @@
     if (t > Traits<T>::eps()) { out[0] = t; out[1] = t1; }
 }
 
+#ifndef BVH_WIDE_ORDERED_PLANES
+#define BVH_WIDE_ORDERED_PLANES 1
+#endif
+template <typename T> struct WidePlanes {
+    static constexpr uint32_t GROUP = 4u * (uint32_t)sizeof(T), HALF = 3u * GROUP, REFS = 2u * HALF;
+    static_assert(HALF < 256u, "a near offset fits a byte");
+    static __device__ __forceinline__ uint32_t pack(const T inv[3]) {
+        return (inv[0] < (T)0 ? HALF : 0u) | (inv[1] < (T)0 ? HALF << 8 : 0u) | (inv[2] < (T)0 ? HALF << 16 : 0u);
+    }
+    static __device__ __forceinline__ uint32_t near_offset(uint32_t po, int k) { return (po >> (8 * k)) & 0xFFu; }
+    static constexpr uint32_t NONFINITE = 0x80000000u;
+    static __device__ __forceinline__ uint32_t of_ray(const T inv[3], bool fin) { return pack(inv) | (fin ? 0u : NONFINITE); }
+};
+
 template <typename T, int MODE> struct LaneRay {
     T o[3], inv[3];
     T d[mode_tris(MODE) || mode_sphere(MODE) ? 3 : 1];
@@ -330,6 +344,48 @@
         for (int j = 0; j < CHUNKS; j++) c[j] = q[j];
         WideRegs<T> r;
         __builtin_memcpy(&r, c, sizeof r);
+        return r;
+    }
+    static constexpr int GC = (int)(WidePlanes<T>::GROUP / 16);
+    static_assert(offsetof(WideNode<T>, mx) == WidePlanes<T>::HALF && offsetof(WideNode<T>, ref) == WidePlanes<T>::REFS &&
+                  offsetof(WideRegs<T>, mx) == WidePlanes<T>::HALF && offsetof(WideRegs<T>, ref) == WidePlanes<T>::REFS, "plane groups of a wide node");
+    typedef uint32_t Chunk __attribute__((ext_vector_type(4)));
+    template <typename P> static __device__ __forceinline__ void put(WideRegs<T>& r, int k, P n, P f) {
+        Chunk cn[GC], cf[GC];
+#pragma unroll
+        for (int j = 0; j < GC; j++) { cn[j] = n[j]; cf[j] = f[j]; }
+        __builtin_memcpy(r.mn[k], cn, sizeof cn);
+        __builtin_memcpy(r.mx[k], cf, sizeof cf);
+    }
+    static __device__ __forceinline__ uint32_t per_fetch(uint32_t po) { asm("" : "+v"(po)); return po; }
+    static __device__ __forceinline__ WideRegs<T> from_lds_ordered(const uint4* nodes, uint32_t slot, uint32_t po) {
+        using P = WidePlanes<T>;
+        typedef __attribute__((address_space(3))) const Chunk* Lds;
+        const uint32_t q = (uint32_t)(uintptr_t)(Lds)reinterpret_cast<const Chunk*>(nodes + __umul24(slot, (uint32_t)CHUNKS));
+        po = per_fetch(po);
+        WideRegs<T> r;
+#pragma unroll
+        for (int k = 0; k < 3; k++) {
+            const uint32_t nk = P::near_offset(po, k);
+            put(r, k, (Lds)(q + nk) + k * GC, (Lds)(q - nk) + (3 + k) * GC);
+        }
+        const Chunk rf = ((Lds)q)[6 * GC];
+        r.ref[0] = rf.x; r.ref[1] = rf.y; r.ref[2] = rf.z; r.ref[3] = rf.w;
+        return r;
+    }
+    static __device__ __forceinline__ WideRegs<T> from_global_ordered(const WideNode<T>* __restrict__ wide, uint32_t id, uint32_t po) {
+        using P = WidePlanes<T>;
+        const char* base = reinterpret_cast<const char*>(wide);
+        const uint32_t nb = id * (uint32_t)sizeof(WideNode<T>), fb = nb + P::HALF;
+        po = per_fetch(po);
+        WideRegs<T> r;
+#pragma unroll
+        for (int k = 0; k < 3; k++) {
+            const uint32_t nk = P::near_offset(po, k);
+            put(r, k, reinterpret_cast<const Chunk*>(base + (size_t)(nb + nk)) + k * GC, reinterpret_cast<const Chunk*>(base + (size_t)(fb - nk)) + k * GC);
+        }
+        const uint4 rf = *reinterpret_cast<const uint4*>(base + (size_t)nb + P::REFS);
+        r.ref[0] = rf.x; r.ref[1] = rf.y; r.ref[2] = rf.z; r.ref[3] = rf.w;
         return r;
     }
 };
diff --git a/bvh_amd/csrc/walk_wide.hip b/bvh_amd/csrc/walk_wide.hip
--- a/bvh_amd/csrc/walk_wide.hip
+++ b/bvh_amd/csrc/walk_wide.hip
@@ -29,7 +29,7 @@
 }
 
 template <typename T, bool EXACT>
-__device__ __forceinline__ uint32_t wide_hits(const T o[3], const T inv[3], const WideRegs<T>& nd) {
+__device__ __forceinline__ uint32_t wide_hits(const T o[3], const T inv[3], const WideRegs<T>& nd, uint32_t po = 0u) {
     uint32_t m = 0;
     if (!EXACT) {
 #pragma unroll
@@ -50,12 +50,27 @@
             const T mn1[3] = {nd.mn[0][c1], nd.mn[1][c1], nd.mn[2][c1]}, mx1[3] = {nd.mx[0][c1], nd.mx[1][c1], nd.mx[2][c1]};
             T jmn[3], jmx[3];
 #pragma unroll
-            for (int k = 0; k < 3; k++) { jmn[k] = tmin(mn0[k], mn1[k]); jmx[k] = tmax(mx0[k], mx1[k]); }
+            for (int k = 0; k < 3; k++) {
+                const bool swapped = WidePlanes<T>::near_offset(po, k) != 0u;
+                jmn[k] = swapped ? tmax(mn0[k], mn1[k]) : tmin(mn0[k], mn1[k]);
+                jmx[k] = swapped ? tmin(mx0[k], mx1[k]) : tmax(mx0[k], mx1[k]);
+            }
             if (slab_hit<T>(o, inv, jmn, jmx, t0, t1)) {
                 if (slab_hit<T>(o, inv, mn0, mx0, t0, t1)) m |= 1u << c0;
                 if (slab_hit<T>(o, inv, mn1, mx1, t0, t1)) m |= 1u << c1;
             }
         }
+    }
+    return m;
+}
+
+template <typename T>
+__device__ __forceinline__ uint32_t wide_hits_ordered(const T o[3], const T inv[3], const WideRegs<T>& nd) {
+    uint32_t m = 0;
+#pragma unroll
+    for (int c = 0; c < 4; c++) {
+        const T nr[3] = {nd.mn[0][c], nd.mn[1][c], nd.mn[2][c]}, fr[3] = {nd.mx[0][c], nd.mx[1][c], nd.mx[2][c]};
+        m |= slab_hit_ordered<T>(o, inv, nr, fr) ? (1u << c) : 0u;
     }
     return m;
 }
@@ -68,8 +83,9 @@
     uint32_t ref[16];
     T half_diag[16];
 };
+template <typename T> __device__ __forceinline__ bool box_inverted(const T b[6]) { return b[0] > b[3] || b[1] > b[4] || b[2] > b[5]; }
 template <typename T, int ITEMS_LOG4>
-__device__ __forceinline__ void item_table_build(const WideNode<T>* __restrict__ wide, ItemTable<T>* tb, uint32_t tid) {
+__device__ __forceinline__ void item_table_build(const WideNode<T>* __restrict__ wide, ItemTable<T>* tb, uint32_t tid, uint32_t* inverted) {
     constexpr uint32_t ITEMS = 1u << (2 * ITEMS_LOG4);
     if (tid < ITEMS) {
         const uint32_t c = ITEMS_LOG4 == 2 ? tid >> 2 : tid, k = tid & 3u;
@@ -98,6 +114,8 @@
         tb->ref[tid] = ref;
         const T dx = b[3] - b[0], dy = b[4] - b[1], dz = b[5] - b[2];
         tb->half_diag[tid] = (T)BVH_WIDE_LONG_FRAC * sqrt(dx * dx + dy * dy + dz * dz);
+        const unsigned long long any = __ballot(box_inverted<T>(b));
+        if (tid == 0) *inverted = any != 0ull ? 1u : 0u;
     }
 }
 template <int ITEMS_LOG4> __device__ __forceinline__ uint32_t item_slot(uint32_t j) {
@@ -109,7 +127,7 @@
 template <typename T, int L4, bool GUIDE = false>
 __device__ __forceinline__ void filter_rays_into_list(const ItemTable<T>* tb, const typename Traits<T>::Ray* __restrict__ rays, uint32_t n_rays,
                                                       uint32_t* __restrict__ list, uint32_t per_wg, uint32_t my_rays, uint32_t G, uint32_t b,
-                                                      uint32_t tid, uint32_t bd, int lane, uint32_t* s_nlist, uint32_t* s_nback,
+                                                      uint32_t tid, uint32_t bd, int lane, uint32_t* s_nlist, uint32_t* s_nback, bool ordered,
                                                       const bvhgpu_ray_f64* __restrict__ rays64 = nullptr, double guide_S = 0.0, bool* any_bad = nullptr) {
     constexpr uint32_t ITEMS = 1u << (2 * L4);
     for (uint32_t l0 = 0; l0 < my_rays; l0 += bd) {
@@ -129,6 +147,18 @@
             }
             if (!ray_is_finite<T>(o, inv)) {
                 mask = 1u << WIDE_ITEM_WHOLE; longm = mask;
+            } else if (BVH_WIDE_ORDERED_PLANES && ordered) {
+                const T *nr[3], *fr[3];
+#pragma unroll
+                for (int k = 0; k < 3; k++) { const int far_first = inv[k] < (T)0 ? 3 : 0; nr[k] = &tb->box[0][k] + far_first; fr[k] = &tb->box[0][k] + (3 - far_first); }
+#pragma unroll 4
+                for (uint32_t j = 0; j < ITEMS; j++) {
+                    const T n3[3] = {nr[0][6 * j], nr[1][6 * j], nr[2][6 * j]}, f3[3] = {fr[0][6 * j], fr[1][6 * j], fr[2][6 * j]};
+                    T len;
+                    const bool hit = slab_hit_ordered_len<T>(o, inv, n3, f3, len);
+                    mask |= hit ? (1u << j) : 0u;
+                    longm |= (hit && len > tb->half_diag[j]) ? (1u << j) : 0u;
+                }
             } else {
 #pragma unroll 4
                 for (uint32_t j = 0; j < ITEMS; j++) {
@@ -174,7 +204,7 @@
     constexpr int L4 = 2;
     constexpr uint32_t ITEMS = 16;
     __shared__ ItemTable<T> tb;
-    __shared__ uint32_t s_nlist, s_nback, s_bad;
+    __shared__ uint32_t s_nlist, s_nback, s_bad, s_inverted;
     const uint32_t tid = threadIdx.x, bd = blockDim.x;
     const int lane = lane_id();
     if (tid == 0) { s_nlist = 0u; s_nback = 0u; s_bad = (build_ctr[BUILD_CTR_TOPMASK] & 0xFFFEu) == 0xFFFEu ? 0u : 1u; }
@@ -199,6 +229,8 @@
         }
         ok = ok && cnt > 1u;
         if (!ok) atomicOr(&s_bad, 1u);
+        const unsigned long long any_inv = __ballot(ok && box_inverted<T>(bx));
+        if (tid == 0) s_inverted = any_inv != 0ull ? 1u : 0u;
 #pragma unroll
         for (int k = 0; k < 6; k++) tb.box[tid][k] = bx[k];
         const T dx = bx[3] - bx[0], dy = bx[4] - bx[1], dz = bx[5] - bx[2];
@@ -210,7 +242,8 @@
     const uint32_t my_blocks = n_blocks > blockIdx.x ? (n_blocks - blockIdx.x + gridDim.x - 1u) / gridDim.x : 0u;
     const uint32_t per_wg = ((n_blocks + gridDim.x - 1u) / gridDim.x) << 6;
     uint32_t* list = list_all + (size_t)blockIdx.x * per_wg * ITEMS;
-    filter_rays_into_list<T, L4>(&tb, rays, n_rays, list, per_wg, my_blocks << 6, gridDim.x, blockIdx.x, tid, bd, lane, &s_nlist, &s_nback);
+    filter_rays_into_list<T, L4>(&tb, rays, n_rays, list, per_wg, my_blocks << 6, gridDim.x, blockIdx.x, tid, bd, lane, &s_nlist, &s_nback,
+                                 __builtin_amdgcn_readfirstlane(s_inverted) == 0u);
     __syncthreads();
     if (tid == 0) { wg_items[2u * blockIdx.x] = s_nlist; wg_items[2u * blockIdx.x + 1u] = s_nback; }
 }
@@ -255,7 +288,10 @@
 __global__ __launch_bounds__(MAX_THREADS, MIN_WAVES) void k_traverse_wide(
     const WideNode<T>* __restrict__ wide, const uint32_t* __restrict__ wslot_node, uint32_t K, uint32_t stack_lds,
     const typename Traits<T>::Ray* __restrict__ rays, uint32_t n_rays, uint32_t* __restrict__ list_all, const uint32_t* __restrict__ wg_items,
-    WalkOut<T> w, uint32_t* __restrict__ gstack, uint32_t gstack_cap, uint32_t* __restrict__ overflow, GuideArgs ga, uint32_t whole_steps) {
+    WalkOut<T> w, uint32_t* __restrict__ gstack, uint32_t gstack_cap, uint32_t* __restrict__ overflow, GuideArgs ga, uint32_t whole_steps,
+    const uint32_t* __restrict__ fact) {
+    const uint32_t irregular = __builtin_amdgcn_readfirstlane((BVH_WIDE_ORDERED_PLANES && fact != nullptr) ? fact[0] : 1u);
+    const bool big = fact == nullptr;
     static_assert(GUIDE == 0 || ((MODE == MODE_INDICES || MODE == MODE_CLOSEST) && sizeof(T) == 4), "the guide walk is the f32 walk of an f64 index / closest-hit batch");
     constexpr bool GUIDE_CLOSEST = GUIDE != 0 && MODE == MODE_CLOSEST;
     double gbest = 0.0;
@@ -268,13 +304,14 @@
     uint32_t& s_next = *reinterpret_cast<uint32_t*>(wsmem);
     uint32_t& s_nlist = *(reinterpret_cast<uint32_t*>(wsmem) + 1);
     uint32_t& s_nback = *(reinterpret_cast<uint32_t*>(wsmem) + 2);
+    uint32_t& s_tb_inverted = *(reinterpret_cast<uint32_t*>(wsmem) + 3);
     uint32_t* s_item_ref = reinterpret_cast<uint32_t*>(wsmem + 1);
     uint4* nodes = wsmem + 5;
     uint32_t* s_stack = reinterpret_cast<uint32_t*>(nodes + (size_t)CH * K);
     const uint32_t bd = blockDim.x, tid = threadIdx.x;
     const int WIDE_INNER_STEPS = ITEMS_LOG4 == 0 ? (int)whole_steps : BVH_WIDE_INNER_STEPS;
     constexpr uint32_t SB = MAX_THREADS;
-    const size_t G = (size_t)gridDim.x * bd, gid = (size_t)blockIdx.x * bd + tid;
+    const uint32_t G = gridDim.x * bd, gid = blockIdx.x * bd + tid;
     const int lane = lane_id();
     const unsigned long long lt = lanemask_lt();
     double guide_S = 0.0;
@@ -311,7 +348,7 @@
     uint32_t* list = nullptr;
     if (ITEMS_LOG4 > 0) {
         __shared__ ItemTable<T> tb;
-        item_table_build<T, L4>(wide, &tb, tid);
+        item_table_build<T, L4>(wide, &tb, tid, &s_tb_inverted);
         __syncthreads();
         if (tid < ITEMS) {
             const uint32_t ref = tb.ref[tid], slot = item_slot<L4>(tid);
@@ -322,9 +359,10 @@
         if (pre_front != NONE) {
             if (tid == 0) { s_nlist = pre_front; s_nback = wg_items[2u * blockIdx.x + 1u]; }
         } else {
+            const bool tb_ordered = __builtin_amdgcn_readfirstlane(s_tb_inverted) == 0u;
             if constexpr (GUIDE != 0) filter_rays_into_list<T, L4, true>(&tb, rays, n_rays, list, per_wg, my_rays, gridDim.x, blockIdx.x, tid, bd, lane, &s_nlist, &s_nback,
-                                                                            ga.rays64, guide_S, &guide_bad);
-            else filter_rays_into_list<T, L4>(&tb, rays, n_rays, list, per_wg, my_rays, gridDim.x, blockIdx.x, tid, bd, lane, &s_nlist, &s_nback);
+                                                                            tb_ordered, ga.rays64, guide_S, &guide_bad);
+            else filter_rays_into_list<T, L4>(&tb, rays, n_rays, list, per_wg, my_rays, gridDim.x, blockIdx.x, tid, bd, lane, &s_nlist, &s_nback, tb_ordered);
         }
         __threadfence_block();
     }
@@ -338,6 +376,7 @@
 
     LaneRay<T, MODE> ray;
     ray.clear();
+    uint32_t ray_po = 0u;
     uint32_t cur = CUR_NONE, sp = 0, item = NONE;
     bool exhausted = wg_begin >= wg_end;
     bool ovf = false;
@@ -345,7 +384,7 @@
     PoolCursor pc;
     auto push_slow = [&](uint32_t v) {
         if (sp < stack_lds) s_stack[sp * SB + tid] = v;
-        else if (sp - stack_lds < gstack_cap) gstack[(size_t)(sp - stack_lds) * G + gid] = v;
+        else if (sp - stack_lds < gstack_cap) gstack[(sp - stack_lds) * G + gid] = v;
         else ovf = true;
         sp++;
     };
@@ -353,7 +392,7 @@
         if (sp == 0) return CUR_NONE;
         sp--;
         if (sp < stack_lds) return s_stack[sp * SB + tid];
-        return sp - stack_lds < gstack_cap ? gstack[(size_t)(sp - stack_lds) * G + gid] : CUR_NONE;
+        return sp - stack_lds < gstack_cap ? gstack[(sp - stack_lds) * G + gid] : CUR_NONE;
     };
     while (true) {
         bool run = cur != CUR_NONE;
@@ -419,6 +458,7 @@
                         if (item < n_rays) {
                             if constexpr (GUIDE != 0) { bool bad; guide_ray_load(ga.rays64, item, guide_S, ray.o, ray.inv, bad); guide_bad = guide_bad || bad; ray.loaded(item); gbest = __builtin_inf(); }
                             else ray.load(rays, item, w.tmax);
+                            ray_po = WidePlanes<T>::of_ray(ray.inv, ray.fin);
                             cur = WIDE_INNER | WIDE_RESIDENT | 0u;
                         } else {
                             item = NONE;
@@ -428,6 +468,7 @@
                         const uint32_t j = item & ((1u << WIDE_ITEM_BITS) - 1u);
                         if constexpr (GUIDE != 0) { bool bad; guide_ray_load(ga.rays64, item >> WIDE_ITEM_BITS, guide_S, ray.o, ray.inv, bad); ray.loaded(item >> WIDE_ITEM_BITS); gbest = __builtin_inf(); }
                         else ray.load(rays, item >> WIDE_ITEM_BITS, w.tmax);
+                        ray_po = WidePlanes<T>::of_ray(ray.inv, ray.fin);
                         cur = j == WIDE_ITEM_WHOLE ? (WIDE_INNER | WIDE_RESIDENT | 0u) : s_item_ref[j];
                         if (j == WIDE_ITEM_WHOLE) item = item & ~((1u << WIDE_ITEM_BITS) - 1u);
                     }
@@ -439,7 +480,8 @@
             }
             if (!__any(run)) break;
         }
-        const bool fast = !__any(run && !ray.fin);
+        const bool fast = !__any(run && (ray_po & WidePlanes<T>::NONFINITE) != 0u);
+        const bool ordered = fast && irregular == 0u;
 #ifdef BVH_WIDE_PROFILE
         prof_steps += WIDE_INNER_STEPS;
         pu[9]++; pu[10] += fast ? 0 : 1;
@@ -461,10 +503,13 @@
 #endif
             if (cur & WIDE_INNER) {
                 const uint32_t id = cur & (WIDE_RESIDENT - 1u);
+                const uint32_t po = BVH_WIDE_ORDERED_PLANES ? ray_po : 0u;
                 WideRegs<T> nd;
-                if (cur & WIDE_RESIDENT) nd = WideIo<T>::from_lds(nodes, id);
+                if (cur & WIDE_RESIDENT) nd = WideIo<T>::from_lds_ordered(nodes, id, big ? 0u : po);
+                else if (!big) nd = WideIo<T>::from_global_ordered(wide, id, po);
                 else nd = WideIo<T>::from_global(wide + id);
-                const uint32_t m = fast ? wide_hits<T, false>(ray.o, ray.inv, nd) : wide_hits<T, true>(ray.o, ray.inv, nd);
+                const uint32_t m = ordered ? wide_hits_ordered<T>(ray.o, ray.inv, nd)
+                                           : (fast ? wide_hits<T, false>(ray.o, ray.inv, nd) : wide_hits<T, true>(ray.o, ray.inv, nd, big ? 0u : po));
                 const uint32_t first = m & (0u - m);
                 const uint32_t rest = m ^ first;
 #ifdef BVH_WIDE_PROFILE
@@ -527,10 +572,12 @@
         pc.left = 0;
     }
     walk_epilogue<T, MODE>(w, pc, lane, false, 0, 0, 0, 0);
-    if (MODE < MODE_CLOSEST && w.scan_sums) {
+    uint32_t* scan_sums = w.scan_sums;
+    asm volatile("" : "+s"(scan_sums));
+    if (MODE < MODE_CLOSEST && scan_sums) {
         __syncthreads();
         for (uint32_t b = tid; b < my_blocks; b += bd)
-            if (s_bsum[b]) atomicAdd(&w.scan_sums[(b * gridDim.x + blockIdx.x) / (uint32_t)(SCAN_BLOCK / 64)], s_bsum[b]);
+            if (s_bsum[b]) atomicAdd(&scan_sums[(b * gridDim.x + blockIdx.x) / (uint32_t)(SCAN_BLOCK / 64)], s_bsum[b]);
     }
 #ifdef BVH_WIDE_PROFILE
     if (lane == 0) {
@@ -621,7 +668,8 @@
     hipLaunchKernelGGL(kern, grid, dim3(g.threads), g.lds_bytes, st, GUIDE ? t->wide_guide.as<WideNode<T>>() : t->wide.as<WideNode<T>>(),
                        t->wslot_node.as<uint32_t>(), g.K, g.stack_lds, rays_dev, (uint32_t)n_rays, list, wg_items, w, h->wstack.as<uint32_t>(),
                        WIDE_GSTACK, ovf_flag, ga,
-                       (uint32_t)((h->flags & BVHGPU_TRAVERSE_COHERENT) ? BVH_WIDE_INNER_STEPS_COHERENT : BVH_WIDE_INNER_STEPS_WHOLE));
+                       (uint32_t)((h->flags & BVHGPU_TRAVERSE_COHERENT) ? BVH_WIDE_INNER_STEPS_COHERENT : BVH_WIDE_INNER_STEPS_WHOLE),
+                       (uint64_t)t->n_nodes * sizeof(WideNode<T>) < ((uint64_t)1 << 32) ? tree_fact(t) : (uint32_t*)nullptr);
     h->walk_kernel = name;
 }
 
```

Result: no change. 3029 Mrays/s, median of 6 (+1.7%).
